# lenke182/flood-uav-video-segmentation

Hardware: AMD Instinct MI355X
Metric: segmentation FPS @713x713 (PSPNet-ResNet50 keyframe + linear interp, frame_delta=5) (higher is better)
Workload: dtype f32

## Files before the change

### flood_uav_video_segmentation_amd/_lib.py

```python
import ctypes
import os

import torch

_HERE = os.path.dirname(os.path.abspath(__file__))
LIB_PATH = os.path.join(_HERE, "libfloodseg.so")

c_float_p = ctypes.POINTER(ctypes.c_float)
c_void = ctypes.c_void_p
c_int = ctypes.c_int
c_i64 = ctypes.c_int64
c_f32 = ctypes.c_float


class FsConfig(ctypes.Structure):
    _fields_ = [("arch", c_int), ("layers", c_int), ("classes", c_int), ("patch", c_int), ("d_model", c_int),
                ("n_layers", c_int), ("dec_layers", c_int), ("image_size", c_int), ("flags", c_int), ("winograd_tile", c_int)]


ARCH_PSPNET = 0
ARCH_DEEPLABV3 = 1
ARCH_SEGMENTER = 2
OPT_NO_WINOGRAD = 1
OPT_NO_FUSED_HEAD = 2
OPT_NO_FUSED_SHORTCUT = 4
OPT_NO_FUSED_WINOGRAD = 8
OPT_NO_SPLIT_BF16 = 16
OPT_NO_RES_TOUCH = 128
OPT_NO_FUSED_POOL = 256
OPT_NO_FUSED_QKV = 1024
CONV_CHUNK_MAJOR = 0x400

_SIGNATURES = {
    "fs_version": (c_int, []),
    "fs_last_error": (ctypes.c_char_p, []),
    "fs_create": (c_int, [ctypes.POINTER(FsConfig), ctypes.POINTER(c_void)]),
    "fs_destroy": (c_int, [c_void]),
    "fs_load_weight": (c_int, [c_void, ctypes.c_char_p, c_void, ctypes.POINTER(c_i64), c_int, c_int, c_void]),
    "fs_finalize": (c_int, [c_void, c_void]),
    "fs_feature_shape": (c_int, [c_void, c_int, c_int, ctypes.POINTER(c_int), ctypes.POINTER(c_int), ctypes.POINTER(c_int)]),
    "fs_workspace_bytes": (ctypes.c_size_t, [c_void, c_int, c_int, c_int]),
    "fs_reserve": (c_int, [c_void, c_int, c_int, c_int, c_void]),
    "fs_reserved_bytes": (ctypes.c_size_t, [c_void]),
    "fs_encoder_forward": (c_int, [c_void, c_void, c_int, c_int, c_int, c_void, c_void]),
    "fs_decoder_forward": (c_int, [c_void, c_void, c_int, c_int, c_int, c_void, c_void]),
    "fs_segment_forward": (c_int, [c_void, c_void, c_int, c_int, c_int, c_void, c_void]),
    "fs_encoder_forward2": (c_int, [c_void, c_void, c_int, c_void, c_int, c_int, c_int, c_void, c_void]),
    "fs_segment_forward2": (c_int, [c_void, c_void, c_int, c_void, c_int, c_int, c_int, c_void, c_void]),
    "fs_segment_crops": (c_int, [c_void, c_void, c_void, c_int, c_int, c_int, ctypes.POINTER(c_int), ctypes.POINTER(c_int), c_int, c_int,
                                 c_void, c_void]),
    "fs_profile_enable": (c_int, [c_void, c_int]),
    "fs_profile_dump": (c_int, [c_void, ctypes.c_char_p, ctypes.c_size_t]),
    "fs_grid_sample_nchw": (c_int, [c_void, c_int, c_int, c_int, c_int, c_void, c_int, c_int, c_void, c_int, c_void]),
    "fs_grid_sample_nhwc": (c_int, [c_void, c_int, c_int, c_int, c_int, c_int, c_void, c_int, c_int, c_void, c_int, c_int, c_void]),
    "fs_resize_bilinear_nchw": (c_int, [c_void, c_int, c_int, c_int, c_void, c_int, c_int, c_int, c_void]),
    "fs_resize_bilinear_nhwc": (c_int, [c_void, c_int, c_int, c_int, c_int, c_int, c_void, c_int, c_int, c_int, c_int, c_void]),
    "fs_blend": (c_int, [c_void, c_f32, c_void, c_f32, c_void, c_i64, c_void]),
    "fs_seg_tail": (c_int, [c_void, c_void, ctypes.POINTER(c_void), ctypes.POINTER(c_void), c_int, c_int, c_int, c_int, c_int,
                            c_int, c_int, c_int, c_int, c_void, c_void, c_void, c_void]),
    "fs_feat_tail": (c_int, [c_void, c_void, c_int, c_int, c_int, ctypes.POINTER(c_void), ctypes.POINTER(c_void), c_int, c_int, c_void, c_int, c_int,
                             c_int, c_int, c_void, c_void, c_void]),
    "fs_seg_tail_accumulate": (c_int, [c_void, c_void, ctypes.POINTER(c_void), ctypes.POINTER(c_void), c_int, c_int, c_int, c_int, c_int,
                                       c_int, c_int, c_int, c_int, c_void, c_void, c_int, c_int, c_int, c_int, c_void, c_void]),
    "fs_canvas_resize_argmax": (c_int, [c_void, c_int, c_int, c_int, c_int, c_void, c_int, c_int, c_void]),
    "fs_crop_grids": (c_int, [ctypes.POINTER(c_void), c_int, c_int, c_int, c_int, c_int, c_int, ctypes.POINTER(c_int), ctypes.POINTER(c_int),
                              c_int, c_int, c_void, c_void]),
    "fs_crops_fuse": (c_int, [c_void, c_void, c_void, c_int, ctypes.POINTER(c_int), ctypes.POINTER(c_int)] + [c_int] * 9 + [c_void, c_void, c_int, c_int,
                              c_void, c_void]),
    "fs_argmax_u8": (c_int, [c_void, c_int, c_int, c_i64, c_void, c_void]),
    "fs_resize_crop": (c_int, [c_void, c_int, c_int, c_int, c_int, c_int, c_int, c_int, c_void, c_void, c_int, c_int, c_void]),
    "fs_resize_argmax_u8": (c_int, [c_void, c_int, c_int, c_int, c_int, c_void, c_int, c_int, c_void]),
    "fs_iou_hist": (c_int, [c_void, c_void, c_i64, c_int, c_int, c_void, c_void]),
    "fs_colorize": (c_int, [c_void, c_void, c_int, c_void, c_i64, c_void]),
    "fs_mv_to_grids": (c_int, [c_void, c_int, c_int, c_int, c_int, c_int, c_int, c_int, c_void, c_void, c_void, c_void]),
    "fs_softmax_accumulate": (c_int, [c_void, c_int, c_int, c_int, c_int, c_void, c_void, c_int, c_int, c_int, c_int, c_void]),
    "fs_canvas_finish": (c_int, [c_void, c_void, c_int, c_int, c_i64, c_void, c_void]),
    "fs_ms_prepare": (c_int, [c_void] + [c_int] * 6 + [c_float_p, c_float_p, c_void, c_int, c_void]),
    "fs_ms_fuse": (c_int, [c_void, c_void, c_int, ctypes.POINTER(c_int), ctypes.POINTER(c_int)] + [c_int] * 9 + [c_void, c_void] + [c_int] * 4
                   + [c_void, c_void]),
    "fs_test_hooks": (c_void, []),
}

_HOOKS = [
# ... 49 lines not shown
    ("seg_tail_weighted", c_int, [c_void, c_void, ctypes.POINTER(c_void), ctypes.POINTER(c_void)] + [c_int] * 9 + [c_void] * 4 + [c_int] * 4
     + [c_void, c_void, c_void]),
    ("crops_fuse_weighted", c_int, [c_void, c_void, c_void, c_int, ctypes.POINTER(c_int), ctypes.POINTER(c_int)] + [c_int] * 9
     + [c_void, c_void, c_int, c_int, c_void, c_void, c_void]),
    ("feat_tail_weighted", c_int, [c_void, c_void, c_int, c_int, c_int, ctypes.POINTER(c_void), ctypes.POINTER(c_void), c_int, c_int, c_void, c_int,
                                   c_int, c_int, c_int, c_void, c_void, c_void, c_void]),
    ("mask_confidence", c_int, [c_void] + [c_int] * 4 + [c_void, c_void, c_int, c_int, c_void]),
    ("canvas_confidence", c_int, [c_void] + [c_int] * 4 + [c_void, c_void, c_int, c_int, c_void]),
    ("frame_report", c_int, [c_void, c_void] + [c_int] * 5 + [c_void, c_void]),
    ("mask_regions", c_int, [c_void] + [c_int] * 5 + [c_void, c_void]),
    ("region_table", c_int, [c_void, c_void, c_void] + [c_int] * 6 + [c_void] * 5),
    ("region_filter", c_int, [c_void, c_void, c_void] + [c_int] * 6 + [c_void, c_void, c_void]),
    ("region_links", c_int, [c_void] * 6 + [c_int] * 6 + [c_void] * 5),
    ("region_tracks", c_int, [c_void] * 4 + [c_int] * 2 + [c_void] * 3),
    ("region_links_mc", c_int, [c_void] * 8 + [c_int] * 8 + [c_void] * 5),
]
EXT2_MAGIC = 0x4653455854414232

_EXT3_HOOKS = [
    ("region_outlines", c_int, [c_void] + [c_int] * 7 + [c_void] * 6),
]
EXT3_MAGIC = 0x4653455854414233

_EXT4_HOOKS = [
    ("outline_simplify", c_int, [c_void] * 3 + [c_int] * 5 + [c_void] * 5),
]
EXT4_MAGIC = 0x4653455854414234

_EXT5_HOOKS = [
    ("frame_compose_regions", c_int, [c_void, c_int, c_int, c_void, c_int, c_void, c_void, c_void] + [c_int] * 5 + [c_void, c_void, c_void] + [c_int] * 3
     + [c_void] * 4 + [c_int, c_void, c_int, c_void, c_int, c_int, c_i64, ctypes.c_uint32, ctypes.c_uint32, c_void, c_void]),
]
EXT5_MAGIC = 0x4653455854414235

_EXT6_HOOKS = [
    ("mask_stabilize", c_int, [c_void] * 4 + [c_int] * 9 + [c_void] * 5),
]
EXT6_MAGIC = 0x4653455854414236

_EXT7_HOOKS = [
    ("mask_distance", c_int, [c_void] + [c_int] * 3 + [ctypes.c_uint32, c_int] + [c_void] * 4),
    ("region_proximity", c_int, [c_void] * 5 + [c_int] * 5 + [ctypes.c_uint32, c_void, c_int] + [c_void] * 3),
]
EXT7_MAGIC = 0x4653455854414237

_EXT8_HOOKS = [
    ("global_motion", c_int, [c_void] * 3 + [ctypes.c_uint32] + [c_int] * 6 + [ctypes.c_int64, c_int, c_void, c_void]),
    ("pose_chain", c_int, [c_void] * 3 + [c_int] * 8 + [c_void]),
    ("mosaic_accumulate", c_int, [c_void] * 2 + [c_int] * 8 + [c_void] * 2),
    ("mosaic_resolve", c_int, [c_void] + [c_int] * 3 + [c_void] * 5),
]
EXT8_MAGIC = 0x4653455854414238


class FsTestApi(ctypes.Structure):
    _fields_ = [("size", ctypes.c_size_t)] + [(name, ctypes.CFUNCTYPE(res, *args)) for name, res, args in _HOOKS]


class FsExtApi(ctypes.Structure):
    _fields_ = [("magic", ctypes.c_uint64), ("size", ctypes.c_size_t)] + [(name, ctypes.CFUNCTYPE(res, *args)) for name, res, args in _EXT_HOOKS]


class FsHookTables(ctypes.Structure):
    _fields_ = [("test", FsTestApi), ("ext", FsExtApi)]


class FsExt2Api(ctypes.Structure):
    _fields_ = [("magic", ctypes.c_uint64), ("size", ctypes.c_size_t)] + [(name, ctypes.CFUNCTYPE(res, *args)) for name, res, args in _EXT2_HOOKS]


class FsHookTables2(ctypes.Structure):
    _fields_ = [("base", FsHookTables), ("ext2", FsExt2Api)]


class FsExt3Api(ctypes.Structure):
    _fields_ = [("magic", ctypes.c_uint64), ("size", ctypes.c_size_t)] + [(name, ctypes.CFUNCTYPE(res, *args)) for name, res, args in _EXT3_HOOKS]


class FsHookTables3(ctypes.Structure):
    _fields_ = [("base2", FsHookTables2), ("ext3", FsExt3Api)]


class FsExt4Api(ctypes.Structure):
    _fields_ = [("magic", ctypes.c_uint64), ("size", ctypes.c_size_t)] + [(name, ctypes.CFUNCTYPE(res, *args)) for name, res, args in _EXT4_HOOKS]


class FsHookTables4(ctypes.Structure):
    _fields_ = [("base3", FsHookTables3), ("ext4", FsExt4Api)]


class FsExt5Api(ctypes.Structure):
    _fields_ = [("magic", ctypes.c_uint64), ("size", ctypes.c_size_t)] + [(name, ctypes.CFUNCTYPE(res, *args)) for name, res, args in _EXT5_HOOKS]


class FsHookTables5(ctypes.Structure):
    _fields_ = [("base4", FsHookTables4), ("ext5", FsExt5Api)]


class FsExt6Api(ctypes.Structure):
    _fields_ = [("magic", ctypes.c_uint64), ("size", ctypes.c_size_t)] + [(name, ctypes.CFUNCTYPE(res, *args)) for name, res, args in _EXT6_HOOKS]


class FsHookTables6(ctypes.Structure):
    _fields_ = [("base5", FsHookTables5), ("ext6", FsExt6Api)]


class FsExt7Api(ctypes.Structure):
    _fields_ = [("magic", ctypes.c_uint64), ("size", ctypes.c_size_t)] + [(name, ctypes.CFUNCTYPE(res, *args)) for name, res, args in _EXT7_HOOKS]


class FsHookTables7(ctypes.Structure):
    _fields_ = [("base6", FsHookTables6), ("ext7", FsExt7Api)]


class FsExt8Api(ctypes.Structure):
    _fields_ = [("magic", ctypes.c_uint64), ("size", ctypes.c_size_t)] + [(name, ctypes.CFUNCTYPE(res, *args)) for name, res, args in _EXT8_HOOKS]


class FsHookTables8(ctypes.Structure):
    _fields_ = [("base7", FsHookTables7), ("ext8", FsExt8Api)]


class _Library:

    def __init__(self, cdll):
        self._cdll = cdll
        self._hooks = None
        self._ext = None
        self._ext2 = None
        self._ext3 = None
        self._ext4 = None
        self._ext5 = None
        self._ext6 = None
        self._ext7 = None
        self._ext8 = None

    def __getattr__(self, name):
        if name.startswith("fs_") and any(name == "fs_" + h[0] for h in _EXT8_HOOKS):
            if self._ext8 is None:
                all7 = ctypes.cast(self._cdll.fs_test_hooks(), ctypes.POINTER(FsHookTables7)).contents
                all5 = all7.base6.base5
                all2 = all5.base4.base3.base2
                if (all2.base.test.size != ctypes.sizeof(FsTestApi) or all2.base.ext.magic != EXT_MAGIC or all2.base.ext.size != ctypes.sizeof(FsExtApi)
                        or all2.ext2.magic != EXT2_MAGIC or all2.ext2.size != ctypes.sizeof(FsExt2Api)
                        or all5.base4.base3.ext3.magic != EXT3_MAGIC or all5.base4.base3.ext3.size != ctypes.sizeof(FsExt3Api)
                        or all5.base4.ext4.magic != EXT4_MAGIC or all5.base4.ext4.size != ctypes.sizeof(FsExt4Api)
                        or all5.ext5.magic != EXT5_MAGIC or all5.ext5.size != ctypes.sizeof(FsExt5Api)
                        or all7.base6.ext6.magic != EXT6_MAGIC or all7.base6.ext6.size != ctypes.sizeof(FsExt6Api)
                        or all7.ext7.magic != EXT7_MAGIC or all7.ext7.size != ctypes.sizeof(FsExt7Api)):
                    raise RuntimeError(f"floodseg: the library's first eight hook tables are not the ones this binding knows ({name} is missing)")
                ext8 = ctypes.cast(self._cdll.fs_test_hooks(), ctypes.POINTER(FsHookTables8)).contents.ext8
                if ext8.magic != EXT8_MAGIC:
                    raise RuntimeError(f"floodseg: the library has no eighth extension table ({name} is missing)")
                self._ext8 = ext8
            member = getattr(FsExt8Api, name[3:])
            if self._ext8.size < member.offset + member.size:
                raise RuntimeError(f"floodseg: the library's eighth extension table is older than this binding ({name} is missing)")
            fn = getattr(self._ext8, name[3:])
            setattr(self, name, fn)
            return fn
        if name.startswith("fs_") and any(name == "fs_" + h[0] for h in _EXT7_HOOKS):
            if self._ext7 is None:
                all6 = ctypes.cast(self._cdll.fs_test_hooks(), ctypes.POINTER(FsHookTables6)).contents
                all5 = all6.base5
                all2 = all5.base4.base3.base2
                if (all2.base.test.size != ctypes.sizeof(FsTestApi) or all2.base.ext.magic != EXT_MAGIC or all2.base.ext.size != ctypes.sizeof(FsExtApi)
                        or all2.ext2.magic != EXT2_MAGIC or all2.ext2.size != ctypes.sizeof(FsExt2Api)
                        or all5.base4.base3.ext3.magic != EXT3_MAGIC or all5.base4.base3.ext3.size != ctypes.sizeof(FsExt3Api)
                        or all5.base4.ext4.magic != EXT4_MAGIC or all5.base4.ext4.size != ctypes.sizeof(FsExt4Api)
                        or all5.ext5.magic != EXT5_MAGIC or all5.ext5.size != ctypes.sizeof(FsExt5Api)
                        or all6.ext6.magic != EXT6_MAGIC or all6.ext6.size != ctypes.sizeof(FsExt6Api)):
                    raise RuntimeError(f"floodseg: the library's first seven hook tables are not the ones this binding knows ({name} is missing)")
                ext7 = ctypes.cast(self._cdll.fs_test_hooks(), ctypes.POINTER(FsHookTables7)).contents.ext7
                if ext7.magic != EXT7_MAGIC:
                    raise RuntimeError(f"floodseg: the library has no seventh extension table ({name} is missing)")
                self._ext7 = ext7
            member = getattr(FsExt7Api, name[3:])
            if self._ext7.size < member.offset + member.size:
                raise RuntimeError(f"floodseg: the library's seventh extension table is older than this binding ({name} is missing)")
            fn = getattr(self._ext7, name[3:])
            setattr(self, name, fn)
            return fn
        if name.startswith("fs_") and any(name == "fs_" + h[0] for h in _EXT6_HOOKS):
            if self._ext6 is None:
                all5 = ctypes.cast(self._cdll.fs_test_hooks(), ctypes.POINTER(FsHookTables5)).contents
                all2 = all5.base4.base3.base2
                if (all2.base.test.size != ctypes.sizeof(FsTestApi) or all2.base.ext.magic != EXT_MAGIC or all2.base.ext.size != ctypes.sizeof(FsExtApi)
                        or all2.ext2.magic != EXT2_MAGIC or all2.ext2.size != ctypes.sizeof(FsExt2Api)
                        or all5.base4.base3.ext3.magic != EXT3_MAGIC or all5.base4.base3.ext3.size != ctypes.sizeof(FsExt3Api)
                        or all5.base4.ext4.magic != EXT4_MAGIC or all5.base4.ext4.size != ctypes.sizeof(FsExt4Api)
# ... 111 lines not shown
            f"{LIB_PATH} not found: build it with `python -c 'import __graft_entry__ as g; g.build()'` "
            "(hipcc --offload-arch=gfx950); there is no CPU fallback for this path")
    lib = ctypes.CDLL(LIB_PATH)
    for name, (res, args) in _SIGNATURES.items():
        if ALLOW_MISSING and not hasattr(lib, name):
            continue
        fn = getattr(lib, name)
        fn.restype = res
        fn.argtypes = args
    _lib = _Library(lib)
    return _lib


def exported_symbols():
    return sorted(_SIGNATURES)


def hook_names():
    return [h[0] for h in _HOOKS]


def ext_hook_names():
    return [h[0] for h in _EXT_HOOKS]


def ext2_hook_names():
    return [h[0] for h in _EXT2_HOOKS]


def ext3_hook_names():
    return [h[0] for h in _EXT3_HOOKS]


def ext4_hook_names():
    return [h[0] for h in _EXT4_HOOKS]


def ext5_hook_names():
    return [h[0] for h in _EXT5_HOOKS]


def ext6_hook_names():
    return [h[0] for h in _EXT6_HOOKS]


def ext7_hook_names():
    return [h[0] for h in _EXT7_HOOKS]


def ext8_hook_names():
    return [h[0] for h in _EXT8_HOOKS]


def check(rc):
    if rc != 0:
        msg = load().fs_last_error()
        raise RuntimeError("floodseg: " + (msg.decode() if msg else f"error {rc}"))


def stream_ptr(device=None):
    return ctypes.c_void_p(torch.cuda.current_stream(device).cuda_stream)


def one_device(*tensors, handle_device=None, what="floodseg"):
    dev = None
    for t in tensors:
        if t is None:
            continue
        if not t.is_cuda:
            raise RuntimeError(f"{what}: tensors must live on the GPU (no CPU fallback exists)")
        if dev is None:
            dev = t.device
        elif t.device != dev:
            raise RuntimeError(f"{what}: tensors on different devices ({dev} and {t.device})")
    if dev is None:
        raise RuntimeError(f"{what}: no device tensor given")
    if handle_device is not None and dev != handle_device:
        raise RuntimeError(f"{what}: tensor on {dev} but the network's weights live on {handle_device}")
    return dev


def ptr(t):
    if t is None:
        return ctypes.c_void_p(0)
    return ctypes.c_void_p(t.data_ptr())
```

### flood_uav_video_segmentation_amd/csrc/conv_igemm.hip

```cpp
#include "kernels.h"
#include "igemm_epilogue.h"

#include <algorithm>
#include <cstdlib>

namespace fs {

#define FS_DMA_PUBLISH() { __builtin_amdgcn_s_waitcnt(0x0070); __syncthreads(); }
constexpr int conv_split_rows(int BN, int waves) { return (BN / 16 + waves - 1) / waves * waves * 16; }
template <int BM, int BN, bool SPLIT, int WAVES = 4>
constexpr int conv_tile_lds_floats() { return 2 * (BM * 32 + (SPLIT ? 3 * conv_split_rows(BN, WAVES) * 16 : BN * 32)); }

template <int TM>
__device__ __forceinline__ void split_unit(int lvl, int pr, const f32x4 (&raw)[TM][2], float (&rq)[4 * TM][2], u32x4 (&ah)[TM][3], bool pin) {
    const int pi = pr / 4, pe = pr % 4;
    float x0 = lvl == 0 ? raw[pi][pe >> 1][2 * (pe & 1)] : rq[pr][0];
    float x1 = lvl == 0 ? raw[pi][pe >> 1][2 * (pe & 1) + 1] : rq[pr][1];
    unsigned pk = split_round(x0, x1);
    if (pin) asm volatile("" : "+v"(pk));
    ah[pi][lvl][pe] = pk;
    if (lvl < 2) {
        split_residue(pk, x0, x1);
        rq[pr][0] = x0;
        rq[pr][1] = x1;
    }
}

template <int BM, int BN, int WGM, int WGN, bool DUAL, bool SPLIT>
__device__ __forceinline__ void conv_tile(ConvParams p, const int m0, const int n0, float* __restrict__ lds) {
#if defined(__HIP_DEVICE_COMPILE__)
    constexpr int BK = 32;
    constexpr int NT = 64 * WGM * WGN;
    constexpr int RSTEP = NT / 8;
    constexpr int WM = BM / WGM, WN = BN / WGN;
    constexpr int TM = WM / 32, TN = WN / 32;
    constexpr int BNL = SPLIT ? conv_split_rows(BN, NT / 64) : BN;
    constexpr int BPL = BNL * 16;
    constexpr int RA = BM / RSTEP, RB = SPLIT ? 3 * (BNL / 16) / (NT / 64) : BN / RSTEP;
    constexpr int RB1 = SPLIT ? (BNL / 16) / (NT / 64) : RB;
    static_assert(BN % 32 == 0 && WN % 32 == 0 && (SPLIT || BN % RSTEP == 0), "tile columns: whole 32-column MFMA blocks per wave");
    constexpr int STAGE = BM * BK + (SPLIT ? 3 * BPL : BN * BK);

    const int t = threadIdx.x, lane = t & 63, wv = t >> 6;
    const int wm = wv / WGN, wn = wv % WGN, l31 = lane & 31, hh = lane >> 5;
    const int wv_u = __builtin_amdgcn_readfirstlane(wv);
    const int M = p.B * p.Ho * p.Wo;
    const int K = p.KH * p.KW * p.Cin + (DUAL ? p.Cin2 : 0);
    const int cpt = p.Cin >> 5;
    const int nchunks1 = p.KH * p.KW * cpt;
    const int nchunks = nchunks1 + (DUAL ? p.Cin2 >> 5 : 0);

    const int sc = t & 7, r0 = t >> 3;
    const int swz = sc ^ ((r0 >> 1) & 7);
    constexpr unsigned SENT = 0x80000000u;
    const long long pad_off = ((long long)p.pad * p.W + p.pad) * p.ld_in;
    const unsigned a_bytes = (unsigned)(((long long)p.B * p.H * p.W * p.ld_in + pad_off) * 4);
    const __amdgpu_buffer_rsrc_t a_rsrc = __builtin_amdgcn_make_buffer_rsrc((void*)(p.in - pad_off), 0, a_bytes, 0x00020000);
    const int ldw = p.ld_wgt ? p.ld_wgt : K;
    const __amdgpu_buffer_rsrc_t b_rsrc =
        SPLIT ? __builtin_amdgcn_make_buffer_rsrc((void*)p.wgt3, 0, 2u * p.plane_bytes + (unsigned)((((long long)p.Cout - 1) * ldw + K) * 2), 0x00020000)
              : __builtin_amdgcn_make_buffer_rsrc((void*)p.wgt, 0, (unsigned)((((long long)p.Cout - 1) * ldw + K) * 4), 0x00020000);
    unsigned a_voff[RA], a_mask[RA];
    if (p.KH * p.KW == 1 && p.stride == 1 && p.pad == 0) {
#pragma unroll
        for (int j = 0; j < RA; ++j) {
            const int m = m0 + r0 + RSTEP * j;
            a_voff[j] = (unsigned)((m * p.ld_in + swz * 4) * 4);
            a_mask[j] = m < M ? 1u : 0u;
        }
    } else {
#pragma unroll
        for (int j = 0; j < RA; ++j) {
            const int m = m0 + r0 + RSTEP * j;
            const bool v = m < M;
            const int mm = v ? m : 0;
            const int hw = p.Ho * p.Wo;
            const int b = mm / hw;
            const int rem = mm - b * hw;
            const int oy = rem / p.Wo;
            const int ox = rem - oy * p.Wo;
            a_voff[j] = (unsigned)(((b * p.H * p.W + oy * p.stride * p.W + ox * p.stride) * p.ld_in + swz * 4) * 4);
// ... 198 lines not shown
            __builtin_amdgcn_sched_barrier(0);
            cur ^= 1;
        }
        asm volatile("" ::"v"(touch0), "v"(touch1));
        if (!DUAL && p.res) igemm_load_residual(rv, p, M, em_base, en_base);
#undef FS_READ3
#undef FS_STEP3
    } else {
    if (!DUAL && p.res && nchunks <= 2) igemm_load_residual(rv, p, M, em_base, en_base);
    FS_FRAGS(0, 0, a0, b0)
    for (int kc = 0; kc < nchunks; ++kc) {
        FS_FRAGS(cur, 1, a1, b1)
        FS_MMA(a0, b0)
        __builtin_amdgcn_sched_group_barrier(0x008, 1, 0);
        __builtin_amdgcn_sched_group_barrier(0x100, TM + TN, 0);
        __builtin_amdgcn_sched_group_barrier(0x008, 4 * TM * TN - 1, 0);
        __builtin_amdgcn_sched_barrier(0);
        FS_FRAGS(cur, 2, a0, b0)
        __builtin_amdgcn_sched_barrier(0);
        FS_MMA(a1, b1)
        __builtin_amdgcn_sched_barrier(0);
        FS_FRAGS(cur, 3, a1, b1)
        __builtin_amdgcn_sched_barrier(0);
        FS_MMA(a0, b0)
        __builtin_amdgcn_sched_barrier(0);
        FS_DMA_PUBLISH()
        if (kc + 2 < nchunks) {
            FS_DMA_ALL(cur)
            FS_DMA_ADVANCE()
        }
        if (!DUAL && p.res && kc + 3 == nchunks) igemm_load_residual(rv, p, M, em_base, en_base);
        if (kc + 1 < nchunks) FS_FRAGS(cur ^ 1, 0, a0, b0)
        __builtin_amdgcn_sched_barrier(0);
        FS_MMA(a1, b1)
        __builtin_amdgcn_sched_barrier(0);
        cur ^= 1;
    }
    }
#undef FS_DMA_ROW
#undef FS_DMA_ADVANCE
#undef FS_DMA_ALL
#undef FS_FRAGS
#undef FS_MMA

    if constexpr (SPLIT && !DUAL && BN == 96 && TM == 1) {
        const int Dm = p.kv_heads * 64;
        if (p.kv_k && n0 >= Dm) {
            const int kind = n0 >= 2 * Dm ? 2 : 1;
            igemm_epilogue_kv<TN>(acc, sc_n, sh_n, p, kind, em_base, en_base - kind * Dm, en_base < p.Cout, lane);
            return;
        }
    }
    if (!DUAL && p.res) {
        if (p.relu == 1) igemm_epilogue<1, true>(acc, rv, sc_n, sh_n, p, M, em_base, en_base);
        else if (p.relu == 2) igemm_epilogue<2, true>(acc, rv, sc_n, sh_n, p, M, em_base, en_base);
        else igemm_epilogue<0, true>(acc, rv, sc_n, sh_n, p, M, em_base, en_base);
    } else {
        if (p.relu == 1) igemm_epilogue<1, false>(acc, rv, sc_n, sh_n, p, M, em_base, en_base);
        else if (p.relu == 2) igemm_epilogue<2, false>(acc, rv, sc_n, sh_n, p, M, em_base, en_base);
        else igemm_epilogue<0, false>(acc, rv, sc_n, sh_n, p, M, em_base, en_base);
    }
#endif
}

template <int BM, int BN, int WGM = 2, int WGN = 2, bool DUAL = false, bool SPLIT = false>
__global__ __launch_bounds__(64 * WGM * WGN) void conv_igemm_dma_f32(ConvParams p, int tiles_m, int tiles_n) {
#if defined(__HIP_DEVICE_COMPILE__)
    constexpr int PM = 8;
    __shared__ __attribute__((aligned(1024))) float lds[conv_tile_lds_floats<BM, BN, SPLIT, WGM * WGN>()];
    const int nblk = gridDim.x, bid = blockIdx.x;
    const int q = nblk >> 3, rr = nblk & 7, xcd = bid & 7;
    const int lid = (xcd < rr ? xcd * (q + 1) : rr * (q + 1) + (xcd - rr) * q) + (bid >> 3);
    const int per_group = tiles_m * tiles_n;
    const int grp = lid / per_group;
    const int lig = lid - grp * per_group;
    const int panel = lig / (PM * tiles_n);
    const int within = lig - panel * (PM * tiles_n);
    const int prow = min(PM, tiles_m - panel * PM);
    const int m0 = (panel * PM + within % prow) * BM, n0 = (within / prow) * BN;
    p.in += (long long)grp * p.g_in;
    p.wgt += (long long)grp * p.g_wgt;
    if (SPLIT) p.wgt3 = (const char*)p.wgt3 + (long long)grp * p.g_wgt * 2;
    p.out += (long long)grp * p.g_out;
    p.kv_b = grp;
    conv_tile<BM, BN, WGM, WGN, DUAL, SPLIT>(p, m0, n0, lds);
#endif
}

namespace {
struct TileCfg { int bm, bn; const char* name; };
const TileCfg kTiles[7] = {{0, 0, "auto"}, {128, 128, "igemm128x128"}, {128, 64, "igemm128x64"},
                           {64, 64, "igemm64x64"}, {64, 128, "igemm64x128"}, {0, 0, nullptr}, {128, 96, "split128x96"}};
bool tile_id_ok(int tile) { return tile >= 0 && tile <= 6 && tile != 5; }

int pick_tile(const ConvParams& p) {
    const int M = p.B * p.Ho * p.Wo;
    const double eff[7] = {0, 1.00, 0.92, 0.80, 0.92, 0, 0.97};
    int best = 1;
    double best_t = 1e300;
    const int last = p.in2 ? 2 : p.wgt3 ? 3 : 4;
    for (int c = 1; c <= 6; ++c) {
        if (c > last && !(c == 6 && p.wgt3 && !p.in2 && p.Cout % 96 == 0)) continue;
        const int bm = kTiles[c].bm, bn = kTiles[c].bn;
        if (p.Cout < bn && bn > 64) continue;
        const long tiles = (long)cdiv(M, bm) * cdiv(p.Cout, bn) * (p.groups > 1 ? p.groups : 1);
        const long per_cu = (tiles + 255) / 256;
        const double t = (double)per_cu * bm * bn / (eff[c] * (per_cu >= 2 ? 1.0 : 0.8));
        if (t < best_t) { best_t = t; best = c; }
    }
    return best;
}
}

const char* conv_igemm_tile_name(const ConvParams& p, int tile) {
    if (!tile_id_ok(tile)) return "(bad tile)";
    if (tile == 0) tile = pick_tile(p);
    if (p.in2 && p.wgt3) return tile == 2 ? "split128x64cat" : "split128x128cat";
    if (p.in2) return tile == 2 ? "igemm128x64cat" : "igemm128x128cat";
    if (p.wgt3) return tile == 1 ? "split128x128" : tile == 2 ? "split128x64" : tile == 4 ? "split64x128" : tile == 6 ? "split128x96" : "split64x64";
    return kTiles[tile].name;
}

namespace {
bool ldw_ok(const ConvParams& p) { return (p.ld_wgt ? p.ld_wgt : p.KH * p.KW * p.Cin + (p.in2 ? p.Cin2 : 0)) % 8 == 0; }

__global__ void split_bf16x3_kernel(const float* __restrict__ w, long long n, unsigned short* __restrict__ planes) {
    const long long i = (long long)blockIdx.x * blockDim.x + threadIdx.x;
    if (i >= n) return;
    split3(w[i], planes[i], planes[n + i], planes[2 * n + i]);
}
}

int launch_split_bf16x3(const float* w, long long n, void* planes, hipStream_t s) {
    FS_REQUIRE(w && planes && n > 0 && n % 8 == 0, "split_bf16x3: bad arguments (n=%lld)", n);
    hipLaunchKernelGGL(split_bf16x3_kernel, dim3((unsigned)((n + 255) / 256)), dim3(256), 0, s, w, n, (unsigned short*)planes);
    FS_HIP(hipGetLastError());
    return 0;
}

namespace {
int check_conv_params(const ConvParams& p) {
    FS_REQUIRE(p.Cin % 32 == 0, "conv_igemm: Cin=%d must be a multiple of 32", p.Cin);
    if (p.in2) {
        FS_REQUIRE(p.KH == 1 && p.KW == 1 && p.stride == 1 && p.pad == 0 && p.res == nullptr && p.groups <= 1,
                   "conv_igemm: a concatenated-K launch takes two 1x1 convs, the first with stride 1, and no residual");
        FS_REQUIRE(p.Cin2 >= 32 && p.Cin2 % 32 == 0 && p.ld_in2 % 4 == 0 && p.ld_in2 >= p.Cin2 && p.stride2 >= 1 && ((uintptr_t)p.in2 & 15) == 0,
                   "conv_igemm: bad second operand (Cin2=%d ld=%d stride=%d)", p.Cin2, p.ld_in2, p.stride2);
        FS_REQUIRE((p.H2 - 1) / p.stride2 + 1 == p.Ho && (p.W2 - 1) / p.stride2 + 1 == p.Wo, "conv_igemm: second operand %dx%d / stride %d does not give %dx%d",
                   p.H2, p.W2, p.stride2, p.Ho, p.Wo);
        FS_REQUIRE((int64_t)p.B * p.H2 * p.W2 * p.ld_in2 * 4 < (int64_t)1 << 31, "conv_igemm: second operand must be smaller than 2 GiB");
    }
    FS_REQUIRE(p.ld_in % 4 == 0 && p.ld_in >= p.Cin, "conv_igemm: bad ld_in=%d (Cin=%d)", p.ld_in, p.Cin);
    FS_REQUIRE(p.ld_out >= p.Cout, "conv_igemm: bad ld_out=%d (Cout=%d)", p.ld_out, p.Cout);
    FS_REQUIRE(((uintptr_t)p.in & 15) == 0 && ((uintptr_t)p.wgt & 15) == 0, "conv_igemm: unaligned operand");
    FS_REQUIRE(p.Ho == (p.H + 2 * p.pad - p.dil * (p.KH - 1) - 1) / p.stride + 1 &&
               p.Wo == (p.W + 2 * p.pad - p.dil * (p.KW - 1) - 1) / p.stride + 1,
               "conv_igemm: output geometry %dx%d inconsistent with input %dx%d", p.Ho, p.Wo, p.H, p.W);
    FS_REQUIRE(((int64_t)p.B * p.H * p.W * p.ld_in + ((int64_t)p.pad * p.W + p.pad) * p.ld_in) * 4 < (int64_t)1 << 31,
               "conv_igemm: input tensor must be smaller than 2 GiB");
    FS_REQUIRE((int64_t)p.Cout * std::max(p.ld_wgt, p.KH * p.KW * p.Cin + (p.in2 ? p.Cin2 : 0)) * 4 < (int64_t)1 << 31, "conv_igemm: filter bank must be smaller than 2 GiB");
    FS_REQUIRE(p.ld_wgt == 0 || (p.ld_wgt >= p.KH * p.KW * p.Cin + (p.in2 ? p.Cin2 : 0) && p.ld_wgt % 4 == 0), "conv_igemm: bad ld_wgt=%d", p.ld_wgt);
    FS_REQUIRE(p.KH * p.KW <= 32, "conv_igemm: at most 32 filter taps");
    FS_REQUIRE((int64_t)p.B * p.Ho * p.Wo * p.ld_out * 4 < (int64_t)1 << 31 && ((uintptr_t)p.out & 3) == 0,
               "conv_igemm: output tensor must be smaller than 2 GiB");
    FS_REQUIRE(p.res == nullptr || (int64_t)p.B * p.Ho * p.Wo * p.ld_res * 4 < (int64_t)1 << 31, "conv_igemm: residual tensor must be smaller than 2 GiB");
    if (!(p.res == nullptr || p.ld_res >= p.Cout)) return fail("conv_igemm: bad ld_res");
    return 0;
}
}

int launch_conv_igemm(const ConvParams& p, hipStream_t s, int tile) {
    FS_TRY(check_conv_params(p));
    FS_REQUIRE(tile_id_ok(tile), "conv_igemm: tile %d is not 0..4 or 6", tile);
    if (tile == 0) tile = pick_tile(p);
    FS_REQUIRE(tile < 6 || (p.wgt3 && !p.in2), "conv_igemm: tile 6 (128 x 96) exists on the split-operand route only");
    const int M = p.B * p.Ho * p.Wo;
    const int bm = kTiles[tile].bm, bn = kTiles[tile].bn;
    const int tm = cdiv(M, bm), tn = cdiv(p.Cout, bn);
    const int groups = p.groups > 1 ? p.groups : 1;
    FS_REQUIRE(groups == 1 || p.res == nullptr, "conv_igemm: grouped GEMM has no residual input");
    const dim3 grid(tm * tn * groups), block(256);
    if (p.kv_k) {
        const int Dm = p.kv_heads * 64;
        FS_REQUIRE(tile == 6 && p.wgt3 && !p.in2 && !p.res && p.KH == 1 && p.KW == 1 && p.stride == 1 && p.pad == 0 && p.relu == 0,
                   "conv_igemm: the K / V plane epilogue belongs to a plain Linear on the 128 x 96 split tile");
        FS_REQUIRE(p.kv_vt && p.kv_heads >= 1 && Dm % 96 == 0 && p.Cout == 3 * Dm && p.kv_N == M && p.kv_Npad % 32 == 0 && p.kv_Npad >= M &&
                       p.kv_Npad <= tm * bm && (int64_t)3 * p.kv_plane_bytes < (int64_t)1 << 31 &&
                       (int64_t)p.kv_plane_bytes == (int64_t)groups * p.kv_heads * p.kv_Npad * 128 && (((uintptr_t)p.kv_k | (uintptr_t)p.kv_vt) & 15) == 0,
                   "conv_igemm: bad K / V plane geometry (heads %d, tokens %d, padded %d)", p.kv_heads, p.kv_N, p.kv_Npad);
    }
    if (p.wgt3) {
        FS_REQUIRE(((uintptr_t)p.wgt3 & 15) == 0 && p.plane_bytes % 16 == 0 && (int64_t)3 * p.plane_bytes < (int64_t)1 << 31 && ldw_ok(p),
                   "conv_igemm: bad split filter bank (plane_bytes=%u)", p.plane_bytes);
        FS_REQUIRE((int64_t)groups * p.g_wgt * 2 <= (int64_t)p.plane_bytes, "conv_igemm: the groups' filters (%d x %lld) exceed a plane of the split bank", groups, p.g_wgt);
    }
    if (p.in2 && p.wgt3) {
        if (tile == 2) hipLaunchKernelGGL((conv_igemm_dma_f32<128, 64, 4, 1, true, true>), grid, block, 0, s, p, tm, tn);
        else if (tile == 1) hipLaunchKernelGGL((conv_igemm_dma_f32<128, 128, 4, 1, true, true>), grid, block, 0, s, p, tm, tn);
        else return fail("conv_igemm: concatenated-K launches use tile 1 or 2");
        FS_HIP(hipGetLastError());
        return 0;
    }
    if (p.in2) {
        if (tile == 2) hipLaunchKernelGGL((conv_igemm_dma_f32<128, 64, 2, 2, true>), grid, block, 0, s, p, tm, tn);
        else if (tile == 1) hipLaunchKernelGGL((conv_igemm_dma_f32<128, 128, 2, 2, true>), grid, block, 0, s, p, tm, tn);
        else return fail("conv_igemm: concatenated-K launches use tile 1 or 2");
        FS_HIP(hipGetLastError());
        return 0;
    }
    if (p.wgt3) {
        switch (tile) {
            case 1: hipLaunchKernelGGL((conv_igemm_dma_f32<128, 128, 4, 1, false, true>), grid, block, 0, s, p, tm, tn); break;
            case 2: hipLaunchKernelGGL((conv_igemm_dma_f32<128, 64, 4, 1, false, true>), grid, block, 0, s, p, tm, tn); break;
            case 3: hipLaunchKernelGGL((conv_igemm_dma_f32<64, 64, 2, 2, false, true>), grid, block, 0, s, p, tm, tn); break;
            case 4: hipLaunchKernelGGL((conv_igemm_dma_f32<64, 128, 2, 2, false, true>), grid, block, 0, s, p, tm, tn); break;
            case 6: hipLaunchKernelGGL((conv_igemm_dma_f32<128, 96, 4, 1, false, true>), grid, block, 0, s, p, tm, tn); break;
            default: return fail("conv_igemm: the split-operand route has tiles 1, 2, 3, 4 and 6");
        }
        FS_HIP(hipGetLastError());
        return 0;
    }
#define FS_CONV_LAUNCH(BM_, BN_) hipLaunchKernelGGL((conv_igemm_dma_f32<BM_, BN_>), grid, block, 0, s, p, tm, tn);
    switch (tile) {
        case 1: FS_CONV_LAUNCH(128, 128) break;
        case 2: FS_CONV_LAUNCH(128, 64) break;
        case 3: FS_CONV_LAUNCH(64, 64) break;
        default: FS_CONV_LAUNCH(64, 128) break;
    }
#undef FS_CONV_LAUNCH
    FS_HIP(hipGetLastError());
    return 0;
}


}
```

### flood_uav_video_segmentation_amd/csrc/igemm_epilogue.h

```cpp
#pragma once
#include "kernels.h"
#include "split.h"

namespace fs {

#if defined(__HIP_DEVICE_COMPILE__)
template <int TM, int TN>
__device__ __forceinline__ void igemm_load_residual(float (&rv)[TM][TN][16], const ConvParams& p, int M, int m_base, int n_base) {
    constexpr unsigned SENT = 0x80000000u;
    const __amdgpu_buffer_rsrc_t r_rsrc = __builtin_amdgcn_make_buffer_rsrc((void*)p.res, 0, (unsigned)((long long)M * p.ld_res * 4), 0x00020000);
    const unsigned row_r = (unsigned)p.ld_res * 4u;
#pragma unroll
    for (int j = 0; j < TN; ++j) {
        const int n = n_base + j * 32;
#pragma unroll
        for (int i = 0; i < TM; ++i) {
            const unsigned vr = n < p.Cout ? (unsigned)(m_base + i * 32) * row_r + (unsigned)n * 4u : SENT;
#pragma unroll
            for (int e = 0; e < 16; ++e)
                rv[i][j][e] = __builtin_bit_cast(float, __builtin_amdgcn_raw_buffer_load_b32(r_rsrc, vr + (unsigned)mfma32_row(e, 0) * row_r, 0, 0));
        }
    }
}

__device__ __forceinline__ float gelu_erf(float x) {
    const float a = fminf(fabsf(x), 4.f);
    float q = -1.434946029e-07f;
    q = fmaf(q, a, 3.633772167e-06f);
    q = fmaf(q, a, -4.095856275e-05f);
    q = fmaf(q, a, 2.688578097e-04f);
    q = fmaf(q, a, -1.106124604e-03f);
    q = fmaf(q, a, 2.616208512e-03f);
    q = fmaf(q, a, -3.566103114e-04f);
    q = fmaf(q, a, -2.759680524e-02f);
    q = fmaf(q, a, 1.482741833e-01f);
    q = fmaf(q, a, 9.184474349e-01f);
    q = fmaf(q, a, 1.627907038e+00f);
    return copysignf(1.f - __builtin_amdgcn_exp2f(-(q * a)), x);
}

template <int ACT, bool RES, int TM, int TN>
__device__ __forceinline__ void igemm_epilogue(const f32x16 (&acc)[TM][TN], const float (&rv)[TM][TN][16], const float (&sc)[TN],
                                               const float (&sh)[TN], const ConvParams& p, int M, int m_base, int n_base) {
    constexpr unsigned SENT = 0x80000000u;
    const __amdgpu_buffer_rsrc_t o_rsrc = __builtin_amdgcn_make_buffer_rsrc((void*)p.out, 0, (unsigned)((long long)M * p.ld_out * 4), 0x00020000);
    const unsigned row_o = (unsigned)p.ld_out * 4u;
#pragma unroll
    for (int j = 0; j < TN; ++j) {
        const int n = n_base + j * 32;
        const bool nok = n < p.Cout;
#pragma unroll
        for (int i = 0; i < TM; ++i) {
            const int mb = m_base + i * 32;
            const unsigned vo = nok ? (unsigned)mb * row_o + (unsigned)n * 4u : SENT;
#pragma unroll
            for (int e = 0; e < 16; ++e) {
                float v = acc[i][j][e] * sc[j] + sh[j];
                if (RES) v += rv[i][j][e];
                if (ACT == 1) v = fmaxf(v, 0.f);
                else if (ACT == 2) v = 0.5f * v * (1.f + gelu_erf(v * 0.70710678118654752f));
                __builtin_amdgcn_raw_buffer_store_b32(__builtin_bit_cast(unsigned, v), o_rsrc, vo + (unsigned)mfma32_row(e, 0) * row_o, 0, 0);
            }
        }
    }
}

template <int TN>
__device__ __forceinline__ void igemm_epilogue_kv(const f32x16 (&acc)[1][TN], const float (&sc)[TN], const float (&sh)[TN], const ConvParams& p, int kind,
                                                  int m_base, int n_rel, bool col_ok, int lane) {
    constexpr unsigned SENT = 0x80000000u;
    const int hh = lane >> 5, odd = lane & 1;
    const int N = p.kv_N, Npad = p.kv_Npad;
    const __amdgpu_buffer_rsrc_t rsrc = __builtin_amdgcn_make_buffer_rsrc((void*)(kind == 1 ? p.kv_k : p.kv_vt), 0, 3u * p.kv_plane_bytes, 0x00020000);
#pragma unroll
    for (int j = 0; j < TN; ++j) {
        const int n = n_rel + j * 32;
        const int bh = p.kv_b * p.kv_heads + (n >> 6), d = n & 63;
        if (kind == 1) {
#pragma unroll
            for (int ep = 0; ep < 8; ++ep) {
                const int e0 = 2 * ep, key0 = m_base + mfma32_row(e0, 0);
                const float v0 = key0 < N ? acc[0][j][e0] * sc[j] + sh[j] : 0.f;
                const float v1 = key0 + 1 < N ? acc[0][j][e0 + 1] * sc[j] + sh[j] : 0.f;
                unsigned H, Mm, L;
                split_pair(v0, v1, H, Mm, L);
                const unsigned send_hm = odd ? ((H & 0xffffu) | (Mm << 16)) : ((H >> 16) | (Mm & 0xffff0000u));
                const unsigned send_l = odd ? (L & 0xffffu) : (L >> 16);
                const unsigned recv_hm = (unsigned)__builtin_amdgcn_mov_dpp((int)send_hm, 0xB1, 0xf, 0xf, true);
                const unsigned recv_l = (unsigned)__builtin_amdgcn_mov_dpp((int)send_l, 0xB1, 0xf, 0xf, true);
                const unsigned oH = odd ? ((recv_hm & 0xffffu) | (H & 0xffff0000u)) : ((H & 0xffffu) | (recv_hm << 16));
                const unsigned oM = odd ? ((recv_hm >> 16) | (Mm & 0xffff0000u)) : ((Mm & 0xffffu) | (recv_hm & 0xffff0000u));
                const unsigned oL = odd ? ((recv_l & 0xffffu) | (L & 0xffff0000u)) : ((L & 0xffffu) | (recv_l << 16));
                const int key = key0 + odd;
                const unsigned vo = (col_ok && key < Npad) ? (unsigned)(((bh * Npad + key) * 64 + (d & ~1)) * 2) : SENT;
                __builtin_amdgcn_raw_buffer_store_b32(oH, rsrc, vo, 0, 0);
                __builtin_amdgcn_raw_buffer_store_b32(oM, rsrc, vo, (int)p.kv_plane_bytes, 0);
                __builtin_amdgcn_raw_buffer_store_b32(oL, rsrc, vo, (int)(2u * p.kv_plane_bytes), 0);
            }
        } else {
            const int kb = m_base - 4 * hh;
#pragma unroll
            for (int g = 0; g < 2; ++g) {
                u32x4 H, Mm, L;
#pragma unroll
                for (int t2 = 0; t2 < 4; ++t2) {
                    const int e0 = 8 * g + 2 * t2, key0 = m_base + mfma32_row(e0, 0);
                    const float v0 = key0 < N ? acc[0][j][e0] * sc[j] + sh[j] : 0.f;
                    const float v1 = key0 + 1 < N ? acc[0][j][e0 + 1] * sc[j] + sh[j] : 0.f;
                    unsigned h, m, l;
                    split_pair(v0, v1, h, m, l);
                    H[t2] = h; Mm[t2] = m; L[t2] = l;
                }
                const unsigned vo = (col_ok && kb < Npad) ? (unsigned)(((bh * 64 + d) * Npad + kb + 16 * g + 8 * hh) * 2) : SENT;
                __builtin_amdgcn_raw_buffer_store_b128(H, rsrc, vo, 0, 0);
                __builtin_amdgcn_raw_buffer_store_b128(Mm, rsrc, vo, (int)p.kv_plane_bytes, 0);
// ... 9 lines not shown
```

### flood_uav_video_segmentation_amd/csrc/kernels.h

```cpp
#pragma once
#include "common.h"

namespace fs {

struct ConvParams {
    const float* in;    int ld_in;
    const float* wgt;
    int ld_wgt;
    const float* scale;
    const float* shift;
    const float* res;   int ld_res;
    float* out;         int ld_out;
    int B, H, W, Cin;
    int Ho, Wo, Cout;
    int KH, KW, stride, pad, dil;
    const float* in2;   int ld_in2;
    int Cin2, stride2, H2, W2;
    int relu;
    int res_touch;
    int korder;
    int groups;
    long long g_in, g_wgt, g_out;
    const void* wgt3;
    unsigned plane_bytes;
    unsigned short* kv_k;
    unsigned short* kv_vt;
    int kv_N, kv_Npad, kv_heads;
    unsigned kv_plane_bytes;
    int kv_b;
};
int launch_conv_igemm(const ConvParams& p, hipStream_t s, int tile = 0);
const char* conv_igemm_tile_name(const ConvParams& p, int tile = 0);
int launch_split_bf16x3(const float* w, long long n, void* planes, hipStream_t s);

static inline int conv_out_size(int in, int k, int stride, int pad, int dil) { return (in + 2 * pad - dil * (k - 1) - 1) / stride + 1; }
static inline ConvParams conv2d_params(const float* in, int ld_in, const float* wgt, const float* scale, const float* shift, const float* res, int ld_res,
                                       float* out, int ld_out, int B, int H, int W, int Cin, int Cout, int KH, int KW, int stride, int pad, int dil,
                                       int relu, int korder) {
    ConvParams p{};
    p.in = in; p.ld_in = ld_in; p.wgt = wgt; p.scale = scale; p.shift = shift; p.res = res; p.ld_res = ld_res; p.out = out; p.ld_out = ld_out;
    p.B = B; p.H = H; p.W = W; p.Cin = Cin; p.Cout = Cout;
    p.Ho = conv_out_size(H, KH, stride, pad, dil);
    p.Wo = conv_out_size(W, KW, stride, pad, dil);
    p.KH = KH; p.KW = KW; p.stride = stride; p.pad = pad; p.dil = dil; p.relu = relu; p.korder = korder;
    return p;
}
static inline ConvParams gemm_params(const float* in, int ld_in, const float* w, float* out, int ld_out, int rows, int K, int N) {
    return conv2d_params(in, ld_in, w, nullptr, nullptr, nullptr, 0, out, ld_out, 1, rows, 1, K, N, 1, 1, 1, 0, 1, 0, 0);
}
static inline void attach_planes(ConvParams& p, const void* planes, size_t elems) {
    p.wgt3 = planes;
    p.plane_bytes = (unsigned)(elems * 2);
}

struct FrameSrc {
    const float* in;
    const float* in2;
    int B1;
    int ncrops, FH, FW;
    short cy[32], cx[32];
};
static inline FrameSrc frames_plain(const float* in, const float* in2, int B1) {
    FrameSrc f{};
    f.in = in;
    f.in2 = in2;
    f.B1 = B1;
    return f;
}

struct StemParams {
    FrameSrc src;
    const float* wgt;
    const float* scale; const float* shift;
    float* out; int ld_out;
    int B, H, W, Ho, Wo, Cout, KH, KW, stride, pad;
    int split;
};
int launch_stem_conv(const StemParams& p, hipStream_t s);
static inline StemParams stem_params(const FrameSrc& src, const float* wgt, const float* scale, const float* shift, float* out, int B, int H, int W,
                                     int Cout, int KH, int KW, int stride, int pad, int split) {
    StemParams p{};
    p.src = src; p.wgt = wgt; p.scale = scale; p.shift = shift; p.out = out; p.ld_out = Cout;
    p.B = B; p.H = H; p.W = W; p.Cout = Cout; p.KH = KH; p.KW = KW; p.stride = stride; p.pad = pad; p.split = split;
    p.Ho = conv_out_size(H, KH, stride, pad, 1);
    p.Wo = conv_out_size(W, KW, stride, pad, 1);
// ... 165 lines not shown
int launch_region_links(const int* index, const long long* table, const long long* counts, const int* prev_index, const long long* prev_table,
                        const long long* prev_counts, int n, int H, int W, int max_regions, int max_pairs, int min_overlap, int* back, int* fwd,
                        long long* link_counts, void* workspace, hipStream_t s);
int launch_region_links_mc(const int* index, const long long* table, const long long* counts, const int* prev_index, const long long* prev_table,
                           const long long* prev_counts, const int* mv, const int* pair_stats, int n, int H, int W, int frame_h, int frame_w,
                           int max_regions, int max_pairs, int min_overlap, int* back, int* fwd, long long* link_counts, void* workspace, hipStream_t s);
int launch_region_tracks(const int* back, const int* fwd, const long long* counts, const long long* prev_tracks, int n, int max_regions,
                         long long* state, long long* tracks, hipStream_t s);

int launch_mask_stabilize(const uint8_t* mask, const uint8_t* conf, const int* mv, const int* pair_stats, int n, int H, int W, int frame_h, int frame_w,
                          int K, int persist, int trust, int has_state, uint32_t* state, uint8_t* out, long long* counts, void* workspace, hipStream_t s);

int launch_mask_distance(const uint8_t* mask, int n, int H, int W, uint32_t source_set, int max_dist, uint32_t* d2, int32_t* nearest, void* workspace,
                         hipStream_t s);
int launch_region_proximity(const uint8_t* mask, const uint32_t* d2, const int32_t* nearest, const int32_t* index, const long long* counts, int n, int H,
                            int W, int K, int max_regions, uint32_t target_set, const int32_t* thresholds, int B, long long* exposure, long long* near,
                            hipStream_t s);

int launch_global_motion(const int32_t* tables, const int32_t* pair_stats, const uint8_t* mask, uint32_t exclude_set, int n, int FH, int FW, int H, int W,
                         int rounds, long long tol_q20, int min_inliers, long long* model, hipStream_t s);
int launch_pose_chain(const long long* model, long long* state, long long* poses, int n, int H, int W, int CH, int CW, int ox, int oy, int max_bridge,
                      hipStream_t s);
int launch_mosaic_accumulate(const uint8_t* mask, const long long* poses, int n, int H, int W, int K, int CH, int CW, int ox, int oy, uint16_t* votes,
                             hipStream_t s);
int launch_mosaic_resolve(const uint16_t* votes, int K, int CH, int CW, uint8_t* cls, uint8_t* conf, uint32_t* seen, long long* totals, hipStream_t s);

int launch_region_outlines(const int* index, int n, int H, int W, int max_regions, int connectivity, int max_contours, int max_vertices,
                           long long* contours, int* vertices, long long* shape, long long* counts, void* workspace, hipStream_t s);

int launch_outline_simplify(const long long* contours, const int* vertices, const long long* counts, int n, int max_contours, int max_vertices, int tol_q,
                            int max_rounds, long long* simple, int* simple_vertices, long long* simple_counts, void* workspace, hipStream_t s);

int launch_patchify(const float* in, const float* in2, int B1, float* out, int B, int H, int W, int P, int gh, int gw, hipStream_t s);
int launch_vit_assemble(const float* emb, const float* cls, const float* pos, float* X, int B, int N, int D, hipStream_t s);
int launch_dec_assemble(const float* Y, const float* cls_emb, float* Z, int B, int N, int K, int D, hipStream_t s);
int launch_layernorm(const float* in, const float* gamma, const float* beta, float* out, int rows, int D, int rows_per_batch,
                     int drop_first, hipStream_t s);
size_t attention_scratch_floats(int B, int N, int heads);
int launch_attention_f32(const float* qkv, float* out, int B, int N, int heads, float scale, float* scratch, hipStream_t s);
size_t attention_split_floats(int B, int N, int heads);
int launch_attention_split(const float* qkv, float* out, int B, int N, int heads, float scale, float* scratch, float* planes, hipStream_t s, bool planes_ready = false);
int launch_splitk_combine(const float* part, int nsplit, const float* bias, const float* res, float* out, int rows, int N, hipStream_t s);
int launch_splitk_combine_ln(const float* part, int nsplit, const float* bias, const float* res, float* out, const float* gamma, const float* beta,
                             float* ln_out, int rows, int N, hipStream_t s);
int launch_mask_head(const float* pp, const float* cc, const float* gamma, const float* beta, float* out, int B, int N, int K,
                     int D, hipStream_t s);


int launch_winograd_filter(const float* w, float* U , int O, int I, int mt, hipStream_t s, int chunk_major = 0);
int launch_winograd_input(const float* in, int ld_in, float* V , int B, int H, int W, int C, int dil, int mt,
                          hipStream_t s);
int launch_winograd_output(const float* M , const float* scale, const float* shift, float* out, int ld_out, int B,
                           int H, int W, int N, int relu, int dil, int mt, hipStream_t s);
struct WinoLayout { bool tile_major; long long s_pos, s_tile; };
WinoLayout winograd_layout(int mt, long long T, int C);
static inline ConvParams winograd_gemm_params(const float* V, const float* U, float* M, int mt, int T, int Cin, int Cout) {
    ConvParams p = gemm_params(V, Cin, U, M, Cout, T, Cin, Cout);
    const WinoLayout a = winograd_layout(mt, T, Cin), o = winograd_layout(mt, T, Cout);
    p.ld_in = (int)a.s_tile;
    p.g_in = a.s_pos;
    p.ld_out = (int)o.s_tile;
    p.g_out = o.s_pos;
    p.groups = (mt + 2) * (mt + 2);
    p.g_wgt = (long long)Cout * Cin;
    return p;
}
static inline size_t wino_v_floats(int mt, size_t T, int Cin, size_t align) { return ((size_t)(mt + 2) * (mt + 2) * T * Cin + align - 1) / align * align; }
static inline size_t wino_vm_floats(int mt, size_t T, int Cin, int Cout, size_t align) {
    return wino_v_floats(mt, T, Cin, align) + (size_t)(mt + 2) * (mt + 2) * T * Cout;
}
static inline int winograd_tiles(int B, int H, int W, int dil, int mt) {
    return B * dil * dil * ((cdiv(H, dil) + mt - 1) / mt) * ((cdiv(W, dil) + mt - 1) / mt);
}
static inline double winograd_gemm_rows(int B, int H, int W, int dil, int mt) {
    return (double)(mt + 2) * (mt + 2) * (double)(cdiv(winograd_tiles(B, H, W, dil, mt), 64) * 64);
}
static inline int winograd_pick_m(int , int H, int W, int dil) {
    const int m = winograd_gemm_rows(1, H, W, dil, 6) < winograd_gemm_rows(1, H, W, dil, 4) ? 6 : 4;
    return winograd_gemm_rows(1, H, W, dil, 3) < winograd_gemm_rows(1, H, W, dil, m) ? 3 : m;
}
static inline int wino_m(int force, int H, int W, int dil) { return force ? force : winograd_pick_m(1, H, W, dil); }

size_t wino_fused_bank_floats(int Cin, int Cout);
bool wino_fused_supported(int Cin, int Cout, int KH, int KW, int stride, int pad, int dil);
int launch_wino4_filter_packed(const float* w, float* U, int O, int I, hipStream_t s, int chunk_major = 0);
int launch_wino4_fused(const float* in, int ld_in, const float* U, const float* scale, const float* shift, float* out, int ld_out, int B, int H,
                       int W, int Cin, int Cout, int relu, hipStream_t s, int variant = 0);

int launch_wino4_fused_pool(const float* in, int ld_in, const float* U, const float* scale, const float* shift, float* pool, int ld_pool, int B,
                            int H, int W, int Cin, int Cout, hipStream_t s);

}
```

### flood_uav_video_segmentation_amd/csrc/net.h

```cpp
#pragma once
#include <map>
#include <memory>
#include <string>
#include <vector>

#include "../../include/floodseg.h"
#include "kernels.h"

namespace fs {

struct RawTensor {
    float* d = nullptr;
    std::vector<int64_t> shape;
    int64_t numel() const {
        int64_t n = 1;
        for (auto s : shape) n *= s;
        return n;
    }
};

struct WinoBank {
    float* U4 = nullptr;
    float* U6 = nullptr;
    float* U3 = nullptr;
    hipEvent_t ready[3] = {nullptr, nullptr, nullptr};
    hipStream_t built_on[3] = {nullptr, nullptr, nullptr};
};

struct ConvBN {
    std::string name;
    float* w = nullptr;
    float* scale = nullptr;
    float* shift = nullptr;
    int Cin = 0, Cout = 0, KH = 1, KW = 1, stride = 1, pad = 0, dil = 1, relu = 0;
    int korder = 0;
    std::shared_ptr<WinoBank> wino;
    float* wf = nullptr;
    int out_size(int in) const { return conv_out_size(in, KH, stride, pad, dil); }
};

struct Bottleneck {
    ConvBN c1, c2, c3, ds;
    bool has_ds = false;
    ConvBN c3ds;
    int ds_cin = 0, ds_stride = 1;
};

struct Linear {
    std::string name;
    float* w = nullptr;
    float* b = nullptr;
    int in = 0, out = 0;
};
struct LNorm {
    float* g = nullptr;
    float* b = nullptr;
    int D = 0;
};
struct VitBlock {
    LNorm n1, n2;
    Linear qkv, proj, fc1, fc2;
};

struct ProfRec {
    std::string name, kernel;
    double flops = 0, bytes = 0;
    hipEvent_t e0 = nullptr, e1 = nullptr;
};

}

struct fs_net {
    fs_config cfg{};
    bool finalized = false;
    std::map<std::string, fs::RawTensor> raw;
    std::vector<float*> owned;

    bool deep_stem = true;
    fs::ConvBN stem[3];
    std::vector<fs::Bottleneck> blocks;
    std::vector<int> layer_end;
    fs::ConvBN ppm[4];
    int bins[4] = {1, 2, 3, 6};
    fs::ConvBN cls_conv;
    fs::ConvBN cls_main;
    fs::ConvBN ppm_z[4];
    float* seg_feat = nullptr;
    size_t seg_feat_elems = 0;
    float* cls_w = nullptr;
    float* cls_b = nullptr;
    fs::ConvBN aspp[4];
    fs::ConvBN aspp_pool;
    fs::ConvBN project, head_conv;
    int cls_cin = 512;

    fs::Linear patch_embed;
    float* cls_token = nullptr;
    float* pos_embed = nullptr;
    int pos_g0 = 0;
    float* pos_cur = nullptr;
    int pos_gh = 0, pos_gw = 0;
    std::vector<fs::VitBlock> enc_blocks, dec_blocks;
    fs::LNorm enc_norm, dec_norm, mask_norm;
    fs::Linear proj_dec, proj_patch, proj_classes;
    float* cls_emb = nullptr;
    float* vit_ws = nullptr;
    size_t vit_ws_elems = 0;
    float* wino_ws = nullptr;
    size_t wino_ws_elems = 0;
    std::vector<hipEvent_t> bank_events;
    size_t bank_elems = 0;
    size_t pos_elems = 0;
    size_t ws_allocs = 0;
    bool use_winograd = true;
    int wino_force_m = 0;
    bool use_fused_head = true;
    bool use_fused_shortcut = true;
    bool use_fused_winograd = true;
    bool use_split = true;
    bool use_fused_qkv = true;
    bool use_fused_pool = true;
    bool res_touch = true;
    std::map<const float*, std::pair<void*, size_t>> split_banks;
    int device = 0;

    float* buf[4] = {nullptr, nullptr, nullptr, nullptr};
    size_t buf_elems = 0;
    float* small = nullptr;
    size_t small_elems = 0;

    bool profiling = false;
    std::vector<fs::ProfRec> prof;

    int feat_channels() const {
        if (cfg.arch == FS_ARCH_SEGMENTER) return cfg.d_model;
        return cfg.arch == FS_ARCH_PSPNET ? 4096 : 2048;
    }
};

namespace fs {
int net_create(const fs_config* cfg, fs_handle* out);
int net_destroy(fs_handle h);
int check_device(fs_net* h, const char* what);
int net_load_weight(fs_handle h, const char* name, const float* data, const int64_t* shape, int ndim, int on_device,
                    hipStream_t s);
int net_finalize(fs_handle h, hipStream_t s);
int net_feature_shape(fs_handle h, int H, int W, int* C, int* fh, int* fw);
size_t net_workspace_bytes(fs_handle h, int B, int H, int W);
int net_reserve(fs_handle h, int B, int H, int W, hipStream_t s);
size_t net_reserved_bytes(fs_handle h);
int net_encoder(fs_handle h, const FrameSrc& src, int B, int H, int W, float* out_nhwc, hipStream_t s);
int net_segment(fs_handle h, const FrameSrc& src, int B, int H, int W, float* out_nchw, hipStream_t s);
int net_decoder(fs_handle h, const float* feat, int B, int fh, int fw, float* out_nchw, hipStream_t s);
int net_profile_dump(fs_handle h, char* buf, size_t n);

int dev_alloc(fs_net* h, float** p, size_t elems);
int ws_grow(fs_net* h, float** p, size_t* have, size_t need, bool zero);
int split_attach(fs_net* h, const float* bank, size_t elems, hipStream_t s);
void split_use(const fs_net* h, ConvParams& p);

int linear_splits(int K, int N, int rows_per_image, int act, bool split_route);
ConvParams linear_params(const float* in, const float* w, const float* bias, const float* res, float* out, int rows, int K, int N, int act,
                         bool res_touch);
ConvParams linear_splitk_params(const float* in, const float* w, float* part, int rows, int K, int N, int split);
ConvParams linear_qkv_params(const float* in, const float* w, const float* bias, float* out, int B, int tokens, int D, float* planes);
ConvParams dual_conv_params(const float* a, int ld_a, const float* b, int ld_b, const float* wgt, const float* shift, float* out, int ld_out, int B,
                            int Ho, int Wo, int Cin, int Cin2, int H2, int W2, int stride2, int Cout, int relu);
ConvParams ppm_z_params(const float* reduced, const float* zw, float* zbuf, int B, int Cr, int Cout9);
int pyramid_pool(fs_net* h, const float* feat, int ld_feat, float* pooled, int B, int H, int W, int C, const int bins[4], hipStream_t s);
int conv_winograd(fs_net* h, const std::string& name, const float* in, int ld_in, const float* U, const void* U3, unsigned plane_bytes, float* V,
                  float* M, const float* scale, const float* shift, float* out, int ld_out, int B, int H, int W, int Cin, int Cout, int dil,
                  int relu, int mt, hipStream_t s);
int vit_reserve(fs_handle h, int B, int H, int W, hipStream_t s);
int fetch(fs_net* h, const std::string& name, const RawTensor** out);
int prof_begin(fs_net* h, const std::string& name, const char* kernel, double flops, double bytes, hipStream_t s);
int prof_end(fs_net* h, hipStream_t s);
int run_igemm(fs_net* h, const std::string& name, const ConvParams& p, double flops, double bytes, hipStream_t s, int tile = 0);
int vit_finalize(fs_handle h, hipStream_t s);
int vit_feature_shape(fs_handle h, int H, int W, int* C, int* fh, int* fw);
int vit_encoder(fs_handle h, const FrameSrc& src, int B, int H, int W, float* out_tokens, hipStream_t s);
int vit_decoder(fs_handle h, const float* tokens, int B, int gh, int gw, float* out_nchw, hipStream_t s);
}
```

### flood_uav_video_segmentation_amd/csrc/net.hip

```cpp
#include "net.h"

#include <cmath>
#include <cstdarg>
#include <cstring>

namespace fs {

std::string& last_error() {
    static thread_local std::string e;
    return e;
}
int fail(const char* fmt, ...) {
    char buf[1024];
    va_list ap;
    va_start(ap, fmt);
    vsnprintf(buf, sizeof(buf), fmt, ap);
    va_end(ap);
    last_error() = buf;
    return 1;
}

int dev_alloc(fs_net* h, float** p, size_t elems) {
    FS_HIP(hipMalloc(reinterpret_cast<void**>(p), std::max<size_t>(elems, 4) * sizeof(float)));
    h->owned.push_back(*p);
// ... 14 lines not shown
}

int split_attach(fs_net* h, const float* bank, size_t elems, hipStream_t s) {
    if (!h->use_split || elems % 8 != 0 || h->split_banks.count(bank)) return 0;
    float* planes = nullptr;
    FS_TRY(dev_alloc(h, &planes, (3 * elems + 1) / 2));
    FS_TRY(launch_split_bf16x3(bank, (long long)elems, planes, s));
    h->split_banks[bank] = {planes, elems};
    return 0;
}

void split_use(const fs_net* h, ConvParams& p) {
    p.wgt3 = nullptr;
    if (!h->use_split || p.Cin % 32 != 0 || h->split_banks.empty()) return;
    auto it = h->split_banks.upper_bound(p.wgt);
    if (it == h->split_banks.begin()) return;
    --it;
    const size_t off = (size_t)(p.wgt - it->first), elems = it->second.second;
    const int K = p.KH * p.KW * p.Cin + (p.in2 ? p.Cin2 : 0);
    if (off >= elems || off % 8 != 0 || (p.ld_wgt ? p.ld_wgt : K) % 8 != 0 || elems * 6 >= ((size_t)1 << 31)) return;
    p.wgt3 = (const char*)it->second.first + off * 2;
    p.plane_bytes = (unsigned)(elems * 2);
}

int fetch(fs_net* h, const std::string& name, const RawTensor** out) {
    auto it = h->raw.find(name);
    if (it == h->raw.end()) return fail("missing weight '%s'", name.c_str());
    *out = &it->second;
    return 0;
}

int to_host(const RawTensor& t, std::vector<float>& v) {
    v.resize((size_t)t.numel());
    FS_HIP(hipMemcpy(v.data(), t.d, v.size() * sizeof(float), hipMemcpyDeviceToHost));
    return 0;
}

namespace {

bool wino_eligible(const ConvBN& c, bool hwio) {
    return !hwio && c.KH == 3 && c.KW == 3 && c.stride == 1 && c.pad == c.dil && c.Cin >= 128 && c.Cin % 32 == 0 && c.Cout % 4 == 0;
}

int wino_bank(fs_net* h, const ConvBN& c, int mt, hipStream_t s, const float** U) {
    const int k = mt == 6 ? 1 : mt == 3 ? 2 : 0;
    float*& slot = mt == 6 ? c.wino->U6 : mt == 3 ? c.wino->U3 : c.wino->U4;
    if (!slot) {
        FS_REQUIRE(c.korder == 1, "winograd: conv '%s' has no chunk-major filter bank", c.name.c_str());
        float* bank = nullptr;
        const size_t elems = (size_t)(mt + 2) * (mt + 2) * c.Cout * c.Cin;
        FS_TRY(dev_alloc(h, &bank, elems));
        FS_TRY(launch_winograd_filter(c.w, bank, c.Cout, c.Cin, mt, s, 1));
        FS_TRY(split_attach(h, bank, elems, s));
        hipEvent_t ev = nullptr;
        FS_HIP(hipEventCreateWithFlags(&ev, hipEventDisableTiming));
        FS_HIP(hipEventRecord(ev, s));
        c.wino->ready[k] = ev;
        c.wino->built_on[k] = s;
        h->bank_events.push_back(ev);
        h->bank_elems += elems + (h->use_split ? (3 * elems + 1) / 2 : 0);
        ++h->ws_allocs;
        slot = bank;
    } else if (c.wino->built_on[k] != s && c.wino->ready[k]) {
        FS_HIP(hipStreamWaitEvent(s, c.wino->ready[k], 0));
    }
    *U = slot;
    return 0;
}

int fetch_host(fs_net* h, const std::string& name, std::vector<float>& v) {
    const RawTensor* t;
    FS_TRY(fetch(h, name, &t));
    return to_host(*t, v);
}

int make_conv(fs_net* h, ConvBN& c, const std::string& wname, const std::string& bn, const std::string& bias, int stride,
              int pad, int dil, int relu, bool hwio, hipStream_t s) {
    const RawTensor* w;
    FS_TRY(fetch(h, wname, &w));
    FS_REQUIRE(w->shape.size() == 4, "weight '%s' is not 4-D", wname.c_str());
    c.name = wname;
    c.Cout = (int)w->shape[0];
    c.Cin = (int)w->shape[1];
    c.KH = (int)w->shape[2];
    c.KW = (int)w->shape[3];
    c.stride = stride;
    c.pad = pad;
    c.dil = dil;
    c.relu = relu;
    FS_TRY(dev_alloc(h, &c.w, (size_t)w->numel()));
    if (hwio) {
        FS_TRY(launch_pack_oihw_to_hwio(w->d, c.w, c.Cout, c.Cin, c.KH, c.KW, s));
    } else if (c.KH * c.KW > 1 && c.Cin % 32 == 0) {
        c.korder = 1;
        FS_TRY(launch_pack_oihw_chunk_major(w->d, c.w, c.Cout, c.Cin, c.KH, c.KW, s));
    } else {
        FS_TRY(launch_pack_oihw_to_ohwi(w->d, c.w, c.Cout, c.Cin, c.KH, c.KW, s));
    }
    if (!hwio && c.Cin % 32 == 0) FS_TRY(split_attach(h, c.w, (size_t)w->numel(), s));
    if (wino_eligible(c, hwio)) c.wino = std::make_shared<WinoBank>();
    if (!hwio && c.korder == 1 && c.Cin <= 128 && wino_fused_supported(c.Cin, c.Cout, c.KH, c.KW, c.stride, c.pad, c.dil)) {
        FS_TRY(dev_alloc(h, &c.wf, wino_fused_bank_floats(c.Cin, c.Cout)));
        FS_TRY(launch_wino4_filter_packed(c.w, c.wf, c.Cout, c.Cin, s, 1));
    }
    if (!bn.empty()) {
        const size_t n = (size_t)c.Cout;
// ... 17 lines not shown
        const RawTensor* b;
        FS_TRY(fetch(h, bias, &b));
        FS_REQUIRE(b->numel() == c.Cout, "bias '%s' does not match %d output channels", bias.c_str(), c.Cout);
        FS_TRY(dev_alloc(h, &c.shift, (size_t)c.Cout));
        FS_HIP(hipMemcpy(c.shift, b->d, (size_t)c.Cout * sizeof(float), hipMemcpyDeviceToDevice));
    }
    return 0;
}

}

int prof_begin(fs_net* h, const std::string& name, const char* kernel, double flops, double bytes, hipStream_t s) {
    if (!h || !h->profiling) return 0;
    ProfRec r;
    r.name = name;
    r.kernel = kernel;
    r.flops = flops;
    r.bytes = bytes;
    FS_HIP(hipEventCreate(&r.e0));
    FS_HIP(hipEventCreate(&r.e1));
    FS_HIP(hipEventRecord(r.e0, s));
    h->prof.push_back(r);
    return 0;
}
int prof_end(fs_net* h, hipStream_t s) {
    if (!h || !h->profiling) return 0;
    FS_HIP(hipEventRecord(h->prof.back().e1, s));
    return 0;
}

int run_igemm(fs_net* h, const std::string& name, const ConvParams& p, double flops, double bytes, hipStream_t s, int tile) {
    FS_TRY(prof_begin(h, name, conv_igemm_tile_name(p, tile), flops, bytes, s));
    FS_TRY(launch_conv_igemm(p, s, tile));
    return prof_end(h, s);
}

int conv_winograd(fs_net* h, const std::string& name, const float* in, int ld_in, const float* U, const void* U3, unsigned plane_bytes, float* V,
                  float* M, const float* scale, const float* shift, float* out, int ld_out, int B, int H, int W, int Cin, int Cout, int dil,
                  int relu, int mt, hipStream_t s) {
    const int T = winograd_tiles(B, H, W, dil, mt);
    ConvParams p = winograd_gemm_params(V, U, M, mt, T, Cin, Cout);
    p.wgt3 = U3;
    p.plane_bytes = plane_bytes;
    const double G = p.groups, v_elems = G * T * Cin, m_elems = G * T * Cout, px = (double)B * H * W;
    FS_TRY(prof_begin(h, name + ".wino_in", "winograd_input", 0, 4.0 * (px * Cin + v_elems), s));
    FS_TRY(launch_winograd_input(in, ld_in, V, B, H, W, Cin, dil, mt, s));
    FS_TRY(prof_end(h, s));
    FS_TRY(run_igemm(h, name + ".wino_gemm", p, 2.0 * G * (double)T * Cin * Cout, 4.0 * (v_elems + G * Cout * Cin + m_elems), s));
    FS_TRY(prof_begin(h, name + ".wino_out", "winograd_output", 0, 4.0 * (m_elems + px * Cout), s));
    FS_TRY(launch_winograd_output(M, scale, shift, out, ld_out, B, H, W, Cout, relu, dil, mt, s));
    return prof_end(h, s);
}

namespace {

int run_conv_winograd(fs_net* h, const ConvBN& c, const float* in, int ld_in, int B, int H, int W, float* out, int ld_out,
                      hipStream_t s) {
    const int mt = wino_m(h->wino_force_m, H, W, c.dil);
    const size_t T = (size_t)winograd_tiles(B, H, W, c.dil, mt);
    const float* U = nullptr;
    FS_TRY(wino_bank(h, c, mt, s, &U));
    FS_TRY(ws_grow(h, &h->wino_ws, &h->wino_ws_elems, wino_vm_floats(mt, T, c.Cin, c.Cout, 8), false));
    float* V = h->wino_ws;
    float* M = h->wino_ws + wino_v_floats(mt, T, c.Cin, 8);
    ConvParams bank = winograd_gemm_params(V, U, M, mt, (int)T, c.Cin, c.Cout);
    split_use(h, bank);
    return conv_winograd(h, c.name, in, ld_in, U, bank.wgt3, bank.plane_bytes, V, M, c.scale, c.shift, out, ld_out, B, H, W, c.Cin, c.Cout,
                         c.dil, c.relu, mt, s);
}

bool takes_winograd(const fs_net* h, const ConvBN& c, int B, int H, int W, bool has_res) {
    if (!(c.wino && h->use_winograd && !has_res)) return false;
    if (c.Cin < 256 && c.wf && h->use_fused_winograd && (long)cdiv(H, 4) * cdiv(W, 4) >= 1500) return false;
    const int mt = wino_m(h->wino_force_m, H, W, c.dil);
    const double wino_rows = (double)(mt + 2) * (mt + 2) * winograd_tiles(B, H, W, c.dil, mt);
    const double direct_rows = 9.0 * (double)B * c.out_size(H) * c.out_size(W);
    return wino_rows < (c.dil <= 4 ? 0.8 : 0.7) * direct_rows;
}

int reserve_conv(fs_net* h, const ConvBN& c, int B, int H, int W, hipStream_t s, size_t* need) {
    if (!takes_winograd(h, c, B, H, W, false)) return 0;
    const int mt = wino_m(h->wino_force_m, H, W, c.dil);
    *need = std::max(*need, wino_vm_floats(mt, (size_t)winograd_tiles(B, H, W, c.dil, mt), c.Cin, c.Cout, 8));
    const float* U = nullptr;
    return wino_bank(h, c, mt, s, &U);
}

bool takes_fused_winograd(const fs_net* h, const ConvBN& c, int B, int H, int W, int ld_in, int ld_out, bool has_res) {
    const bool fits = (int64_t)B * H * W * ld_in * 4 < ((int64_t)1 << 30) && (int64_t)B * H * W * ld_out * 4 < ((int64_t)1 << 31);
    return c.wf && h->use_fused_winograd && !has_res && fits && (long)cdiv(H, 4) * cdiv(W, 4) >= 500;
}

ConvParams conv_params(const fs_net* h, const ConvBN& c, const float* in, int ld_in, int B, int H, int W, float* out, int ld_out, const float* res,
                       int ld_res) {
    ConvParams p = conv2d_params(in, ld_in, c.w, c.scale, c.shift, res, ld_res, out, ld_out, B, H, W, c.Cin, c.Cout, c.KH, c.KW, c.stride, c.pad,
                                 c.dil, c.relu, c.korder);
    p.res_touch = res != nullptr && h->res_touch;
    split_use(h, p);
    return p;
}

int run_conv(fs_net* h, const ConvBN& c, const float* in, int ld_in, int B, int H, int W, float* out, int ld_out,
             const float* res, int ld_res, hipStream_t s) {
    if (takes_winograd(h, c, B, H, W, res != nullptr)) return run_conv_winograd(h, c, in, ld_in, B, H, W, out, ld_out, s);
    if (takes_fused_winograd(h, c, B, H, W, ld_in, ld_out, res != nullptr)) {
        const double tiles = (double)B * cdiv(H, 4) * cdiv(W, 4);
        FS_TRY(prof_begin(h, c.name, "wino_fused", 2.0 * 36.0 * tiles * c.Cin * c.Cout,
                          4.0 * ((double)B * H * W * (c.Cin + c.Cout) + 36.0 * c.Cin * c.Cout), s));
        FS_TRY(launch_wino4_fused(in, ld_in, c.wf, c.scale, c.shift, out, ld_out, B, H, W, c.Cin, c.Cout, c.relu, s));
        return prof_end(h, s);
    }
    ConvParams p = conv_params(h, c, in, ld_in, B, H, W, out, ld_out, res, ld_res);
    const double M = (double)B * p.Ho * p.Wo;
    const double flops = 2.0 * M * c.Cout * c.KH * c.KW * c.Cin;
    const double bytes = 4.0 * ((double)B * H * W * c.Cin + (double)c.Cout * c.KH * c.KW * c.Cin + M * c.Cout * (res ? 2 : 1));
    return run_igemm(h, c.name, p, flops, bytes, s);
}

int ensure_workspace(fs_net* h, size_t buf_elems, size_t small_elems) {
    if (buf_elems > h->buf_elems) {
        for (int i = 0; i < 4; ++i) {
            size_t have = h->buf_elems;
            FS_TRY(ws_grow(h, &h->buf[i], &have, buf_elems, false));
        }
        h->buf_elems = buf_elems;
    }
    return ws_grow(h, &h->small, &h->small_elems, small_elems, true);
}

struct Geometry {
    int H1, W1, H2, W2, H3, W3;
};

Geometry geometry(const fs_net* h, int H, int W) {
    Geometry g;
    g.H1 = h->stem[0].out_size(H);
    g.W1 = h->stem[0].out_size(W);
    g.H2 = conv_out_size(g.H1, 3, 2, 1, 1);
    g.W2 = conv_out_size(g.W1, 3, 2, 1, 1);
    g.H3 = conv_out_size(g.H2, 3, 2, 1, 1);
    g.W3 = conv_out_size(g.W2, 3, 2, 1, 1);
    return g;
}

size_t encoder_buf_elems(const fs_net* h, int B, int H, int W) {
    const Geometry g = geometry(h, H, W);
    const size_t a = (size_t)B * g.H1 * g.W1 * 128;
    const size_t b = (size_t)B * g.H2 * g.W2 * 256;
    const size_t c = (size_t)B * g.H3 * g.W3 * 2048;
    return std::max(a, std::max(b, c));
}

size_t small_elems_for(int B) { return (size_t)B * (50 * 2048 + 4 * 36 * (512 + 9 * 512)) + 1024; }

}

int net_create(const fs_config* cfg, fs_handle* out) {
    FS_REQUIRE(cfg && out, "fs_create: null argument");
    FS_REQUIRE(cfg->arch == FS_ARCH_PSPNET || cfg->arch == FS_ARCH_DEEPLABV3 || cfg->arch == FS_ARCH_SEGMENTER,
               "fs_create: unknown arch %d", cfg->arch);
    FS_REQUIRE(cfg->arch == FS_ARCH_SEGMENTER || cfg->layers == 50 || cfg->layers == 101 || cfg->layers == 152,
               "fs_create: layers must be 50, 101 or 152");
    const int max_classes = cfg->arch == FS_ARCH_PSPNET ? 32 : 64;
    FS_REQUIRE(cfg->classes >= 1 && cfg->classes <= max_classes, "fs_create: classes out of range (%d; this arch takes 1..%d)", cfg->classes, max_classes);
    FS_REQUIRE((cfg->flags & ~(FS_OPT_NO_WINOGRAD | FS_OPT_NO_FUSED_HEAD | FS_OPT_NO_FUSED_SHORTCUT | FS_OPT_NO_FUSED_WINOGRAD | FS_OPT_NO_SPLIT_BF16 |
                               FS_OPT_NO_RES_TOUCH | FS_OPT_NO_FUSED_POOL | FS_OPT_NO_FUSED_QKV)) == 0,
               "fs_create: unknown option bits 0x%x", cfg->flags);
    FS_REQUIRE(cfg->winograd_tile == 0 || cfg->winograd_tile == 3 || cfg->winograd_tile == 4 || cfg->winograd_tile == 6,
               "fs_create: winograd_tile must be 0, 3, 4 or 6");
    fs_net* h = new fs_net();
    h->cfg = *cfg;
    h->use_winograd = !(cfg->flags & FS_OPT_NO_WINOGRAD);
    h->wino_force_m = cfg->winograd_tile;
    h->use_fused_head = !(cfg->flags & FS_OPT_NO_FUSED_HEAD);
    h->use_fused_shortcut = !(cfg->flags & FS_OPT_NO_FUSED_SHORTCUT);
    h->use_fused_winograd = !(cfg->flags & (FS_OPT_NO_FUSED_WINOGRAD | FS_OPT_NO_WINOGRAD));
    h->use_split = !(cfg->flags & FS_OPT_NO_SPLIT_BF16);
    h->res_touch = !(cfg->flags & FS_OPT_NO_RES_TOUCH);
    h->use_fused_pool = !(cfg->flags & FS_OPT_NO_FUSED_POOL);
    h->use_fused_qkv = h->use_split && !(cfg->flags & FS_OPT_NO_FUSED_QKV);
    if (hipGetDevice(&h->device) != hipSuccess) {
        delete h;
        return fail("fs_create: no HIP device");
    }
    h->deep_stem = cfg->arch == FS_ARCH_PSPNET;
    *out = h;
    return 0;
}

int check_device(fs_net* h, const char* what) {
    int cur = -1;
    FS_HIP(hipGetDevice(&cur));
    FS_REQUIRE(cur == h->device, "%s: the handle was created on HIP device %d but device %d is current", what, h->device, cur);
    return 0;
}

int net_destroy(fs_handle h) {
    if (!h) return 0;
    (void)hipDeviceSynchronize();
    for (auto& kv : h->raw)
        if (kv.second.d) (void)hipFree(kv.second.d);
    for (float* p : h->owned) (void)hipFree(p);
    for (int i = 0; i < 4; ++i)
        if (h->buf[i]) (void)hipFree(h->buf[i]);
    if (h->small) (void)hipFree(h->small);
    if (h->vit_ws) (void)hipFree(h->vit_ws);
    if (h->seg_feat) (void)hipFree(h->seg_feat);
    if (h->wino_ws) (void)hipFree(h->wino_ws);
    if (h->pos_cur) (void)hipFree(h->pos_cur);
    for (hipEvent_t e : h->bank_events) (void)hipEventDestroy(e);
    for (auto& r : h->prof) {
        (void)hipEventDestroy(r.e0);
        (void)hipEventDestroy(r.e1);
    }
    delete h;
    return 0;
}

int net_load_weight(fs_handle h, const char* name, const float* data, const int64_t* shape, int ndim, int on_device,
                    hipStream_t s) {
    FS_REQUIRE(h && name && data && (shape || ndim == 0), "fs_load_weight: null argument");
    FS_REQUIRE(!h->finalized, "fs_load_weight: network already finalized");
    FS_TRY(check_device(h, "fs_load_weight"));
    RawTensor t;
    t.shape.assign(shape, shape + ndim);
    const int64_t n = t.numel();
    FS_REQUIRE(n > 0, "fs_load_weight: '%s' is empty", name);
    auto it = h->raw.find(name);
    if (it != h->raw.end()) {
        (void)hipFree(it->second.d);
        h->raw.erase(it);
    }
    FS_HIP(hipMalloc(reinterpret_cast<void**>(&t.d), (size_t)n * sizeof(float)));
    FS_HIP(hipMemcpyAsync(t.d, data, (size_t)n * sizeof(float), on_device ? hipMemcpyDeviceToDevice : hipMemcpyHostToDevice, s));
    h->raw[name] = t;
    return 0;
}

namespace {
int load_classifier(fs_net* h, const std::string& prefix, int K) {
    const RawTensor *w, *b;
    FS_TRY(fetch(h, prefix + ".weight", &w));
    FS_TRY(fetch(h, prefix + ".bias", &b));
    FS_REQUIRE(w->shape.size() == 4 && w->shape[0] == K && w->shape[1] == h->cls_cin, "%s.weight has wrong shape", prefix.c_str());
    FS_TRY(dev_alloc(h, &h->cls_w, (size_t)w->numel()));
    FS_TRY(dev_alloc(h, &h->cls_b, (size_t)K));
    FS_HIP(hipMemcpy(h->cls_w, w->d, (size_t)w->numel() * sizeof(float), hipMemcpyDeviceToDevice));
    FS_HIP(hipMemcpy(h->cls_b, b->d, (size_t)K * sizeof(float), hipMemcpyDeviceToDevice));
    return 0;
}

int release_raw(fs_net* h) {
    FS_HIP(hipDeviceSynchronize());
    for (auto& kv : h->raw) {
        (void)hipFree(kv.second.d);
        kv.second.d = nullptr;
    }
    h->raw.clear();
    h->finalized = true;
    return 0;
}
// ... 119 lines not shown

int net_feature_shape(fs_handle h, int H, int W, int* C, int* fh, int* fw) {
    FS_REQUIRE(h && h->finalized, "fs_feature_shape: network not finalized");
    if (h->cfg.arch == FS_ARCH_SEGMENTER) return vit_feature_shape(h, H, W, C, fh, fw);
    const Geometry g = geometry(h, H, W);
    if (C) *C = h->feat_channels();
    if (fh) *fh = g.H3;
    if (fw) *fw = g.W3;
    return 0;
}

size_t net_workspace_bytes(fs_handle h, int B, int H, int W) {
    if (!h || !h->finalized) return 0;
    if (h->cfg.arch == FS_ARCH_SEGMENTER) {
        const int P = h->cfg.patch, D = h->cfg.d_model;
        const size_t T = (size_t)B * (((H + P - 1) / P) * ((W + P - 1) / P) + 1 + h->cfg.classes);
        return (T * D * 15 + T * 3 * P * P + 64) * sizeof(float);
    }
    return (4 * encoder_buf_elems(h, B, H, W) + small_elems_for(B)) * sizeof(float);
}

int net_reserve(fs_handle h, int B, int H, int W, hipStream_t s) {
    FS_REQUIRE(h && h->finalized, "fs_reserve: network not finalized");
    FS_TRY(check_device(h, "fs_reserve"));
    FS_REQUIRE(B >= 1 && H >= 1 && W >= 1, "fs_reserve: bad arguments (B=%d H=%d W=%d)", B, H, W);
    if (h->cfg.arch == FS_ARCH_SEGMENTER) return vit_reserve(h, B, H, W, s);
    FS_REQUIRE(H >= 33 && W >= 33, "fs_reserve: frames of at least 33 x 33 (got %d x %d)", H, W);
    const Geometry g = geometry(h, H, W);
    const int fh = g.H3, fw = g.W3;
    const size_t px = (size_t)B * fh * fw;
    const bool psp = h->cfg.arch == FS_ARCH_PSPNET;
    size_t buf = encoder_buf_elems(h, B, H, W);
    buf = std::max(buf, psp ? std::max(px * 512, ppm_term_scratch_floats(B, fh, h->cls_main.Cout)) : px * 1280);
    FS_TRY(ensure_workspace(h, buf, small_elems_for(B)));
    if (!psp || !h->use_fused_head) FS_TRY(ws_grow(h, &h->seg_feat, &h->seg_feat_elems, px * (size_t)h->feat_channels(), false));
    size_t wino = 0;
    if (h->deep_stem) {
        FS_TRY(reserve_conv(h, h->stem[1], B, g.H1, g.W1, s, &wino));
        FS_TRY(reserve_conv(h, h->stem[2], B, g.H1, g.W1, s, &wino));
    }
    int curH = g.H2, curW = g.W2;
    for (const Bottleneck& blk : h->blocks) {
        FS_TRY(reserve_conv(h, blk.c2, B, curH, curW, s, &wino));
        curH = blk.c2.out_size(curH);
        curW = blk.c2.out_size(curW);
    }
    if (psp) {
        FS_TRY(reserve_conv(h, h->use_fused_head ? h->cls_main : h->cls_conv, B, fh, fw, s, &wino));
        FS_TRY(reserve_conv(h, h->cls_conv, B, fh, fw, s, &wino));
    } else {
        for (int i = 1; i < 4; ++i) FS_TRY(reserve_conv(h, h->aspp[i], B, fh, fw, s, &wino));
        FS_TRY(reserve_conv(h, h->head_conv, B, fh, fw, s, &wino));
    }
    return ws_grow(h, &h->wino_ws, &h->wino_ws_elems, wino, false);
}

size_t net_reserved_bytes(fs_handle h) {
    if (!h) return 0;
    return (4 * h->buf_elems + h->small_elems + h->seg_feat_elems + h->wino_ws_elems + h->vit_ws_elems + h->pos_elems + h->bank_elems) * sizeof(float);
}

ConvParams dual_conv_params(const float* a, int ld_a, const float* b, int ld_b, const float* wgt, const float* shift, float* out, int ld_out, int B,
                            int Ho, int Wo, int Cin, int Cin2, int H2, int W2, int stride2, int Cout, int relu) {
    ConvParams p = conv2d_params(a, ld_a, wgt, nullptr, shift, nullptr, 0, out, ld_out, B, Ho, Wo, Cin, Cout, 1, 1, 1, 0, 1, relu, 0);
    p.in2 = b; p.ld_in2 = ld_b; p.Cin2 = Cin2; p.stride2 = stride2; p.H2 = H2; p.W2 = W2;
    return p;
}

ConvParams ppm_z_params(const float* reduced, const float* zw, float* zbuf, int B, int Cr, int Cout9) {
    const int rows = B * 36;
    ConvParams p = gemm_params(reduced, Cr, zw, zbuf, Cout9, rows, Cr, Cout9);
    p.groups = 4;
    p.g_in = (long long)rows * Cr;
    p.g_wgt = (long long)Cout9 * Cr;
    p.g_out = (long long)rows * Cout9;
    return p;
}

int pyramid_pool(fs_net* h, const float* feat, int ld_feat, float* pooled, int B, int H, int W, int C, const int bins[4], hipStream_t s) {
    size_t pool_off[4];
    {
        size_t po = 0;
        for (int i = 0; i < 4; ++i) {
            pool_off[i] = po;
            po += (size_t)B * bins[i] * bins[i] * C;
        }
    }
    const double bytes = 4.0 * B * H * W * C;
    if (H % 6 == 0 && W % 6 == 0 && bins[0] == 1 && bins[1] == 2 && bins[2] == 3 && bins[3] == 6) {
        FS_TRY(prof_begin(h, "ppm.pool6+combine", "adaptive_avgpool", 0, bytes, s));
        FS_TRY(launch_adaptive_avgpool(feat, ld_feat, pooled + pool_off[3], B, H, W, C, 6, s));
        FS_TRY(launch_ppm_pool_combine(pooled + pool_off[3], pooled + pool_off[0], pooled + pool_off[1], pooled + pool_off[2], B, C, s));
        FS_TRY(prof_end(h, s));
        return 0;
    }
    for (int i = 0; i < 4; ++i) {
        FS_TRY(prof_begin(h, "ppm.pool" + std::to_string(bins[i]), "adaptive_avgpool", 0, bytes, s));
        FS_TRY(launch_adaptive_avgpool(feat, ld_feat, pooled + pool_off[i], B, H, W, C, bins[i], s));
        FS_TRY(prof_end(h, s));
    }
    return 0;
}

namespace {
int pyramid_reduce(fs_net* h, const float* feat, int ld_feat, int B, int H, int W, hipStream_t s) {
    float* pooled = h->small;
    float* reduced = h->small + (size_t)B * 50 * 2048;
    FS_TRY(pyramid_pool(h, feat, ld_feat, pooled, B, H, W, 2048, h->bins, s));
    RowdotBatch pb{};
    double flops = 0;
    size_t pool_off = 0;
    for (int i = 0; i < 4; ++i) {
// ... 1 lines not shown
        const ConvBN& c = h->ppm[i];
        pb.p[i] = RowdotProblem{pooled + pool_off, c.w, c.scale, c.shift, reduced + (size_t)i * B * 36 * 512, B * cells};
        pool_off += (size_t)B * cells * 2048;
        flops += 2.0 * B * cells * 2048.0 * 512.0;
    }
    FS_TRY(prof_begin(h, "ppm.features.*.1.weight", "rowdot_1x1", flops, 4.0 * 4 * 2048.0 * 512.0, s));
    FS_TRY(launch_rowdot_1x1_batch(pb, 4, 2048, 512, 2048, 512, 1, s));
    FS_TRY(prof_end(h, s));
    return 0;
}

int encoder_core(fs_handle h, const FrameSrc& src, int B, int H, int W, float* out, float** feat2048, hipStream_t s) {
    const bool fused = out == nullptr;
    const Geometry g = geometry(h, H, W);
    FS_TRY(ensure_workspace(h, encoder_buf_elems(h, B, H, W), small_elems_for(B)));
    const bool psp = h->cfg.arch == FS_ARCH_PSPNET;
    float *X = h->buf[0], *F1 = h->buf[1], *F2 = h->buf[2], *F3 = h->buf[3];

    {
        const ConvBN& c = h->stem[0];
        const StemParams p = stem_params(src, c.w, c.scale, c.shift, X, B, H, W, c.Cout, c.KH, c.KW, c.stride, c.pad, h->use_split);
        const double M = (double)B * g.H1 * g.W1;
        FS_TRY(prof_begin(h, c.name, h->use_split ? "stem_conv_split" : "stem_conv", 2.0 * M * c.Cout * c.KH * c.KW * 3, 4.0 * (B * 3.0 * H * W + M * c.Cout), s));
        FS_TRY(launch_stem_conv(p, s));
        FS_TRY(prof_end(h, s));
    }
    int C = h->stem[0].Cout;
    bool pooled = false;
    if (h->deep_stem) {
        FS_TRY(run_conv(h, h->stem[1], X, C, B, g.H1, g.W1, F1, h->stem[1].Cout, nullptr, 0, s));
        const ConvBN& c = h->stem[2];
        pooled = h->use_fused_pool && c.relu == 1 && c.scale && takes_fused_winograd(h, c, B, g.H1, g.W1, h->stem[1].Cout, c.Cout, false) &&
                 g.H2 == (g.H1 - 1) / 2 + 1 && g.W2 == (g.W1 - 1) / 2 + 1;
        if (pooled) {
            const double tiles = (double)B * cdiv(g.H1, 4) * cdiv(g.W1, 4);
            FS_TRY(prof_begin(h, c.name + "+maxpool", "wino_fused_pool", 2.0 * 36.0 * tiles * c.Cin * c.Cout,
                              4.0 * ((double)B * g.H1 * g.W1 * c.Cin + 2.0 * (double)B * g.H2 * g.W2 * c.Cout + 36.0 * c.Cin * c.Cout), s));
            FS_TRY(launch_wino4_fused_pool(F1, h->stem[1].Cout, c.wf, c.scale, c.shift, X, c.Cout, B, g.H1, g.W1, c.Cin, c.Cout, s));
            FS_TRY(prof_end(h, s));
        } else {
            FS_TRY(run_conv(h, c, F1, h->stem[1].Cout, B, g.H1, g.W1, X, c.Cout, nullptr, 0, s));
        }
        C = c.Cout;
    }
    if (!pooled) {
        const double M = (double)B * g.H2 * g.W2;
        FS_TRY(prof_begin(h, "maxpool", "maxpool3x3s2", 0, 4.0 * ((double)B * g.H1 * g.W1 * C + M * C), s));
        FS_TRY(launch_maxpool3x3s2(X, C, F1, C, B, g.H1, g.W1, C, g.H2, g.W2, s));
        FS_TRY(prof_end(h, s));
        std::swap(X, F1);
    }
    int curH = g.H2, curW = g.W2;
    const int nblocks = (int)h->blocks.size();
    for (int bi = 0; bi < nblocks; ++bi) {
        const Bottleneck& blk = h->blocks[bi];
        const bool last = bi == nblocks - 1;
        const int oH = blk.c2.out_size(curH), oW = blk.c2.out_size(curW);
        FS_TRY(run_conv(h, blk.c1, X, C, B, curH, curW, F1, blk.c1.Cout, nullptr, 0, s));
        FS_TRY(run_conv(h, blk.c2, F1, blk.c1.Cout, B, curH, curW, F2, blk.c2.Cout, nullptr, 0, s));
        const int Cn = blk.c3.Cout;
        float* dst = last ? (fused ? F1 : out) : nullptr;
        const int ld_dst = last && !fused ? h->feat_channels() : Cn;
        ConvBN c3 = blk.c3;
        c3.relu = 1;
        if (blk.has_ds && blk.c3ds.w && h->use_fused_shortcut) {
            if (!dst) dst = F3;
            ConvParams p = dual_conv_params(F2, blk.c2.Cout, X, C, blk.c3ds.w, blk.c3ds.shift, dst, ld_dst, B, oH, oW, blk.c3ds.Cin, blk.ds_cin, curH,
                                            curW, blk.ds_stride, Cn, 1);
            split_use(h, p);
            const double M = (double)B * oH * oW;
            const double fl = 2.0 * M * Cn * (p.Cin + p.Cin2), by = 4.0 * (M * p.Cin + (double)B * curH * curW * p.Cin2 + (double)Cn * (p.Cin + p.Cin2) + M * Cn);
            FS_TRY(run_igemm(h, blk.c3ds.name, p, fl, by, s));
            if (!last) std::swap(X, F3);
        } else if (blk.has_ds) {
            FS_TRY(run_conv(h, blk.ds, X, C, B, curH, curW, F3, Cn, nullptr, 0, s));
            if (!dst) dst = F3;
            FS_TRY(run_conv(h, c3, F2, blk.c2.Cout, B, oH, oW, dst, ld_dst, F3, Cn, s));
            if (!last) std::swap(X, F3);
        } else {
            if (!dst) dst = X;
            FS_TRY(run_conv(h, c3, F2, blk.c2.Cout, B, oH, oW, dst, ld_dst, X, C, s));
        }
        C = Cn;
        curH = oH;
        curW = oW;
    }
    FS_REQUIRE(curH == g.H3 && curW == g.W3 && C == 2048, "encoder geometry mismatch");
    if (fused) {
        *feat2048 = F1;
        out = F1;
    }
    if (!psp) return 0;
    if (fused) return 0;
    FS_TRY(pyramid_reduce(h, out, 4096, B, curH, curW, s));
    float* reduced = h->small + (size_t)B * 50 * 2048;
    for (int i = 0; i < 4; ++i) {
        const int bin = h->bins[i];
        FS_TRY(prof_begin(h, "ppm.up" + std::to_string(bin), "upsample_into", 0, 4.0 * B * curH * curW * 512.0, s));
        FS_TRY(launch_upsample_into(reduced + (size_t)i * B * 36 * 512, bin, bin, out + 2048 + 512 * i, 4096, B, curH, curW, 512, 1, s));
        FS_TRY(prof_end(h, s));
    }
    return 0;
}
}

namespace {
int check_frames(const FrameSrc& f, int B, const char* what) {
    if (f.ncrops) return 0;
    FS_REQUIRE(B >= 1 && f.B1 >= 0 && f.B1 <= B && (f.B1 == 0 || f.in) && (f.B1 == B || f.in2), "%s: bad frame batch (B1=%d of B=%d)", what, f.B1, B);
    return 0;
}
}

int net_encoder(fs_handle h, const FrameSrc& src, int B, int H, int W, float* out, hipStream_t s) {
    FS_REQUIRE(h && h->finalized, "fs_encoder_forward: network not finalized");
    FS_TRY(check_device(h, "fs_encoder_forward"));
    FS_TRY(check_frames(src, B, "fs_encoder_forward"));
    if (h->cfg.arch == FS_ARCH_SEGMENTER) return vit_encoder(h, src, B, H, W, out, s);
    FS_REQUIRE(out && H >= 33 && W >= 33, "fs_encoder_forward: bad arguments (B=%d H=%d W=%d)", B, H, W);
    return encoder_core(h, src, B, H, W, out, nullptr, s);
}

int net_segment(fs_handle h, const FrameSrc& src, int B, int H, int W, float* out_nchw, hipStream_t s) {
    FS_REQUIRE(h && h->finalized, "fs_segment_forward: network not finalized");
    FS_TRY(check_device(h, "fs_segment_forward"));
    FS_REQUIRE(out_nchw && B >= 1 && H >= 1 && W >= 1, "fs_segment_forward: bad arguments (B=%d H=%d W=%d)", B, H, W);
    FS_TRY(check_frames(src, B, "fs_segment_forward"));
    int C = 0, fh = 0, fw = 0;
    if (h->cfg.arch != FS_ARCH_PSPNET || !h->use_fused_head) {
        FS_TRY(net_feature_shape(h, H, W, &C, &fh, &fw));
        const size_t need = h->cfg.arch == FS_ARCH_SEGMENTER ? (size_t)B * (fh * fw + 1) * C : (size_t)B * fh * fw * C;
        FS_TRY(ws_grow(h, &h->seg_feat, &h->seg_feat_elems, need, false));
        FS_TRY(net_encoder(h, src, B, H, W, h->seg_feat, s));
        return net_decoder(h, h->seg_feat, B, fh, fw, out_nchw, s);
    }
    FS_REQUIRE(H >= 33 && W >= 33, "fs_segment_forward: bad arguments (B=%d H=%d W=%d)", B, H, W);
    const Geometry g = geometry(h, H, W);
    fh = g.H3;
    fw = g.W3;
    FS_TRY(ensure_workspace(h, std::max(encoder_buf_elems(h, B, H, W), ppm_term_scratch_floats(B, fh, h->cls_main.Cout)), small_elems_for(B)));
    float* feat = nullptr;
    FS_TRY(encoder_core(h, src, B, H, W, nullptr, &feat, s));
    hipStream_t ps = s;
    FS_TRY(pyramid_reduce(h, feat, 2048, B, fh, fw, ps));
    float *T = nullptr, *R = nullptr;
    for (int i = 0; i < 4; ++i)
        if (h->buf[i] != feat) {
            R = T;
            T = h->buf[i];
        }
    FS_REQUIRE(ppm_term_scratch_floats(B, fh, h->cls_main.Cout) <= h->buf_elems, "fs_segment_forward: workspace too small for the pyramid term");
    const int K = h->cfg.classes, O = h->cls_main.Cout;
    const size_t px = (size_t)B * fh * fw;
    float* reduced = h->small + (size_t)B * 50 * 2048;
    float* zbuf = reduced + (size_t)4 * B * 36 * 512;
    const float* Z[4];
    {
        const ConvBN& z = h->ppm_z[0];
        ConvParams p = ppm_z_params(reduced, z.w, zbuf, B, 512, z.Cout);
        split_use(h, p);
        FS_TRY(run_igemm(h, "decoder.0.weight[:, ppm]", p, 2.0 * B * 50 * 512.0 * z.Cout, 4.0 * (4.0 * z.Cout * 512 + B * 50.0 * (512 + z.Cout)), ps));
        for (int i = 0; i < 4; ++i) Z[i] = zbuf + (size_t)i * p.g_out;
    }
    ConvBN raw = h->cls_main;
    raw.scale = raw.shift = nullptr;
    raw.relu = 0;
    FS_TRY(run_conv(h, raw, feat, 2048, B, fh, fw, T, O, nullptr, 0, s));
    FS_TRY(prof_begin(h, "decoder.0.pyramid_term+decoder.4", "ppm_term_classify", 2.0 * px * O * (24.0 + K), 4.0 * px * O, s));
    FS_TRY(launch_ppm_term_classify(T, O, Z, h->bins, R, h->cls_main.scale, h->cls_main.shift, B, fh, fw, O, 1, h->cls_w, h->cls_b, out_nchw, K, s));
    return prof_end(h, s);
}

int net_decoder(fs_handle h, const float* feat, int B, int fh, int fw, float* out_nchw, hipStream_t s) {
    FS_REQUIRE(h && h->finalized, "fs_decoder_forward: network not finalized");
    FS_TRY(check_device(h, "fs_decoder_forward"));
    if (h->cfg.arch == FS_ARCH_SEGMENTER) return vit_decoder(h, feat, B, fh, fw, out_nchw, s);
    FS_REQUIRE(feat && out_nchw && B >= 1 && fh >= 1 && fw >= 1, "fs_decoder_forward: bad arguments");
    const int K = h->cfg.classes;
    const size_t px = (size_t)B * fh * fw;
    if (h->cfg.arch == FS_ARCH_PSPNET) {
        FS_TRY(ensure_workspace(h, px * 512, small_elems_for(B)));
        float* T = h->buf[0];
        FS_TRY(run_conv(h, h->cls_conv, feat, 4096, B, fh, fw, T, 512, nullptr, 0, s));
        FS_TRY(prof_begin(h, "decoder.4", "classifier_nchw", 2.0 * px * 512.0 * K, 4.0 * px * 512.0, s));
        FS_TRY(launch_classifier_nchw(T, 512, h->cls_w, h->cls_b, out_nchw, B, fh * fw, 512, K, s));
        return prof_end(h, s);
    }
    FS_TRY(ensure_workspace(h, px * 1280, small_elems_for(B)));
    float *cat = h->buf[0], *P = h->buf[1], *Q = h->buf[2];
    for (int i = 0; i < 4; ++i) FS_TRY(run_conv(h, h->aspp[i], feat, 2048, B, fh, fw, cat + 256 * i, 1280, nullptr, 0, s));
    float* pooled = h->small;
    float* reduced = h->small + (size_t)B * 2048;
    FS_TRY(prof_begin(h, "aspp.pool", "adaptive_avgpool", 0, 4.0 * px * 2048.0, s));
    if (fh % 6 == 0 && fw % 6 == 0) {
        float* cells = h->small + (size_t)B * 4096;
        float* spare = cells + (size_t)B * 36 * 2048;
        FS_TRY(launch_adaptive_avgpool(feat, 2048, cells, B, fh, fw, 2048, 6, s));
        FS_TRY(launch_ppm_pool_combine(cells, pooled, spare, spare + (size_t)B * 4 * 2048, B, 2048, s));
    } else {
        FS_TRY(launch_adaptive_avgpool(feat, 2048, pooled, B, fh, fw, 2048, 1, s));
    }
    FS_TRY(prof_end(h, s));
    FS_TRY(prof_begin(h, h->aspp_pool.name, "rowdot_1x1", 2.0 * B * 2048.0 * 256.0, 4.0 * 2048.0 * 256.0, s));
    FS_TRY(launch_rowdot_1x1(pooled, 2048, h->aspp_pool.w, h->aspp_pool.scale, h->aspp_pool.shift, reduced, 256, B, 2048, 256, 1, s));
    FS_TRY(prof_end(h, s));
    FS_TRY(prof_begin(h, "aspp.up", "upsample_into", 0, 4.0 * px * 256.0, s));
    FS_TRY(launch_upsample_into(reduced, 1, 1, cat + 1024, 1280, B, fh, fw, 256, 0, s));
    FS_TRY(prof_end(h, s));
    FS_TRY(run_conv(h, h->project, cat, 1280, B, fh, fw, P, 256, nullptr, 0, s));
    FS_TRY(run_conv(h, h->head_conv, P, 256, B, fh, fw, Q, 256, nullptr, 0, s));
    FS_TRY(prof_begin(h, "classifier.4", "classifier_nchw", 2.0 * px * 256.0 * K, 4.0 * px * 256.0, s));
    FS_TRY(launch_classifier_nchw(Q, 256, h->cls_w, h->cls_b, out_nchw, B, fh * fw, 256, K, s));
    return prof_end(h, s);
}

int net_profile_dump(fs_handle h, char* buf, size_t n) {
    FS_REQUIRE(h && buf && n > 0, "fs_profile_dump: bad arguments");
    FS_HIP(hipDeviceSynchronize());
    size_t off = 0;
    buf[0] = 0;
// ... 15 lines not shown
```

### flood_uav_video_segmentation_amd/csrc/split.h

```cpp
#pragma once
#include "common.h"

namespace fs {

typedef __bf16 bf16x8 __attribute__((ext_vector_type(8)));
typedef __bf16 bf16x2 __attribute__((ext_vector_type(2)));
typedef unsigned u32x4 __attribute__((ext_vector_type(4)));
typedef int i32x4 __attribute__((ext_vector_type(4)));
typedef float f32x16 __attribute__((ext_vector_type(16)));

__device__ __forceinline__ unsigned split_round(float x0, float x1) {
    return __builtin_bit_cast(unsigned, __builtin_convertvector((f32x2){x0, x1}, bf16x2));
}
__device__ __forceinline__ void split_residue(unsigned pk, float& x0, float& x1) {
    x0 -= __builtin_bit_cast(float, pk << 16);
    x1 -= __builtin_bit_cast(float, pk & 0xffff0000u);
}
__device__ __forceinline__ unsigned split_level(float& x0, float& x1) {
    const unsigned pk = split_round(x0, x1);
    split_residue(pk, x0, x1);
    return pk;
}

__device__ __forceinline__ void split_pair(float x0, float x1, unsigned& h, unsigned& m, unsigned& l) {
    h = split_level(x0, x1);
    m = split_level(x0, x1);
    l = split_round(x0, x1);
}

__device__ __forceinline__ void split8(const float (&x)[8], u32x4 (&t)[3]) {
#pragma unroll
    for (int e = 0; e < 4; ++e) {
        unsigned h, m, l;
        split_pair(x[2 * e], x[2 * e + 1], h, m, l);
        t[0][e] = h; t[1][e] = m; t[2][e] = l;
    }
}

__device__ __forceinline__ void split3(float x, unsigned short& h, unsigned short& m, unsigned short& l) {
    unsigned ph, pm, pl;
    split_pair(x, 0.f, ph, pm, pl);
    h = (unsigned short)ph; m = (unsigned short)pm; l = (unsigned short)pl;
}

constexpr int SPLIT_PA[6] = {2, 0, 1, 1, 0, 0}, SPLIT_PB[6] = {0, 2, 1, 0, 1, 0};

__host__ __device__ constexpr int mfma32_row(int e, int h) { return (e & 3) + 8 * (e >> 2) + 4 * h; }

}
```

### flood_uav_video_segmentation_amd/csrc/winograd.hip

```cpp
#include "kernels.h"
#include "split.h"
#include "winograd.h"

namespace fs {

template <int MT>
__global__ __launch_bounds__(256) void winograd_filter_kernel(const float* __restrict__ w, float* __restrict__ U, int O, int I, int chunk_major) {
    constexpr int A = Wino<MT>::A;
    const int64_t total = (int64_t)O * I;
    const int ts = chunk_major ? 32 : 1;
    for (int64_t i = (int64_t)blockIdx.x * 256 + threadIdx.x; i < total; i += (int64_t)gridDim.x * 256) {
        const float* g = chunk_major ? w + (i >> 5) * 288 + (i & 31) : w + i * 9;
        double t[A][3];
#pragma unroll
        for (int s = 0; s < 3; ++s) {
            double col[A];
            Wino<MT>::g(g[(0 * 3 + s) * ts], g[(1 * 3 + s) * ts], g[(2 * 3 + s) * ts], col);
#pragma unroll
            for (int r = 0; r < A; ++r) t[r][s] = col[r];
        }
#pragma unroll
        for (int r = 0; r < A; ++r) {
            double u[A];
            Wino<MT>::g(t[r][0], t[r][1], t[r][2], u);
#pragma unroll
            for (int q = 0; q < A; ++q) U[(size_t)(r * A + q) * total + i] = (float)u[q];
        }
    }
}

int launch_winograd_filter(const float* w_oihw, float* U, int O, int I, int mt, hipStream_t s, int chunk_major) {
    FS_REQUIRE(mt == 3 || mt == 4 || mt == 6, "winograd: tile size must be 3, 4 or 6");
    FS_REQUIRE(!chunk_major || I % 32 == 0, "winograd_filter: a chunk-major bank needs Cin %% 32 == 0");
    const int64_t total = (int64_t)O * I;
    const dim3 grid((unsigned)std::min<int64_t>(cdiv64(total, 256), 65535));
    if (mt == 3) hipLaunchKernelGGL(winograd_filter_kernel<3>, grid, dim3(256), 0, s, w_oihw, U, O, I, chunk_major);
    else if (mt == 4) hipLaunchKernelGGL(winograd_filter_kernel<4>, grid, dim3(256), 0, s, w_oihw, U, O, I, chunk_major);
    else hipLaunchKernelGGL(winograd_filter_kernel<6>, grid, dim3(256), 0, s, w_oihw, U, O, I, chunk_major);
    FS_HIP(hipGetLastError());
    return 0;
}


template <int MT>
__global__ __launch_bounds__((MT + 2) * 32) void winograd_input_kernel(const float* __restrict__ in, int ld_in, float* __restrict__ V, int B, int H,
                                                                       int W, int C4, int th, int tw, int dil, long long s_pos, long long s_tile) {
    constexpr int A = Wino<MT>::A;
    __shared__ f32x4 tmp[A][A][32];
    const unsigned T = (unsigned)(B * dil * dil * th * tw);
    const int cq = threadIdx.x & 31, lane_x = threadIdx.x >> 5;
    const int c4 = blockIdx.x * 32 + cq;
    const bool cok = c4 < C4;
    for (unsigned t = blockIdx.y; t < T; t += gridDim.y) {
        const unsigned tw_u = (unsigned)tw, th_u = (unsigned)th, dd = (unsigned)(dil * dil);
        const unsigned q1 = t / tw_u, q2 = q1 / th_u, q3 = q2 / dd;
        const int tx = (int)(t - q1 * tw_u), ty = (int)(q1 - q2 * th_u), ph = (int)(q2 - q3 * dd), b = (int)q3;
        const int py = ph / dil, px = ph - py * dil;
        const int y0 = py + dil * (ty * MT - 1), x0 = px + dil * (tx * MT - 1);
        {
            const int ix = x0 + dil * lane_x;
            const float* base = in + (size_t)b * H * W * ld_in + (size_t)c4 * 4;
            f32x4 col[A];
#pragma unroll
            for (int y = 0; y < A; ++y) {
                const int iy = y0 + dil * y;
                const bool ok = cok && (unsigned)iy < (unsigned)H && (unsigned)ix < (unsigned)W;
                col[y] = ok ? *reinterpret_cast<const f32x4*>(base + ((size_t)iy * W + ix) * ld_in) : f32x4(0.f);
            }
            f32x4 tc[A];
            Wino<MT>::bt(col, tc);
#pragma unroll
            for (int r = 0; r < A; ++r) tmp[r][lane_x][cq] = tc[r];
        }
        __syncthreads();
        {
            f32x4 row[A], o[A];
#pragma unroll
            for (int x = 0; x < A; ++x) row[x] = tmp[lane_x][x][cq];
            Wino<MT>::bt(row, o);
            if (cok) {
#pragma unroll
                for (int q = 0; q < A; ++q) *reinterpret_cast<f32x4*>(V + (size_t)(lane_x * A + q) * s_pos + (size_t)t * s_tile + (size_t)c4 * 4) = o[q];
            }
        }
        __syncthreads();
    }
}

WinoLayout winograd_layout(int mt, long long T, int C) {
    const long long G = (long long)(mt + 2) * (mt + 2);
    WinoLayout l;
    l.tile_major = T * G * C * 4 < ((long long)1 << 31);
    l.s_pos = l.tile_major ? C : T * C;
    l.s_tile = l.tile_major ? G * C : C;
    return l;
}

int launch_winograd_input(const float* in, int ld_in, float* V, int B, int H, int W, int C, int dil, int mt, hipStream_t s) {
    FS_REQUIRE(C % 4 == 0 && ld_in % 4 == 0 && dil >= 1, "winograd_input: C must be a multiple of 4");
    FS_REQUIRE(mt == 3 || mt == 4 || mt == 6, "winograd: tile size must be 3, 4 or 6");
    FS_REQUIRE(((uintptr_t)in & 15) == 0 && ((uintptr_t)V & 15) == 0, "winograd_input: unaligned operand");
    const int th = (cdiv(H, dil) + mt - 1) / mt, tw = (cdiv(W, dil) + mt - 1) / mt;
    const long long T = (long long)B * dil * dil * th * tw;
    FS_REQUIRE(T < (1ll << 31), "winograd_input: too many tiles");
    const dim3 grid((unsigned)cdiv(C / 4, 32), (unsigned)std::min<long long>(T, 65535));
    const WinoLayout lay = winograd_layout(mt, T, C);
    if (mt == 3) hipLaunchKernelGGL((winograd_input_kernel<3>), grid, dim3(5 * 32), 0, s, in, ld_in, V, B, H, W, C / 4, th, tw, dil, lay.s_pos, lay.s_tile);
    else if (mt == 4) hipLaunchKernelGGL((winograd_input_kernel<4>), grid, dim3(6 * 32), 0, s, in, ld_in, V, B, H, W, C / 4, th, tw, dil, lay.s_pos, lay.s_tile);
    else hipLaunchKernelGGL((winograd_input_kernel<6>), grid, dim3(8 * 32), 0, s, in, ld_in, V, B, H, W, C / 4, th, tw, dil, lay.s_pos, lay.s_tile);
    FS_HIP(hipGetLastError());
    return 0;
}

template <int MT>
__global__ __launch_bounds__((MT + 2) * 32) void winograd_output_kernel(const float* __restrict__ M, const float* __restrict__ scale,
                                                                        const float* __restrict__ shift, float* __restrict__ out, int ld_out, int B,
                                                                        int H, int W, int N4, int th, int tw, int relu, int dil, long long s_pos,
                                                                        long long s_tile, unsigned out_bytes) {
#if defined(__HIP_DEVICE_COMPILE__)
    constexpr int A = Wino<MT>::A;
    __shared__ f32x4 tmp[MT][A][32];
    const unsigned T = (unsigned)(B * dil * dil * th * tw);
    const int oq = threadIdx.x & 31, lane_q = threadIdx.x >> 5;
    const int n4 = blockIdx.x * 32 + oq;
    const bool nok = n4 < N4;
    for (unsigned t = blockIdx.y; t < T; t += gridDim.y) {
        const unsigned tw_u = (unsigned)tw, th_u = (unsigned)th, dd = (unsigned)(dil * dil);
        const unsigned q1 = t / tw_u, q2 = q1 / th_u, q3 = q2 / dd;
        const int tx = (int)(t - q1 * tw_u), ty = (int)(q1 - q2 * th_u), ph = (int)(q2 - q3 * dd), b = (int)q3;
        const int py = ph / dil, px = ph - py * dil;
        {
            f32x4 col[A], y[MT];
#pragma unroll
            for (int r = 0; r < A; ++r)
                col[r] = nok ? *reinterpret_cast<const f32x4*>(M + (size_t)(r * A + lane_q) * s_pos + (size_t)t * s_tile + (size_t)n4 * 4) : f32x4(0.f);
            Wino<MT>::at(col, y);
#pragma unroll
            for (int a = 0; a < MT; ++a) tmp[a][lane_q][oq] = y[a];
        }
        __syncthreads();
        if (lane_q < MT && nok) {
            const int a = lane_q;
            f32x4 row[A], y[MT];
#pragma unroll
            for (int q = 0; q < A; ++q) row[q] = tmp[a][q][oq];
            Wino<MT>::at(row, y);
            const f32x4 sc = scale ? *reinterpret_cast<const f32x4*>(scale + (size_t)n4 * 4) : f32x4(1.f);
            const f32x4 sh = shift ? *reinterpret_cast<const f32x4*>(shift + (size_t)n4 * 4) : f32x4(0.f);
            const int oy = py + dil * (ty * MT + a);
            const __amdgpu_buffer_rsrc_t o_rsrc = __builtin_amdgcn_make_buffer_rsrc((void*)out, 0, out_bytes, 0x00020000);
            const unsigned rowoff = (unsigned)(((b * H + oy) * W) * ld_out + n4 * 4) * 4u;
#pragma unroll
            for (int c = 0; c < MT; ++c) {
                const int ox = px + dil * (tx * MT + c);
                f32x4 v = y[c] * sc + sh;
                if (relu) v = __builtin_elementwise_max(v, f32x4(0.f));
                const unsigned vo = (oy < H && ox < W) ? rowoff + (unsigned)(ox * ld_out) * 4u : 0x80000000u;
                __builtin_amdgcn_raw_buffer_store_b128(__builtin_bit_cast(u32x4, v), o_rsrc, vo, 0, 0);
            }
        }
        __syncthreads();
    }
#endif
}

int launch_winograd_output(const float* M, const float* scale, const float* shift, float* out, int ld_out, int B, int H, int W, int N,
                           int relu, int dil, int mt, hipStream_t s) {
    FS_REQUIRE(N % 4 == 0 && ld_out % 4 == 0 && dil >= 1, "winograd_output: N must be a multiple of 4");
    FS_REQUIRE(mt == 3 || mt == 4 || mt == 6, "winograd: tile size must be 3, 4 or 6");
    FS_REQUIRE(((uintptr_t)M & 15) == 0 && ((uintptr_t)out & 15) == 0 && ((uintptr_t)scale & 15) == 0 && ((uintptr_t)shift & 15) == 0,
               "winograd_output: unaligned operand");
    const int th = (cdiv(H, dil) + mt - 1) / mt, tw = (cdiv(W, dil) + mt - 1) / mt;
    const long long T = (long long)B * dil * dil * th * tw;
    FS_REQUIRE(T < (1ll << 31), "winograd_output: too many tiles");
    const long long out_bytes = ((long long)B * H * W - 1) * ld_out * 4 + (long long)N * 4;
    FS_REQUIRE(out_bytes < (1ll << 31), "winograd_output: output tensor must be smaller than 2 GiB");
    const dim3 grid((unsigned)cdiv(N / 4, 32), (unsigned)std::min<long long>(T, 65535));
    const WinoLayout lay = winograd_layout(mt, T, N);
    if (mt == 3)
        hipLaunchKernelGGL(winograd_output_kernel<3>, grid, dim3(5 * 32), 0, s, M, scale, shift, out, ld_out, B, H, W, N / 4, th, tw, relu, dil,
                           lay.s_pos, lay.s_tile, (unsigned)out_bytes);
    else if (mt == 4)
        hipLaunchKernelGGL(winograd_output_kernel<4>, grid, dim3(6 * 32), 0, s, M, scale, shift, out, ld_out, B, H, W, N / 4, th, tw, relu, dil,
                           lay.s_pos, lay.s_tile, (unsigned)out_bytes);
    else
        hipLaunchKernelGGL(winograd_output_kernel<6>, grid, dim3(8 * 32), 0, s, M, scale, shift, out, ld_out, B, H, W, N / 4, th, tw, relu, dil,
                           lay.s_pos, lay.s_tile, (unsigned)out_bytes);
    FS_HIP(hipGetLastError());
    return 0;
}

}
```

### flood_uav_video_segmentation_amd/model/hipnet.py

```python
import ctypes

import torch
from torch import nn

from .. import _lib, ops
from .._lib import check, one_device, ptr, stream_ptr


HIP_OPTIONS = ("hip_no_winograd", "hip_no_fused_head", "hip_no_fused_shortcut", "hip_no_fused_winograd", "hip_no_split_bf16", "hip_no_res_touch",
               "hip_no_fused_pool", "hip_no_fused_qkv", "hip_winograd_tile")


def check_hip_options(names):
    unknown = sorted(n for n in names if n.startswith("hip_") and n not in HIP_OPTIONS)
    if unknown:
        raise ValueError(f"floodseg: unknown hip option(s) {unknown}; known: {list(HIP_OPTIONS)}")


def hip_options(hparams):
    names = [n for n in dir(hparams) if not n.startswith("__")]
    if hasattr(hparams, "keys"):
        names += [str(k) for k in hparams.keys()]
    check_hip_options(names)
    return dict(no_winograd=bool(getattr(hparams, "hip_no_winograd", False)),
                no_fused_winograd=bool(getattr(hparams, "hip_no_fused_winograd", False)),
                no_split_bf16=bool(getattr(hparams, "hip_no_split_bf16", False)),
                no_res_touch=bool(getattr(hparams, "hip_no_res_touch", False)),
                no_fused_pool=bool(getattr(hparams, "hip_no_fused_pool", False)),
                no_fused_qkv=bool(getattr(hparams, "hip_no_fused_qkv", False)),
                no_fused_head=bool(getattr(hparams, "hip_no_fused_head", False)),
                no_fused_shortcut=bool(getattr(hparams, "hip_no_fused_shortcut", False)),
                winograd_tile=int(getattr(hparams, "hip_winograd_tile", 0)))


class HipNet:
    def __init__(self, arch, layers, classes, patch=0, d_model=0, n_layers=0, dec_layers=0, image_size=0, no_winograd=False,
                 no_fused_head=False, no_fused_shortcut=False, winograd_tile=0, no_fused_winograd=False, no_split_bf16=False,
                 no_res_touch=False, no_fused_pool=False, no_fused_qkv=False):
        self.arch, self.layers, self.classes = arch, int(layers), int(classes)
        self.vit = (int(patch), int(d_model), int(n_layers), int(dec_layers), int(image_size))
        self.flags = ((_lib.OPT_NO_WINOGRAD if no_winograd else 0) | (_lib.OPT_NO_FUSED_HEAD if no_fused_head else 0)
                      | (_lib.OPT_NO_FUSED_SHORTCUT if no_fused_shortcut else 0) | (_lib.OPT_NO_FUSED_WINOGRAD if no_fused_winograd else 0)
                      | (_lib.OPT_NO_SPLIT_BF16 if no_split_bf16 else 0) | (_lib.OPT_NO_RES_TOUCH if no_res_touch else 0)
                      | (_lib.OPT_NO_FUSED_POOL if no_fused_pool else 0) | (_lib.OPT_NO_FUSED_QKV if no_fused_qkv else 0))
        self.winograd_tile = int(winograd_tile)
        self._h = None
        self.ready = False
        self._lib = None
        self.device = None
        self.generation = 0

    def _create(self):
        lib = self._lib = _lib.load()
        cfg = _lib.FsConfig(self.arch, self.layers, self.classes, *self.vit, self.flags, self.winograd_tile)
        h = ctypes.c_void_p()
        check(lib.fs_create(ctypes.byref(cfg), ctypes.byref(h)))
        self._h = h

    def load(self, canonical_state, device=None):
        if not torch.cuda.is_available():
            raise RuntimeError("floodseg: a HIP device is required (there is no CPU fallback for this path)")
        self.close()
        if device is None:
            on_gpu = {t.device for t in canonical_state.values() if t.is_cuda}
            if len(on_gpu) > 1:
                raise RuntimeError(f"floodseg: state_dict tensors live on several devices ({sorted(map(str, on_gpu))})")
            device = on_gpu.pop() if on_gpu else torch.device("cuda", torch.cuda.current_device())
        device = torch.device(device)
        if device.type != "cuda":
            raise RuntimeError(f"floodseg: the network can only live on a HIP device, not {device}")
        if device.index is None:
            device = torch.device("cuda", torch.cuda.current_device())
        with torch.cuda.device(device):
            self._create()
            lib = self._lib
            keep = []
            for name, t in canonical_state.items():
                t = t.detach()
                if t.is_cuda and t.device != device:
                    raise RuntimeError(f"floodseg: weight '{name}' lives on {t.device}, the network on {device}")
                if t.dtype != torch.float32:
                    t = t.float()
                t = t.contiguous()
                keep.append(t)
                shape = (ctypes.c_int64 * max(t.dim(), 1))(*t.shape)
                check(lib.fs_load_weight(self._h, name.encode(), ptr(t), shape, t.dim(), int(t.is_cuda), stream_ptr()))
            torch.cuda.current_stream().synchronize()
            del keep
            check(lib.fs_finalize(self._h, stream_ptr()))
        self.device = device
        self.ready = True
        self.generation += 1

    def close(self):
        if self._h is not None and self._lib is not None:
            if self.device is not None:
                with torch.cuda.device(self.device):
# ... 93 lines not shown
            xs_ = [x.float().contiguous() for x in frames]
            fh_, fw_ = xs_[0].shape[2], xs_[0].shape[3]
            nc = len(crop_yx)
            ch, cw = int(crop_hw[0]), int(crop_hw[1])
            ys = (ctypes.c_int * nc)(*[int(y) for y, _ in crop_yx])
            xs = (ctypes.c_int * nc)(*[int(x) for _, x in crop_yx])
            _, fh, fw = self.feature_shape(ch, cw)
            shape = (nc * len(xs_), self.classes, fh, fw)
            if out is None:
                out = torch.empty(shape, dtype=torch.float32, device=xs_[0].device)
            elif tuple(out.shape) != shape or out.dtype != torch.float32 or not out.is_contiguous() or out.device != xs_[0].device:
                raise RuntimeError(f"floodseg segment_crops: out must be a contiguous fp32 {shape} tensor on {xs_[0].device}")
            check(self._lib.fs_segment_crops(self._h, ptr(xs_[0]), ptr(xs_[1]) if len(xs_) > 1 else None, fh_, fw_, nc, ys, xs, ch, cw,
                                             ptr(out), stream_ptr()))
        return out

    def profile(self, on):
        self._need_ready()
        check(self._lib.fs_profile_enable(self._h, int(on)))

    def profile_dump(self):
        buf = ctypes.create_string_buffer(1 << 20)
        with torch.cuda.device(self.device):
            check(self._lib.fs_profile_dump(self._h, buf, len(buf)))
        rows = []
        for line in buf.value.decode().splitlines():
            name, kernel, flops, nbytes, ms = line.rsplit(" ", 4)
            rows.append((name, kernel, float(flops), float(nbytes), float(ms)))
        return rows


class HipStage(nn.Module):

    def __init__(self, fn=None, what=""):
        super().__init__()
        self._fn = fn
        self._what = what

    def _load_from_state_dict(self, *args, **kwargs):
        return

    def forward(self, x):
        if self._fn is None:
            raise RuntimeError(f"floodseg: '{self._what}' has no standalone forward on the HIP path")
        return self._fn(x)


class HipSegNet(nn.Module):

    ARCH = None

    def __init__(self, hparams):
        super().__init__()
        self._hip_net = HipNet(self.ARCH, hparams.layers, hparams.classes, **hip_options(hparams))
        self.encoder = HipStage(self._hip_net.encode, "encoder")
        self.decoder = HipStage(self._hip_net.decode, "decoder")

    def reserve(self, batch, h, w):
        self._hip_net.reserve(batch, h, w)

    def encode_frames(self, *frames):
        return self._hip_net.encode(*frames)

    @staticmethod
    def canonical_name(key):
        raise NotImplementedError

    def _load_from_state_dict(self, state_dict, prefix, local_metadata, strict, missing_keys, unexpected_keys, error_msgs):
        canon = {}
        for key, t in state_dict.items():
            if not key.startswith(prefix):
                continue
            name = self.canonical_name(key[len(prefix):])
            if name is None:
                continue
            if name in canon:
                continue
            canon[name] = t
        if not canon:
            if strict:
                missing_keys.append(prefix + "<all weights>")
            return
        try:
            self._hip_net.load(canon)
        except RuntimeError as e:
            error_msgs.append(str(e))

    def load_state_dict(self, state_dict, strict=True, assign=False):
        missing, unexpected, errors = [], [], []
        self._load_from_state_dict(dict(state_dict), "", {}, strict, missing, unexpected, errors)
        if errors or (strict and missing):
            raise RuntimeError("Error(s) in loading state_dict for {}:\n\t{}".format(type(self).__name__, "\n\t".join(errors + missing)))
        return torch.nn.modules.module._IncompatibleKeys(missing, unexpected)
```

### include/floodseg.h

```cpp
#ifndef FLOODSEG_H_
#define FLOODSEG_H_

#include <stddef.h>
#include <stdint.h>

#ifdef __cplusplus
extern "C" {
#endif

typedef struct fs_net* fs_handle;
typedef void* fs_stream;

enum { FS_ARCH_PSPNET = 0, FS_ARCH_DEEPLABV3 = 1, FS_ARCH_SEGMENTER = 2 };

typedef struct fs_config {
    int arch;
    int layers;
    int classes;
    int patch;
    int d_model;
    int n_layers;
    int dec_layers;
    int image_size;
    int flags;
    int winograd_tile;
} fs_config;

enum {
    FS_OPT_NO_WINOGRAD = 1,
    FS_OPT_NO_FUSED_HEAD = 2,
    FS_OPT_NO_FUSED_SHORTCUT = 4,
    FS_OPT_NO_FUSED_WINOGRAD = 8,
    FS_OPT_NO_SPLIT_BF16 = 16,
    FS_OPT_NO_FUSED_POOL = 256,
    FS_OPT_NO_RES_TOUCH = 128,
    FS_OPT_NO_FUSED_QKV = 1024
};

int fs_version(void);
const char* fs_last_error(void);

int fs_create(const fs_config* cfg, fs_handle* out);
int fs_destroy(fs_handle h);
int fs_load_weight(fs_handle h, const char* name, const float* data, const int64_t* shape, int ndim, int on_device,
                   fs_stream stream);
int fs_finalize(fs_handle h, fs_stream stream);
int fs_feature_shape(fs_handle h, int H, int W, int* C, int* fh, int* fw);
size_t fs_workspace_bytes(fs_handle h, int B, int H, int W);
int fs_reserve(fs_handle h, int B, int H, int W, fs_stream stream);
size_t fs_reserved_bytes(fs_handle h);

int fs_encoder_forward(fs_handle h, const float* in_nchw, int B, int H, int W, float* out_nhwc, fs_stream stream);
int fs_decoder_forward(fs_handle h, const float* feat_nhwc, int B, int fh, int fw, float* out_nchw, fs_stream stream);
int fs_segment_forward(fs_handle h, const float* in_nchw, int B, int H, int W, float* out_nchw, fs_stream stream);
int fs_encoder_forward2(fs_handle h, const float* in_a, int Ba, const float* in_b, int Bb, int H, int W, float* out_nhwc,
                        fs_stream stream);
int fs_segment_forward2(fs_handle h, const float* in_a, int Ba, const float* in_b, int Bb, int H, int W, float* out_nchw,
                        fs_stream stream);

int fs_segment_crops(fs_handle h, const float* frame_a, const float* frame_b, int FH, int FW, int ncrops, const int* crop_y,
                     const int* crop_x, int ch, int cw, float* out_nchw, fs_stream stream);

int fs_profile_enable(fs_handle h, int on);
int fs_profile_dump(fs_handle h, char* buf, size_t buflen);

int fs_grid_sample_nchw(const float* in, int B, int C, int Hi, int Wi, const float* grid, int Hg, int Wg, float* out,
                        int align_corners, fs_stream stream);
int fs_grid_sample_nhwc(const float* in, int ld_in, int B, int C, int Hi, int Wi, const float* grid, int Hg, int Wg,
                        float* out, int ld_out, int align_corners, fs_stream stream);
int fs_resize_bilinear_nchw(const float* in, int BC, int Hi, int Wi, float* out, int Ho, int Wo, int align_corners,
                            fs_stream stream);
int fs_resize_bilinear_nhwc(const float* in, int ld_in, int B, int C, int Hi, int Wi, float* out, int ld_out, int Ho,
                            int Wo, int align_corners, fs_stream stream);
int fs_blend(const float* a, float wa, const float* b, float wb, float* out, int64_t numel, fs_stream stream);

int fs_seg_tail(const float* lo_prev, const float* lo_next, const float* const* grids_left,
                const float* const* grids_right, int K, int h, int w, int Hg, int Wg, int H, int W, int n, int no_warp,
                float* out_logits, uint8_t* out_mask, float* scratch, fs_stream stream);

int fs_feat_tail(const float* f_prev, const float* f_next, int C, int fh, int fw, const float* const* grids_left,
                 const float* const* grids_right, int Hg, int Wg, const float* grid0, int H0, int W0, int n, int no_warp, float* stack,
                 float* scratch, fs_stream stream);

int fs_seg_tail_accumulate(const float* lo_prev, const float* lo_next, const float* const* grids_left,
                           const float* const* grids_right, int K, int h, int w, int Hg, int Wg, int H, int W, int n, int no_warp,
                           double* canvas, double* count, int cH, int cW, int y0, int x0, float* scratch, fs_stream stream);

int fs_argmax_u8(const float* in, int B, int K, int64_t HW, uint8_t* out, fs_stream stream);
// ... 33 lines not shown
```

Measured before the change: 1249.

## Add two-plane fp16 split Winograd path with per-filter scaling and amax

Adds a Winograd convolution route that splits the transformed inputs and filters into high and low fp16 planes with per-filter power-of-two scales and activation amax tracking. The batched GEMM then runs on fp16 MFMA instructions using three cross terms in place of the previous split-bf16/f32 path, while the output transform rescales the result. The intent is higher matrix throughput from fp16 MFMA while keeping near-f32 accuracy. It adds amax reduction and scaling work, extra kernels and a new option flag to disable it, and carries a risk of accuracy or range problems.

```diff
diff --git a/flood_uav_video_segmentation_amd/_lib.py b/flood_uav_video_segmentation_amd/_lib.py
--- a/flood_uav_video_segmentation_amd/_lib.py
+++ b/flood_uav_video_segmentation_amd/_lib.py
@@ -29,6 +29,7 @@
 OPT_NO_RES_TOUCH = 128
 OPT_NO_FUSED_POOL = 256
 OPT_NO_FUSED_QKV = 1024
+OPT_NO_WINO_F16X2 = 2048
 CONV_CHUNK_MAJOR = 0x400
 
 _SIGNATURES = {
@@ -184,6 +185,15 @@
 ]
 EXT8_MAGIC = 0x4653455854414238
 
+_EXT9_HOOKS = [
+    ("winograd_f16x2_workspace_floats", ctypes.c_size_t, [c_int] * 7),
+    ("conv3x3_winograd_f16x2_nhwc", c_int, [c_void, c_int] + [c_void] * 5 + [c_int] * 11 + [c_void, c_void]),
+    ("winograd_input_f16x2", c_int, [c_void, c_int, c_void, c_void] + [c_int] * 6 + [c_void]),
+    ("conv1x1_split_amax", c_int, [c_void, c_int] + [c_void] * 4 + [c_int, c_void] + [c_int] * 8 + [c_void, c_void]),
+    ("mfma_f16_probe", c_int, [c_void] * 4),
+]
+EXT9_MAGIC = 0x4653455854414239
+
 
 class FsTestApi(ctypes.Structure):
     _fields_ = [("size", ctypes.c_size_t)] + [(name, ctypes.CFUNCTYPE(res, *args)) for name, res, args in _HOOKS]
@@ -251,6 +261,14 @@
 
 class FsHookTables8(ctypes.Structure):
     _fields_ = [("base7", FsHookTables7), ("ext8", FsExt8Api)]
+
+
+class FsExt9Api(ctypes.Structure):
+    _fields_ = [("magic", ctypes.c_uint64), ("size", ctypes.c_size_t)] + [(name, ctypes.CFUNCTYPE(res, *args)) for name, res, args in _EXT9_HOOKS]
+
+
+class FsHookTables9(ctypes.Structure):
+    _fields_ = [("base8", FsHookTables8), ("ext9", FsExt9Api)]
 
 
 class _Library:
@@ -266,8 +284,33 @@
         self._ext6 = None
         self._ext7 = None
         self._ext8 = None
+        self._ext9 = None
 
     def __getattr__(self, name):
+        if name.startswith("fs_") and any(name == "fs_" + h[0] for h in _EXT9_HOOKS):
+            if self._ext9 is None:
+                all8 = ctypes.cast(self._cdll.fs_test_hooks(), ctypes.POINTER(FsHookTables8)).contents
+                all5 = all8.base7.base6.base5
+                all2 = all5.base4.base3.base2
+                if (all2.base.test.size != ctypes.sizeof(FsTestApi) or all2.base.ext.magic != EXT_MAGIC or all2.base.ext.size != ctypes.sizeof(FsExtApi)
+                        or all2.ext2.magic != EXT2_MAGIC or all2.ext2.size != ctypes.sizeof(FsExt2Api)
+                        or all5.base4.base3.ext3.magic != EXT3_MAGIC or all5.base4.base3.ext3.size != ctypes.sizeof(FsExt3Api)
+                        or all5.base4.ext4.magic != EXT4_MAGIC or all5.base4.ext4.size != ctypes.sizeof(FsExt4Api)
+                        or all5.ext5.magic != EXT5_MAGIC or all5.ext5.size != ctypes.sizeof(FsExt5Api)
+                        or all8.base7.base6.ext6.magic != EXT6_MAGIC or all8.base7.base6.ext6.size != ctypes.sizeof(FsExt6Api)
+                        or all8.base7.ext7.magic != EXT7_MAGIC or all8.base7.ext7.size != ctypes.sizeof(FsExt7Api)
+                        or all8.ext8.magic != EXT8_MAGIC or all8.ext8.size != ctypes.sizeof(FsExt8Api)):
+                    raise RuntimeError(f"floodseg: the library's first nine hook tables are not the ones this binding knows ({name} is missing)")
+                ext9 = ctypes.cast(self._cdll.fs_test_hooks(), ctypes.POINTER(FsHookTables9)).contents.ext9
+                if ext9.magic != EXT9_MAGIC:
+                    raise RuntimeError(f"floodseg: the library has no ninth extension table ({name} is missing)")
+                self._ext9 = ext9
+            member = getattr(FsExt9Api, name[3:])
+            if self._ext9.size < member.offset + member.size:
+                raise RuntimeError(f"floodseg: the library's ninth extension table is older than this binding ({name} is missing)")
+            fn = getattr(self._ext9, name[3:])
+            setattr(self, name, fn)
+            return fn
         if name.startswith("fs_") and any(name == "fs_" + h[0] for h in _EXT8_HOOKS):
             if self._ext8 is None:
                 all7 = ctypes.cast(self._cdll.fs_test_hooks(), ctypes.POINTER(FsHookTables7)).contents
@@ -485,6 +528,10 @@
     return [h[0] for h in _EXT8_HOOKS]
 
 
+def ext9_hook_names():
+    return [h[0] for h in _EXT9_HOOKS]
+
+
 def check(rc):
     if rc != 0:
         msg = load().fs_last_error()
diff --git a/flood_uav_video_segmentation_amd/csrc/conv_igemm.hip b/flood_uav_video_segmentation_amd/csrc/conv_igemm.hip
--- a/flood_uav_video_segmentation_amd/csrc/conv_igemm.hip
+++ b/flood_uav_video_segmentation_amd/csrc/conv_igemm.hip
@@ -26,7 +26,7 @@
     }
 }
 
-template <int BM, int BN, int WGM, int WGN, bool DUAL, bool SPLIT>
+template <int BM, int BN, int WGM, int WGN, bool DUAL, bool SPLIT, bool AMAX = false>
 __device__ __forceinline__ void conv_tile(ConvParams p, const int m0, const int n0, float* __restrict__ lds) {
 #if defined(__HIP_DEVICE_COMPILE__)
     constexpr int BK = 32;
@@ -331,18 +331,18 @@
         }
     }
     if (!DUAL && p.res) {
-        if (p.relu == 1) igemm_epilogue<1, true>(acc, rv, sc_n, sh_n, p, M, em_base, en_base);
-        else if (p.relu == 2) igemm_epilogue<2, true>(acc, rv, sc_n, sh_n, p, M, em_base, en_base);
-        else igemm_epilogue<0, true>(acc, rv, sc_n, sh_n, p, M, em_base, en_base);
+        if (p.relu == 1) igemm_epilogue<1, true, AMAX>(acc, rv, sc_n, sh_n, p, M, em_base, en_base);
+        else if (p.relu == 2) igemm_epilogue<2, true, AMAX>(acc, rv, sc_n, sh_n, p, M, em_base, en_base);
+        else igemm_epilogue<0, true, AMAX>(acc, rv, sc_n, sh_n, p, M, em_base, en_base);
     } else {
-        if (p.relu == 1) igemm_epilogue<1, false>(acc, rv, sc_n, sh_n, p, M, em_base, en_base);
-        else if (p.relu == 2) igemm_epilogue<2, false>(acc, rv, sc_n, sh_n, p, M, em_base, en_base);
-        else igemm_epilogue<0, false>(acc, rv, sc_n, sh_n, p, M, em_base, en_base);
+        if (p.relu == 1) igemm_epilogue<1, false, AMAX>(acc, rv, sc_n, sh_n, p, M, em_base, en_base);
+        else if (p.relu == 2) igemm_epilogue<2, false, AMAX>(acc, rv, sc_n, sh_n, p, M, em_base, en_base);
+        else igemm_epilogue<0, false, AMAX>(acc, rv, sc_n, sh_n, p, M, em_base, en_base);
     }
 #endif
 }
 
-template <int BM, int BN, int WGM = 2, int WGN = 2, bool DUAL = false, bool SPLIT = false>
+template <int BM, int BN, int WGM = 2, int WGN = 2, bool DUAL = false, bool SPLIT = false, bool AMAX = false>
 __global__ __launch_bounds__(64 * WGM * WGN) void conv_igemm_dma_f32(ConvParams p, int tiles_m, int tiles_n) {
 #if defined(__HIP_DEVICE_COMPILE__)
     constexpr int PM = 8;
@@ -362,7 +362,120 @@
     if (SPLIT) p.wgt3 = (const char*)p.wgt3 + (long long)grp * p.g_wgt * 2;
     p.out += (long long)grp * p.g_out;
     p.kv_b = grp;
-    conv_tile<BM, BN, WGM, WGN, DUAL, SPLIT>(p, m0, n0, lds);
+    conv_tile<BM, BN, WGM, WGN, DUAL, SPLIT, AMAX>(p, m0, n0, lds);
+#endif
+}
+
+template <int BM, int BN, int WGM, int WGN>
+__global__ __launch_bounds__(256) void conv_igemm_dma_f32_planes(ConvParams p, int tiles_m, int tiles_n) {
+#if defined(__HIP_DEVICE_COMPILE__)
+    static_assert(WGM * WGN == 4, "four waves");
+    constexpr int PM = 8;
+    constexpr int GA = BM / 16, GB = BN / 16;
+    constexpr int NG = 2 * (GA + GB);
+    constexpr int NJ = NG / 4;
+    static_assert(GA % 4 == 0 && GB % 4 == 0, "every plane is a whole number of four-wave passes");
+    constexpr int STAGE = NG * 256;
+    constexpr int WM = BM / WGM, WN = BN / WGN, TM = WM / 32, TN = WN / 32;
+    static_assert(WM % 32 == 0 && WN % 32 == 0, "whole 32 x 32 MFMA blocks per wave");
+    __shared__ __attribute__((aligned(1024))) float lds[2 * STAGE];
+    const int nblk = gridDim.x, bid = blockIdx.x;
+    const int q = nblk >> 3, rr = nblk & 7, xcd = bid & 7;
+    const int lid = (xcd < rr ? xcd * (q + 1) : rr * (q + 1) + (xcd - rr) * q) + (bid >> 3);
+    const int per_group = tiles_m * tiles_n;
+    const int grp = lid / per_group;
+    const int lig = lid - grp * per_group;
+    const int panel = lig / (PM * tiles_n);
+    const int within = lig - panel * (PM * tiles_n);
+    const int prow = min(PM, tiles_m - panel * PM);
+    const int m0 = (panel * PM + within % prow) * BM, n0 = (within / prow) * BN;
+    p.out += (long long)grp * p.g_out;
+
+    const int t = threadIdx.x, lane = t & 63, wv = t >> 6;
+    const int wm = wv / WGN, wn = wv % WGN, l31 = lane & 31, hh = lane >> 5;
+    const int wv_u = __builtin_amdgcn_readfirstlane(wv);
+    const int M = p.B * p.Ho * p.Wo, K = p.Cin, nchunks = K >> 5;
+    const int ldw = p.ld_wgt ? p.ld_wgt : K;
+    constexpr unsigned SENT = 0x80000000u;
+    const __amdgpu_buffer_rsrc_t a_rsrc = __builtin_amdgcn_make_buffer_rsrc(
+        (void*)((const char*)p.a16 + (long long)grp * p.g_in * 2), 0, p.a_plane_bytes + (unsigned)((((long long)M - 1) * p.ld_in + K) * 2), 0x00020000);
+    const __amdgpu_buffer_rsrc_t b_rsrc = __builtin_amdgcn_make_buffer_rsrc(
+        (void*)((const char*)p.w16 + (long long)grp * p.g_wgt * 2), 0, p.w_plane_bytes + (unsigned)((((long long)p.Cout - 1) * ldw + K) * 2), 0x00020000);
+    unsigned voff[NJ];
+#pragma unroll
+    for (int j = 0; j < NJ; ++j) {
+        const bool isa = 4 * j < 2 * GA;
+        const int g = isa ? (4 * j) % GA + wv : (4 * j - 2 * GA) % GB + wv;
+        const int row = 16 * g + (lane >> 2);
+        const unsigned piece = (unsigned)(((lane & 3) ^ ((row >> 2) & 3)) * 16);
+        if (isa) voff[j] = m0 + row < M ? (unsigned)((m0 + row) * p.ld_in * 2) + piece : SENT;
+        else voff[j] = n0 + row < p.Cout ? (unsigned)((n0 + row) * ldw * 2) + piece : SENT;
+    }
+    f32x16 acc[TM][TN];
+#pragma unroll
+    for (int i = 0; i < TM; ++i)
+#pragma unroll
+        for (int j = 0; j < TN; ++j)
+#pragma unroll
+            for (int e = 0; e < 16; ++e) acc[i][j][e] = 0.f;
+
+    unsigned k_soff = 0;
+#define FS_PL_DMA(STG)                                                                                            \
+    {                                                                                                             \
+        _Pragma("unroll") for (int j = 0; j < NJ; ++j) {                                                          \
+            const bool isa = 4 * j < 2 * GA;                                                                      \
+            const int pl = isa ? (4 * j) / GA : (4 * j - 2 * GA) / GB;                                            \
+            __builtin_amdgcn_raw_ptr_buffer_load_lds(isa ? a_rsrc : b_rsrc,                                       \
+                (__attribute__((address_space(3))) void*)(lds + (STG) * STAGE + (4 * j + wv_u) * 256), 16, voff[j], \
+                k_soff + (unsigned)pl * (isa ? p.a_plane_bytes : p.w_plane_bytes), 0, 0);                         \
+        }                                                                                                         \
+        k_soff += 64;                                                                                             \
+    }
+#define FS_PL_READ(STG, S_, A_, B_)                                                                               \
+    {                                                                                                             \
+        const float* a_src = lds + (STG) * STAGE;                                                                 \
+        const float* b_src = a_src + 2 * GA * 256;                                                                \
+        const int slot = (2 * (S_) + hh) ^ ((l31 >> 2) & 3);                                                      \
+        _Pragma("unroll") for (int pl = 0; pl < 2; ++pl) {                                                        \
+            _Pragma("unroll") for (int i = 0; i < TM; ++i)                                                        \
+                A_[i][pl] = __builtin_bit_cast(f16x8, *reinterpret_cast<const u32x4*>(&a_src[pl * GA * 256 + (wm * WM + i * 32 + l31) * 16 + 4 * slot])); \
+            _Pragma("unroll") for (int j = 0; j < TN; ++j)                                                        \
+                B_[j][pl] = __builtin_bit_cast(f16x8, *reinterpret_cast<const u32x4*>(&b_src[pl * GB * 256 + (wn * WN + j * 32 + l31) * 16 + 4 * slot])); \
+        }                                                                                                         \
+    }
+#define FS_PL_MMA(A_, B_)                                                                                         \
+    _Pragma("unroll") for (int term = 0; term < 3; ++term)                                                        \
+        _Pragma("unroll") for (int i = 0; i < TM; ++i)                                                            \
+            _Pragma("unroll") for (int j = 0; j < TN; ++j)                                                        \
+                acc[i][j] = __builtin_amdgcn_mfma_f32_32x32x16_f16(A_[i][SPLIT16_PA[term]], B_[j][SPLIT16_PB[term]], acc[i][j], 0, 0, 0);
+
+    FS_PL_DMA(0)
+    FS_DMA_PUBLISH()
+    if (nchunks > 1) FS_PL_DMA(1)
+    f16x8 A0[TM][2], B0[TN][2], A1[TM][2], B1[TN][2];
+    FS_PL_READ(0, 0, A0, B0)
+    int cur = 0;
+    for (int kc = 0; kc < nchunks; ++kc) {
+        FS_PL_READ(cur, 1, A1, B1)
+        __builtin_amdgcn_sched_barrier(0);
+        FS_PL_MMA(A0, B0)
+        __builtin_amdgcn_sched_barrier(0);
+        FS_DMA_PUBLISH()
+        if (kc + 2 < nchunks) FS_PL_DMA(cur)
+        __builtin_amdgcn_sched_barrier(0);
+        FS_PL_READ(cur ^ 1, 0, A0, B0)
+        __builtin_amdgcn_sched_barrier(0);
+        FS_PL_MMA(A1, B1)
+        __builtin_amdgcn_sched_barrier(0);
+        cur ^= 1;
+    }
+#undef FS_PL_DMA
+#undef FS_PL_READ
+#undef FS_PL_MMA
+    float rv[TM][TN][16], sc_n[TN], sh_n[TN];
+#pragma unroll
+    for (int j = 0; j < TN; ++j) { sc_n[j] = 1.f; sh_n[j] = 0.f; }
+    igemm_epilogue<0, false>(acc, rv, sc_n, sh_n, p, M, m0 + wm * WM + 4 * hh, n0 + wn * WN + l31);
 #endif
 }
 
@@ -377,9 +490,9 @@
     const double eff[7] = {0, 1.00, 0.92, 0.80, 0.92, 0, 0.97};
     int best = 1;
     double best_t = 1e300;
-    const int last = p.in2 ? 2 : p.wgt3 ? 3 : 4;
+    const int last = p.in2 ? 2 : (p.wgt3 || p.a16) ? 3 : 4;
     for (int c = 1; c <= 6; ++c) {
-        if (c > last && !(c == 6 && p.wgt3 && !p.in2 && p.Cout % 96 == 0)) continue;
+        if (c > last && !(c == 6 && p.wgt3 && !p.in2 && !p.amax && !p.a16 && p.Cout % 96 == 0)) continue;
         const int bm = kTiles[c].bm, bn = kTiles[c].bn;
         if (p.Cout < bn && bn > 64) continue;
         const long tiles = (long)cdiv(M, bm) * cdiv(p.Cout, bn) * (p.groups > 1 ? p.groups : 1);
@@ -394,6 +507,7 @@
 const char* conv_igemm_tile_name(const ConvParams& p, int tile) {
     if (!tile_id_ok(tile)) return "(bad tile)";
     if (tile == 0) tile = pick_tile(p);
+    if (p.a16) return tile == 1 ? "splitf16_128x128" : tile == 2 ? "splitf16_128x64" : tile == 4 ? "splitf16_64x128" : "splitf16_64x64";
     if (p.in2 && p.wgt3) return tile == 2 ? "split128x64cat" : "split128x128cat";
     if (p.in2) return tile == 2 ? "igemm128x64cat" : "igemm128x128cat";
     if (p.wgt3) return tile == 1 ? "split128x128" : tile == 2 ? "split128x64" : tile == 4 ? "split64x128" : tile == 6 ? "split128x96" : "split64x64";
@@ -448,7 +562,67 @@
 }
 }
 
+namespace {
+__global__ __launch_bounds__(64) void mfma_f16_probe_kernel(const unsigned short* __restrict__ a, const unsigned short* __restrict__ b, float* __restrict__ out) {
+#if defined(__HIP_DEVICE_COMPILE__)
+    const int lane = threadIdx.x, l31 = lane & 31, hh = lane >> 5;
+    const f16x8 av = __builtin_bit_cast(f16x8, *reinterpret_cast<const u32x4*>(a + l31 * 16 + 8 * hh));
+    const f16x8 bv = __builtin_bit_cast(f16x8, *reinterpret_cast<const u32x4*>(b + l31 * 16 + 8 * hh));
+    f32x16 acc;
+#pragma unroll
+    for (int e = 0; e < 16; ++e) acc[e] = 0.f;
+    acc = __builtin_amdgcn_mfma_f32_32x32x16_f16(av, bv, acc, 0, 0, 0);
+#pragma unroll
+    for (int e = 0; e < 16; ++e) out[mfma32_row(e, hh) * 32 + l31] = acc[e];
+#endif
+}
+}
+
+int launch_mfma_f16_probe(const void* a, const void* b, float* out, hipStream_t s) {
+    FS_REQUIRE(a && b && out && (((uintptr_t)a | (uintptr_t)b) & 15) == 0, "mfma_f16_probe: bad arguments");
+    hipLaunchKernelGGL(mfma_f16_probe_kernel, dim3(1), dim3(64), 0, s, (const unsigned short*)a, (const unsigned short*)b, out);
+    FS_HIP(hipGetLastError());
+    return 0;
+}
+
+namespace {
+int launch_conv_igemm_planes(const ConvParams& p, hipStream_t s, int tile) {
+    const int M = p.B * p.Ho * p.Wo, K = p.Cin, groups = p.groups > 1 ? p.groups : 1;
+    const long long ldw = p.ld_wgt ? p.ld_wgt : K;
+    FS_REQUIRE(p.w16 && p.out && !p.in2 && !p.res && !p.scale && !p.shift && !p.relu && !p.amax && !p.kv_k && p.KH == 1 && p.KW == 1 && p.stride == 1 &&
+                   p.pad == 0 && p.Ho == p.H && p.Wo == p.W, "conv_igemm: the two-fp16-plane route takes a plain or grouped 1x1 GEMM without an epilogue");
+    FS_REQUIRE(M >= 1 && p.Cout >= 1 && K >= 32 && K % 32 == 0 && p.ld_in % 8 == 0 && p.ld_in >= K && ldw % 8 == 0 && ldw >= K && p.ld_out >= p.Cout,
+               "conv_igemm: bad plane GEMM geometry (M=%d K=%d N=%d ld_in=%d)", M, K, p.Cout, p.ld_in);
+    FS_REQUIRE((((uintptr_t)p.a16 | (uintptr_t)p.w16) & 15) == 0 && p.a_plane_bytes % 16 == 0 && p.w_plane_bytes % 16 == 0 && ((uintptr_t)p.out & 3) == 0 &&
+                   (p.g_in * 2) % 16 == 0 && (p.g_wgt * 2) % 16 == 0,
+               "conv_igemm: unaligned operand planes");
+    FS_REQUIRE((int64_t)2 * p.a_plane_bytes < (int64_t)1 << 31 && (int64_t)2 * p.w_plane_bytes < (int64_t)1 << 31 &&
+                   ((int64_t)(groups - 1) * p.g_in + ((int64_t)M - 1) * p.ld_in + K) * 2 <= (int64_t)p.a_plane_bytes &&
+                   ((int64_t)(groups - 1) * p.g_wgt + ((int64_t)p.Cout - 1) * ldw + K) * 2 <= (int64_t)p.w_plane_bytes,
+               "conv_igemm: the operands' rows exceed their planes (plane bytes %u / %u)", p.a_plane_bytes, p.w_plane_bytes);
+    FS_REQUIRE(((int64_t)(groups - 1) * p.g_out + (int64_t)M * p.ld_out) * 4 < (int64_t)1 << 31, "conv_igemm: output tensor must be smaller than 2 GiB");
+    if (tile == 0) tile = pick_tile(p);
+    const int bm = kTiles[tile].bm, bn = kTiles[tile].bn;
+    const int tm = cdiv(M, bm), tn = cdiv(p.Cout, bn);
+    const dim3 grid(tm * tn * groups), block(256);
+    switch (tile) {
+        case 1: hipLaunchKernelGGL((conv_igemm_dma_f32_planes<128, 128, 2, 2>), grid, block, 0, s, p, tm, tn); break;
+        case 2: hipLaunchKernelGGL((conv_igemm_dma_f32_planes<128, 64, 2, 2>), grid, block, 0, s, p, tm, tn); break;
+        case 3: hipLaunchKernelGGL((conv_igemm_dma_f32_planes<64, 64, 2, 2>), grid, block, 0, s, p, tm, tn); break;
+        case 4: hipLaunchKernelGGL((conv_igemm_dma_f32_planes<64, 128, 2, 2>), grid, block, 0, s, p, tm, tn); break;
+        default: return fail("conv_igemm: the two-fp16-plane route has tiles 1 to 4");
+    }
+    FS_HIP(hipGetLastError());
+    return 0;
+}
+}
+
 int launch_conv_igemm(const ConvParams& p, hipStream_t s, int tile) {
+    if (p.a16) {
+        FS_REQUIRE(tile_id_ok(tile), "conv_igemm: tile %d is not 0..4 or 6", tile);
+        return launch_conv_igemm_planes(p, s, tile);
+    }
+    FS_REQUIRE(!p.amax || (p.wgt3 && !p.in2), "conv_igemm: the amax slot exists on the split-operand route without a second operand");
     FS_TRY(check_conv_params(p));
     FS_REQUIRE(tile_id_ok(tile), "conv_igemm: tile %d is not 0..4 or 6", tile);
     if (tile == 0) tile = pick_tile(p);
@@ -487,6 +661,19 @@
         FS_HIP(hipGetLastError());
         return 0;
     }
+    if (p.wgt3 && p.amax) {
+        FS_REQUIRE(p.Ho * p.Wo >= 128 && groups == 1 && !p.kv_k && ((uintptr_t)p.amax & 3) == 0,
+                   "conv_igemm: the amax slot needs maps of at least 128 pixels and a plain launch (%d x %d, %d groups)", p.Ho, p.Wo, groups);
+        switch (tile) {
+            case 1: hipLaunchKernelGGL((conv_igemm_dma_f32<128, 128, 4, 1, false, true, true>), grid, block, 0, s, p, tm, tn); break;
+            case 2: hipLaunchKernelGGL((conv_igemm_dma_f32<128, 64, 4, 1, false, true, true>), grid, block, 0, s, p, tm, tn); break;
+            case 3: hipLaunchKernelGGL((conv_igemm_dma_f32<64, 64, 2, 2, false, true, true>), grid, block, 0, s, p, tm, tn); break;
+            case 4: hipLaunchKernelGGL((conv_igemm_dma_f32<64, 128, 2, 2, false, true, true>), grid, block, 0, s, p, tm, tn); break;
+            default: return fail("conv_igemm: the amax slot exists on tiles 1 to 4");
+        }
+        FS_HIP(hipGetLastError());
+        return 0;
+    }
     if (p.wgt3) {
         switch (tile) {
             case 1: hipLaunchKernelGGL((conv_igemm_dma_f32<128, 128, 4, 1, false, true>), grid, block, 0, s, p, tm, tn); break;
diff --git a/flood_uav_video_segmentation_amd/csrc/igemm_epilogue.h b/flood_uav_video_segmentation_amd/csrc/igemm_epilogue.h
--- a/flood_uav_video_segmentation_amd/csrc/igemm_epilogue.h
+++ b/flood_uav_video_segmentation_amd/csrc/igemm_epilogue.h
@@ -39,12 +39,17 @@
     return copysignf(1.f - __builtin_amdgcn_exp2f(-(q * a)), x);
 }
 
-template <int ACT, bool RES, int TM, int TN>
+template <int ACT, bool RES, bool AMAX = false, int TM, int TN>
 __device__ __forceinline__ void igemm_epilogue(const f32x16 (&acc)[TM][TN], const float (&rv)[TM][TN][16], const float (&sc)[TN],
                                                const float (&sh)[TN], const ConvParams& p, int M, int m_base, int n_base) {
     constexpr unsigned SENT = 0x80000000u;
     const __amdgpu_buffer_rsrc_t o_rsrc = __builtin_amdgcn_make_buffer_rsrc((void*)p.out, 0, (unsigned)((long long)M * p.ld_out * 4), 0x00020000);
     const unsigned row_o = (unsigned)p.ld_out * 4u;
+    const int hw = p.Ho * p.Wo;
+    const int row0 = m_base & ~127;
+    const int img0 = AMAX ? row0 / hw : 0;
+    const int edge = AMAX ? min((img0 + 1) * hw, M) : 0;
+    int mx0 = 0, mx1 = 0;
 #pragma unroll
     for (int j = 0; j < TN; ++j) {
         const int n = n_base + j * 32;
@@ -60,7 +65,24 @@
                 if (ACT == 1) v = fmaxf(v, 0.f);
                 else if (ACT == 2) v = 0.5f * v * (1.f + gelu_erf(v * 0.70710678118654752f));
                 __builtin_amdgcn_raw_buffer_store_b32(__builtin_bit_cast(unsigned, v), o_rsrc, vo + (unsigned)mfma32_row(e, 0) * row_o, 0, 0);
+                if (AMAX) {
+                    const int m = mb + mfma32_row(e, 0);
+                    const int bits = nok ? (int)(__builtin_bit_cast(unsigned, v) & 0x7fffffffu) : 0;
+                    mx0 = max(mx0, m < edge ? bits : 0);
+                    mx1 = max(mx1, (m >= edge && m < M) ? bits : 0);
+                }
             }
+        }
+    }
+    if (AMAX) {
+#pragma unroll
+        for (int d = 32; d >= 1; d >>= 1) {
+            mx0 = max(mx0, __shfl_xor(mx0, d, 64));
+            mx1 = max(mx1, __shfl_xor(mx1, d, 64));
+        }
+        if ((threadIdx.x & 63) == 0) {
+            if (mx0 > 0) atomicMax(p.amax + img0, mx0);
+            if (mx1 > 0) atomicMax(p.amax + img0 + 1, mx1);
         }
     }
 }
diff --git a/flood_uav_video_segmentation_amd/csrc/kernels.h b/flood_uav_video_segmentation_amd/csrc/kernels.h
--- a/flood_uav_video_segmentation_amd/csrc/kernels.h
+++ b/flood_uav_video_segmentation_amd/csrc/kernels.h
@@ -28,9 +28,14 @@
     int kv_N, kv_Npad, kv_heads;
     unsigned kv_plane_bytes;
     int kv_b;
+    int* amax;
+    const void* a16;
+    const void* w16;
+    unsigned a_plane_bytes, w_plane_bytes;
 };
 int launch_conv_igemm(const ConvParams& p, hipStream_t s, int tile = 0);
 const char* conv_igemm_tile_name(const ConvParams& p, int tile = 0);
+int launch_mfma_f16_probe(const void* a, const void* b, float* out, hipStream_t s);
 int launch_split_bf16x3(const float* w, long long n, void* planes, hipStream_t s);
 
 static inline int conv_out_size(int in, int k, int stride, int pad, int dil) { return (in + 2 * pad - dil * (k - 1) - 1) / stride + 1; }
@@ -302,6 +307,17 @@
                           hipStream_t s);
 int launch_winograd_output(const float* M , const float* scale, const float* shift, float* out, int ld_out, int B,
                            int H, int W, int N, int relu, int dil, int mt, hipStream_t s);
+int launch_winograd_input_f16x2(const float* in, int ld_in, const int* amax, void* V16, int B, int H, int W, int C, int dil, int mt, hipStream_t s);
+int launch_winograd_filter_f16x2(const float* U, void* U16, float* uscale, int O, int I, int mt, hipStream_t s);
+int launch_winograd_output_f16x2(const float* M, const int* amax, const float* uscale, const float* scale, const float* shift, float* out, int ld_out,
+                                 int B, int H, int W, int N, int relu, int dil, int mt, hipStream_t s);
+__host__ __device__ static inline int wino16_exponent(int amax_bits, int mt) {
+    const int e = (amax_bits >> 23) & 0xff;
+    if (amax_bits == 0) return 0;
+    const int k = (e - 126) + (mt == 6 ? 8 : mt == 4 ? 7 : 6) - 15;
+    return k < -126 ? -126 : k > 126 ? 126 : k;
+}
+__host__ __device__ static inline float pow2f(int k) { union { int i; float f; } u; u.i = (k + 127) << 23; return u.f; }
 struct WinoLayout { bool tile_major; long long s_pos, s_tile; };
 WinoLayout winograd_layout(int mt, long long T, int C);
 static inline ConvParams winograd_gemm_params(const float* V, const float* U, float* M, int mt, int T, int Cin, int Cout) {
diff --git a/flood_uav_video_segmentation_amd/csrc/net.h b/flood_uav_video_segmentation_amd/csrc/net.h
--- a/flood_uav_video_segmentation_amd/csrc/net.h
+++ b/flood_uav_video_segmentation_amd/csrc/net.h
@@ -25,6 +25,8 @@
     float* U3 = nullptr;
     hipEvent_t ready[3] = {nullptr, nullptr, nullptr};
     hipStream_t built_on[3] = {nullptr, nullptr, nullptr};
+    void* planes16[3] = {nullptr, nullptr, nullptr};
+    float* uscale[3] = {nullptr, nullptr, nullptr};
 };
 
 struct ConvBN {
@@ -120,6 +122,10 @@
     bool use_split = true;
     bool use_fused_qkv = true;
     bool use_fused_pool = true;
+    bool use_wino_f16 = true;
+    int* amax = nullptr;
+    size_t amax_elems = 0;
+    const int* head_amax = nullptr;
     bool res_touch = true;
     std::map<const float*, std::pair<void*, size_t>> split_banks;
     int device = 0;
@@ -171,6 +177,10 @@
 int conv_winograd(fs_net* h, const std::string& name, const float* in, int ld_in, const float* U, const void* U3, unsigned plane_bytes, float* V,
                   float* M, const float* scale, const float* shift, float* out, int ld_out, int B, int H, int W, int Cin, int Cout, int dil,
                   int relu, int mt, hipStream_t s);
+int conv_winograd_f16x2(fs_net* h, const std::string& name, const float* in, int ld_in, const int* amax, const void* U16, const float* uscale, void* V16,
+                        float* M, const float* scale, const float* shift, float* out, int ld_out, int B, int H, int W, int Cin, int Cout, int dil,
+                        int relu, int mt, hipStream_t s, int tile = 0);
+bool wino_f16x2_fits(int mt, long long T, int Cin, int Cout);
 int vit_reserve(fs_handle h, int B, int H, int W, hipStream_t s);
 int fetch(fs_net* h, const std::string& name, const RawTensor** out);
 int prof_begin(fs_net* h, const std::string& name, const char* kernel, double flops, double bytes, hipStream_t s);
diff --git a/flood_uav_video_segmentation_amd/csrc/net.hip b/flood_uav_video_segmentation_amd/csrc/net.hip
--- a/flood_uav_video_segmentation_amd/csrc/net.hip
+++ b/flood_uav_video_segmentation_amd/csrc/net.hip
@@ -90,6 +90,15 @@
         FS_TRY(dev_alloc(h, &bank, elems));
         FS_TRY(launch_winograd_filter(c.w, bank, c.Cout, c.Cin, mt, s, 1));
         FS_TRY(split_attach(h, bank, elems, s));
+        if (h->use_wino_f16) {
+            float *planes = nullptr, *us = nullptr;
+            FS_TRY(dev_alloc(h, &planes, elems));
+            FS_TRY(dev_alloc(h, &us, (size_t)c.Cout));
+            FS_TRY(launch_winograd_filter_f16x2(bank, planes, us, c.Cout, c.Cin, mt, s));
+            c.wino->planes16[k] = planes;
+            c.wino->uscale[k] = us;
+            h->bank_elems += elems + (size_t)c.Cout;
+        }
         hipEvent_t ev = nullptr;
         FS_HIP(hipEventCreateWithFlags(&ev, hipEventDisableTiming));
         FS_HIP(hipEventRecord(ev, s));
@@ -213,10 +222,35 @@
     return prof_end(h, s);
 }
 
+bool wino_f16x2_fits(int mt, long long T, int Cin, int Cout) {
+    const long long G = (long long)(mt + 2) * (mt + 2);
+    return Cin % 32 == 0 && G * T * Cin * 4 < (1ll << 31) && G * Cout * Cin * 4 < (1ll << 31);
+}
+
+int conv_winograd_f16x2(fs_net* h, const std::string& name, const float* in, int ld_in, const int* amax, const void* U16, const float* uscale, void* V16,
+                        float* M, const float* scale, const float* shift, float* out, int ld_out, int B, int H, int W, int Cin, int Cout, int dil,
+                        int relu, int mt, hipStream_t s, int tile) {
+    const int T = winograd_tiles(B, H, W, dil, mt);
+    FS_REQUIRE(wino_f16x2_fits(mt, T, Cin, Cout), "winograd f16x2: %d tiles x %d -> %d channels exceed the 2 GiB of a plane pair", T, Cin, Cout);
+    ConvParams p = winograd_gemm_params(nullptr, nullptr, M, mt, T, Cin, Cout);
+    const double G = p.groups, v_elems = G * T * Cin, m_elems = G * T * Cout, px = (double)B * H * W;
+    p.a16 = V16;
+    p.a_plane_bytes = (unsigned)(v_elems * 2);
+    p.w16 = U16;
+    p.w_plane_bytes = (unsigned)(G * Cout * Cin * 2);
+    FS_TRY(prof_begin(h, name + ".wino_in", "winograd_input", 0, 4.0 * (px * Cin + v_elems), s));
+    FS_TRY(launch_winograd_input_f16x2(in, ld_in, amax, V16, B, H, W, Cin, dil, mt, s));
+    FS_TRY(prof_end(h, s));
+    FS_TRY(run_igemm(h, name + ".wino_gemm", p, 2.0 * G * (double)T * Cin * Cout, 4.0 * (v_elems + G * Cout * Cin + m_elems), s, tile));
+    FS_TRY(prof_begin(h, name + ".wino_out", "winograd_output", 0, 4.0 * (m_elems + px * Cout), s));
+    FS_TRY(launch_winograd_output_f16x2(M, amax, uscale, scale, shift, out, ld_out, B, H, W, Cout, relu, dil, mt, s));
+    return prof_end(h, s);
+}
+
 namespace {
 
 int run_conv_winograd(fs_net* h, const ConvBN& c, const float* in, int ld_in, int B, int H, int W, float* out, int ld_out,
-                      hipStream_t s) {
+                      hipStream_t s, const int* amax) {
     const int mt = wino_m(h->wino_force_m, H, W, c.dil);
     const size_t T = (size_t)winograd_tiles(B, H, W, c.dil, mt);
     const float* U = nullptr;
@@ -224,6 +258,12 @@
     FS_TRY(ws_grow(h, &h->wino_ws, &h->wino_ws_elems, wino_vm_floats(mt, T, c.Cin, c.Cout, 8), false));
     float* V = h->wino_ws;
     float* M = h->wino_ws + wino_v_floats(mt, T, c.Cin, 8);
+    if (amax) {
+        const int k = mt == 6 ? 1 : mt == 3 ? 2 : 0;
+        FS_REQUIRE(c.wino->planes16[k], "winograd f16x2: conv '%s' has no fp16 planes", c.name.c_str());
+        return conv_winograd_f16x2(h, c.name, in, ld_in, amax, c.wino->planes16[k], c.wino->uscale[k], V, M, c.scale, c.shift, out, ld_out, B, H, W,
+                                   c.Cin, c.Cout, c.dil, c.relu, mt, s);
+    }
     ConvParams bank = winograd_gemm_params(V, U, M, mt, (int)T, c.Cin, c.Cout);
     split_use(h, bank);
     return conv_winograd(h, c.name, in, ld_in, U, bank.wgt3, bank.plane_bytes, V, M, c.scale, c.shift, out, ld_out, B, H, W, c.Cin, c.Cout,
@@ -239,6 +279,12 @@
     return wino_rows < (c.dil <= 4 ? 0.8 : 0.7) * direct_rows;
 }
 
+bool takes_wino_f16x2(const fs_net* h, const ConvBN& c, int B, int H, int W) {
+    if (!h->use_wino_f16 || !takes_winograd(h, c, B, H, W, false) || H * W < 128) return false;
+    const int mt = wino_m(h->wino_force_m, H, W, c.dil);
+    return wino_f16x2_fits(mt, winograd_tiles(B, H, W, c.dil, mt), c.Cin, c.Cout);
+}
+
 int reserve_conv(fs_net* h, const ConvBN& c, int B, int H, int W, hipStream_t s, size_t* need) {
     if (!takes_winograd(h, c, B, H, W, false)) return 0;
     const int mt = wino_m(h->wino_force_m, H, W, c.dil);
@@ -262,9 +308,14 @@
 }
 
 int run_conv(fs_net* h, const ConvBN& c, const float* in, int ld_in, int B, int H, int W, float* out, int ld_out,
-             const float* res, int ld_res, hipStream_t s) {
-    if (takes_winograd(h, c, B, H, W, res != nullptr)) return run_conv_winograd(h, c, in, ld_in, B, H, W, out, ld_out, s);
+             const float* res, int ld_res, hipStream_t s, const int* amax_in = nullptr, int* amax_out = nullptr) {
+    if (takes_winograd(h, c, B, H, W, res != nullptr)) {
+        FS_REQUIRE(!amax_out, "conv '%s': a Winograd launch publishes no amax", c.name.c_str());
+        return run_conv_winograd(h, c, in, ld_in, B, H, W, out, ld_out, s, amax_in);
+    }
+    FS_REQUIRE(!amax_in, "conv '%s': amax slots handed to a conv that is not on the three-launch Winograd route", c.name.c_str());
     if (takes_fused_winograd(h, c, B, H, W, ld_in, ld_out, res != nullptr)) {
+        FS_REQUIRE(!amax_out, "conv '%s': the one-kernel Winograd publishes no amax", c.name.c_str());
         const double tiles = (double)B * cdiv(H, 4) * cdiv(W, 4);
         FS_TRY(prof_begin(h, c.name, "wino_fused", 2.0 * 36.0 * tiles * c.Cin * c.Cout,
                           4.0 * ((double)B * H * W * (c.Cin + c.Cout) + 36.0 * c.Cin * c.Cout), s));
@@ -272,6 +323,8 @@
         return prof_end(h, s);
     }
     ConvParams p = conv_params(h, c, in, ld_in, B, H, W, out, ld_out, res, ld_res);
+    FS_REQUIRE(!amax_out || p.wgt3, "conv '%s': the amax epilogue needs the split-operand route", c.name.c_str());
+    p.amax = amax_out;
     const double M = (double)B * p.Ho * p.Wo;
     const double flops = 2.0 * M * c.Cout * c.KH * c.KW * c.Cin;
     const double bytes = 4.0 * ((double)B * H * W * c.Cin + (double)c.Cout * c.KH * c.KW * c.Cin + M * c.Cout * (res ? 2 : 1));
@@ -325,7 +378,7 @@
     const int max_classes = cfg->arch == FS_ARCH_PSPNET ? 32 : 64;
     FS_REQUIRE(cfg->classes >= 1 && cfg->classes <= max_classes, "fs_create: classes out of range (%d; this arch takes 1..%d)", cfg->classes, max_classes);
     FS_REQUIRE((cfg->flags & ~(FS_OPT_NO_WINOGRAD | FS_OPT_NO_FUSED_HEAD | FS_OPT_NO_FUSED_SHORTCUT | FS_OPT_NO_FUSED_WINOGRAD | FS_OPT_NO_SPLIT_BF16 |
-                               FS_OPT_NO_RES_TOUCH | FS_OPT_NO_FUSED_POOL | FS_OPT_NO_FUSED_QKV)) == 0,
+                               FS_OPT_NO_RES_TOUCH | FS_OPT_NO_FUSED_POOL | FS_OPT_NO_FUSED_QKV | FS_OPT_NO_WINO_F16X2)) == 0,
                "fs_create: unknown option bits 0x%x", cfg->flags);
     FS_REQUIRE(cfg->winograd_tile == 0 || cfg->winograd_tile == 3 || cfg->winograd_tile == 4 || cfg->winograd_tile == 6,
                "fs_create: winograd_tile must be 0, 3, 4 or 6");
@@ -340,6 +393,7 @@
     h->res_touch = !(cfg->flags & FS_OPT_NO_RES_TOUCH);
     h->use_fused_pool = !(cfg->flags & FS_OPT_NO_FUSED_POOL);
     h->use_fused_qkv = h->use_split && !(cfg->flags & FS_OPT_NO_FUSED_QKV);
+    h->use_wino_f16 = h->use_split && h->use_winograd && !(cfg->flags & FS_OPT_NO_WINO_F16X2);
     if (hipGetDevice(&h->device) != hipSuccess) {
         delete h;
         return fail("fs_create: no HIP device");
@@ -368,6 +422,7 @@
     if (h->vit_ws) (void)hipFree(h->vit_ws);
     if (h->seg_feat) (void)hipFree(h->seg_feat);
     if (h->wino_ws) (void)hipFree(h->wino_ws);
+    if (h->amax) (void)hipFree(h->amax);
     if (h->pos_cur) (void)hipFree(h->pos_cur);
     for (hipEvent_t e : h->bank_events) (void)hipEventDestroy(e);
     for (auto& r : h->prof) {
@@ -593,12 +648,13 @@
         for (int i = 1; i < 4; ++i) FS_TRY(reserve_conv(h, h->aspp[i], B, fh, fw, s, &wino));
         FS_TRY(reserve_conv(h, h->head_conv, B, fh, fw, s, &wino));
     }
+    if (h->use_wino_f16) FS_TRY(ws_grow(h, reinterpret_cast<float**>(&h->amax), &h->amax_elems, (h->blocks.size() + 1) * (size_t)B, false));
     return ws_grow(h, &h->wino_ws, &h->wino_ws_elems, wino, false);
 }
 
 size_t net_reserved_bytes(fs_handle h) {
     if (!h) return 0;
-    return (4 * h->buf_elems + h->small_elems + h->seg_feat_elems + h->wino_ws_elems + h->vit_ws_elems + h->pos_elems + h->bank_elems) * sizeof(float);
+    return (4 * h->buf_elems + h->small_elems + h->seg_feat_elems + h->wino_ws_elems + h->amax_elems + h->vit_ws_elems + h->pos_elems + h->bank_elems) * sizeof(float);
 }
 
 ConvParams dual_conv_params(const float* a, int ld_a, const float* b, int ld_b, const float* wgt, const float* shift, float* out, int ld_out, int B,
@@ -706,12 +762,22 @@
     }
     int curH = g.H2, curW = g.W2;
     const int nblocks = (int)h->blocks.size();
+    h->head_amax = nullptr;
+    if (h->use_wino_f16) {
+        FS_TRY(ws_grow(h, reinterpret_cast<float**>(&h->amax), &h->amax_elems, (size_t)(nblocks + 1) * B, false));
+        FS_HIP(hipMemsetAsync(h->amax, 0, (size_t)(nblocks + 1) * B * sizeof(int), s));
+    }
     for (int bi = 0; bi < nblocks; ++bi) {
         const Bottleneck& blk = h->blocks[bi];
         const bool last = bi == nblocks - 1;
         const int oH = blk.c2.out_size(curH), oW = blk.c2.out_size(curW);
-        FS_TRY(run_conv(h, blk.c1, X, C, B, curH, curW, F1, blk.c1.Cout, nullptr, 0, s));
-        FS_TRY(run_conv(h, blk.c2, F1, blk.c1.Cout, B, curH, curW, F2, blk.c2.Cout, nullptr, 0, s));
+        int* const a12 = takes_wino_f16x2(h, blk.c2, B, curH, curW) && !takes_winograd(h, blk.c1, B, curH, curW, false) &&
+                                 !takes_fused_winograd(h, blk.c1, B, curH, curW, C, blk.c1.Cout, false) && blk.c1.Cin % 32 == 0
+                             ? h->amax + (size_t)bi * B : nullptr;
+        int* const a_head = last && fused && psp && !blk.has_ds && takes_wino_f16x2(h, h->cls_main, B, oH, oW) && blk.c3.Cin % 32 == 0 && blk.c3.KH == 1
+                                ? h->amax + (size_t)nblocks * B : nullptr;
+        FS_TRY(run_conv(h, blk.c1, X, C, B, curH, curW, F1, blk.c1.Cout, nullptr, 0, s, nullptr, a12));
+        FS_TRY(run_conv(h, blk.c2, F1, blk.c1.Cout, B, curH, curW, F2, blk.c2.Cout, nullptr, 0, s, a12));
         const int Cn = blk.c3.Cout;
         float* dst = last ? (fused ? F1 : out) : nullptr;
         const int ld_dst = last && !fused ? h->feat_channels() : Cn;
@@ -733,7 +799,8 @@
             if (!last) std::swap(X, F3);
         } else {
             if (!dst) dst = X;
-            FS_TRY(run_conv(h, c3, F2, blk.c2.Cout, B, oH, oW, dst, ld_dst, X, C, s));
+            FS_TRY(run_conv(h, c3, F2, blk.c2.Cout, B, oH, oW, dst, ld_dst, X, C, s, nullptr, a_head));
+            h->head_amax = a_head;
         }
         C = Cn;
         curH = oH;
@@ -819,7 +886,7 @@
     ConvBN raw = h->cls_main;
     raw.scale = raw.shift = nullptr;
     raw.relu = 0;
-    FS_TRY(run_conv(h, raw, feat, 2048, B, fh, fw, T, O, nullptr, 0, s));
+    FS_TRY(run_conv(h, raw, feat, 2048, B, fh, fw, T, O, nullptr, 0, s, h->head_amax));
     FS_TRY(prof_begin(h, "decoder.0.pyramid_term+decoder.4", "ppm_term_classify", 2.0 * px * O * (24.0 + K), 4.0 * px * O, s));
     FS_TRY(launch_ppm_term_classify(T, O, Z, h->bins, R, h->cls_main.scale, h->cls_main.shift, B, fh, fw, O, 1, h->cls_w, h->cls_b, out_nchw, K, s));
     return prof_end(h, s);
diff --git a/flood_uav_video_segmentation_amd/csrc/split.h b/flood_uav_video_segmentation_amd/csrc/split.h
--- a/flood_uav_video_segmentation_amd/csrc/split.h
+++ b/flood_uav_video_segmentation_amd/csrc/split.h
@@ -6,6 +6,7 @@
 typedef __bf16 bf16x8 __attribute__((ext_vector_type(8)));
 typedef __bf16 bf16x2 __attribute__((ext_vector_type(2)));
 typedef unsigned u32x4 __attribute__((ext_vector_type(4)));
+typedef unsigned u32x2 __attribute__((ext_vector_type(2)));
 typedef int i32x4 __attribute__((ext_vector_type(4)));
 typedef float f32x16 __attribute__((ext_vector_type(16)));
 
@@ -45,6 +46,24 @@
 
 constexpr int SPLIT_PA[6] = {2, 0, 1, 1, 0, 0}, SPLIT_PB[6] = {0, 2, 1, 0, 1, 0};
 
+typedef _Float16 f16x8 __attribute__((ext_vector_type(8)));
+typedef _Float16 f16x2 __attribute__((ext_vector_type(2)));
+
+__device__ __forceinline__ unsigned split16_round(float x0, float x1) {
+    return __builtin_bit_cast(unsigned, __builtin_convertvector((f32x2){x0, x1}, f16x2));
+}
+__device__ __forceinline__ void split16_residue(unsigned pk, float& x0, float& x1) {
+    const f32x2 r = __builtin_convertvector(__builtin_bit_cast(f16x2, pk), f32x2);
+    x0 -= r[0];
+    x1 -= r[1];
+}
+__device__ __forceinline__ void split16_pair(float x0, float x1, unsigned& h, unsigned& m) {
+    h = split16_round(x0, x1);
+    split16_residue(h, x0, x1);
+    m = split16_round(x0, x1);
+}
+constexpr int SPLIT16_PA[3] = {1, 0, 0}, SPLIT16_PB[3] = {0, 1, 0};
+
 __host__ __device__ constexpr int mfma32_row(int e, int h) { return (e & 3) + 8 * (e >> 2) + 4 * h; }
 
 }
diff --git a/flood_uav_video_segmentation_amd/csrc/winograd.hip b/flood_uav_video_segmentation_amd/csrc/winograd.hip
--- a/flood_uav_video_segmentation_amd/csrc/winograd.hip
+++ b/flood_uav_video_segmentation_amd/csrc/winograd.hip
@@ -42,9 +42,10 @@
 }
 
 
-template <int MT>
+template <int MT, bool F16 = false>
 __global__ __launch_bounds__((MT + 2) * 32) void winograd_input_kernel(const float* __restrict__ in, int ld_in, float* __restrict__ V, int B, int H,
-                                                                       int W, int C4, int th, int tw, int dil, long long s_pos, long long s_tile) {
+                                                                       int W, int C4, int th, int tw, int dil, long long s_pos, long long s_tile,
+                                                                       const int* __restrict__ amax = nullptr, long long plane_elems = 0) {
     constexpr int A = Wino<MT>::A;
     __shared__ f32x4 tmp[A][A][32];
     const unsigned T = (unsigned)(B * dil * dil * th * tw);
@@ -78,7 +79,20 @@
 #pragma unroll
             for (int x = 0; x < A; ++x) row[x] = tmp[lane_x][x][cq];
             Wino<MT>::bt(row, o);
-            if (cok) {
+            if (cok && F16) {
+                const float sinv = pow2f(-wino16_exponent(amax[b], MT));
+                unsigned short* Vh = reinterpret_cast<unsigned short*>(V);
+#pragma unroll
+                for (int q = 0; q < A; ++q) {
+                    unsigned h0, m0, h1, m1;
+                    split16_pair(o[q][0] * sinv, o[q][1] * sinv, h0, m0);
+                    split16_pair(o[q][2] * sinv, o[q][3] * sinv, h1, m1);
+                    const u32x2 h = {h0, h1}, m = {m0, m1};
+                    const size_t at = (size_t)(lane_x * A + q) * s_pos + (size_t)t * s_tile + (size_t)c4 * 4;
+                    *reinterpret_cast<u32x2*>(Vh + at) = h;
+                    *reinterpret_cast<u32x2*>(Vh + plane_elems + at) = m;
+                }
+            } else if (cok) {
 #pragma unroll
                 for (int q = 0; q < A; ++q) *reinterpret_cast<f32x4*>(V + (size_t)(lane_x * A + q) * s_pos + (size_t)t * s_tile + (size_t)c4 * 4) = o[q];
             }
@@ -96,7 +110,18 @@
     return l;
 }
 
+namespace {
+int winograd_input_any(const float* in, int ld_in, float* V, const int* amax, int B, int H, int W, int C, int dil, int mt, hipStream_t s);
+}
 int launch_winograd_input(const float* in, int ld_in, float* V, int B, int H, int W, int C, int dil, int mt, hipStream_t s) {
+    return winograd_input_any(in, ld_in, V, nullptr, B, H, W, C, dil, mt, s);
+}
+int launch_winograd_input_f16x2(const float* in, int ld_in, const int* amax, void* V16, int B, int H, int W, int C, int dil, int mt, hipStream_t s) {
+    FS_REQUIRE(amax && ((uintptr_t)amax & 3) == 0, "winograd_input_f16x2: no amax slots");
+    return winograd_input_any(in, ld_in, static_cast<float*>(V16), amax, B, H, W, C, dil, mt, s);
+}
+namespace {
+int winograd_input_any(const float* in, int ld_in, float* V, const int* amax, int B, int H, int W, int C, int dil, int mt, hipStream_t s) {
     FS_REQUIRE(C % 4 == 0 && ld_in % 4 == 0 && dil >= 1, "winograd_input: C must be a multiple of 4");
     FS_REQUIRE(mt == 3 || mt == 4 || mt == 6, "winograd: tile size must be 3, 4 or 6");
     FS_REQUIRE(((uintptr_t)in & 15) == 0 && ((uintptr_t)V & 15) == 0, "winograd_input: unaligned operand");
@@ -105,18 +130,25 @@
     FS_REQUIRE(T < (1ll << 31), "winograd_input: too many tiles");
     const dim3 grid((unsigned)cdiv(C / 4, 32), (unsigned)std::min<long long>(T, 65535));
     const WinoLayout lay = winograd_layout(mt, T, C);
-    if (mt == 3) hipLaunchKernelGGL((winograd_input_kernel<3>), grid, dim3(5 * 32), 0, s, in, ld_in, V, B, H, W, C / 4, th, tw, dil, lay.s_pos, lay.s_tile);
-    else if (mt == 4) hipLaunchKernelGGL((winograd_input_kernel<4>), grid, dim3(6 * 32), 0, s, in, ld_in, V, B, H, W, C / 4, th, tw, dil, lay.s_pos, lay.s_tile);
-    else hipLaunchKernelGGL((winograd_input_kernel<6>), grid, dim3(8 * 32), 0, s, in, ld_in, V, B, H, W, C / 4, th, tw, dil, lay.s_pos, lay.s_tile);
-    FS_HIP(hipGetLastError());
-    return 0;
-}
-
-template <int MT>
+    const long long pe = (long long)(mt + 2) * (mt + 2) * T * C;
+    const int* const none = nullptr;
+    if (amax && mt == 3) hipLaunchKernelGGL((winograd_input_kernel<3, true>), grid, dim3(5 * 32), 0, s, in, ld_in, V, B, H, W, C / 4, th, tw, dil, lay.s_pos, lay.s_tile, amax, pe);
+    else if (amax && mt == 4) hipLaunchKernelGGL((winograd_input_kernel<4, true>), grid, dim3(6 * 32), 0, s, in, ld_in, V, B, H, W, C / 4, th, tw, dil, lay.s_pos, lay.s_tile, amax, pe);
+    else if (amax) hipLaunchKernelGGL((winograd_input_kernel<6, true>), grid, dim3(8 * 32), 0, s, in, ld_in, V, B, H, W, C / 4, th, tw, dil, lay.s_pos, lay.s_tile, amax, pe);
+    else if (mt == 3) hipLaunchKernelGGL((winograd_input_kernel<3>), grid, dim3(5 * 32), 0, s, in, ld_in, V, B, H, W, C / 4, th, tw, dil, lay.s_pos, lay.s_tile, none, 0ll);
+    else if (mt == 4) hipLaunchKernelGGL((winograd_input_kernel<4>), grid, dim3(6 * 32), 0, s, in, ld_in, V, B, H, W, C / 4, th, tw, dil, lay.s_pos, lay.s_tile, none, 0ll);
+    else hipLaunchKernelGGL((winograd_input_kernel<6>), grid, dim3(8 * 32), 0, s, in, ld_in, V, B, H, W, C / 4, th, tw, dil, lay.s_pos, lay.s_tile, none, 0ll);
+    FS_HIP(hipGetLastError());
+    return 0;
+}
+}
+
+template <int MT, bool F16 = false>
 __global__ __launch_bounds__((MT + 2) * 32) void winograd_output_kernel(const float* __restrict__ M, const float* __restrict__ scale,
                                                                         const float* __restrict__ shift, float* __restrict__ out, int ld_out, int B,
                                                                         int H, int W, int N4, int th, int tw, int relu, int dil, long long s_pos,
-                                                                        long long s_tile, unsigned out_bytes) {
+                                                                        long long s_tile, unsigned out_bytes, const int* __restrict__ amax = nullptr,
+                                                                        const float* __restrict__ uscale = nullptr) {
 #if defined(__HIP_DEVICE_COMPILE__)
     constexpr int A = Wino<MT>::A;
     __shared__ f32x4 tmp[MT][A][32];
@@ -147,6 +179,12 @@
             Wino<MT>::at(row, y);
             const f32x4 sc = scale ? *reinterpret_cast<const f32x4*>(scale + (size_t)n4 * 4) : f32x4(1.f);
             const f32x4 sh = shift ? *reinterpret_cast<const f32x4*>(shift + (size_t)n4 * 4) : f32x4(0.f);
+            if (F16) {
+                const float sb = pow2f(wino16_exponent(amax[b], MT));
+                const f32x4 us = *reinterpret_cast<const f32x4*>(uscale + (size_t)n4 * 4);
+#pragma unroll
+                for (int c = 0; c < MT; ++c) y[c] = y[c] * sb * us;
+            }
             const int oy = py + dil * (ty * MT + a);
             const __amdgpu_buffer_rsrc_t o_rsrc = __builtin_amdgcn_make_buffer_rsrc((void*)out, 0, out_bytes, 0x00020000);
             const unsigned rowoff = (unsigned)(((b * H + oy) * W) * ld_out + n4 * 4) * 4u;
@@ -164,8 +202,22 @@
 #endif
 }
 
+namespace {
+int winograd_output_any(const float* M, const int* amax, const float* uscale, const float* scale, const float* shift, float* out, int ld_out, int B,
+                        int H, int W, int N, int relu, int dil, int mt, hipStream_t s);
+}
 int launch_winograd_output(const float* M, const float* scale, const float* shift, float* out, int ld_out, int B, int H, int W, int N,
                            int relu, int dil, int mt, hipStream_t s) {
+    return winograd_output_any(M, nullptr, nullptr, scale, shift, out, ld_out, B, H, W, N, relu, dil, mt, s);
+}
+int launch_winograd_output_f16x2(const float* M, const int* amax, const float* uscale, const float* scale, const float* shift, float* out, int ld_out,
+                                 int B, int H, int W, int N, int relu, int dil, int mt, hipStream_t s) {
+    FS_REQUIRE(amax && uscale && ((uintptr_t)amax & 3) == 0 && ((uintptr_t)uscale & 15) == 0, "winograd_output_f16x2: no amax slots / filter scales");
+    return winograd_output_any(M, amax, uscale, scale, shift, out, ld_out, B, H, W, N, relu, dil, mt, s);
+}
+namespace {
+int winograd_output_any(const float* M, const int* amax, const float* uscale, const float* scale, const float* shift, float* out, int ld_out, int B,
+                        int H, int W, int N, int relu, int dil, int mt, hipStream_t s) {
     FS_REQUIRE(N % 4 == 0 && ld_out % 4 == 0 && dil >= 1, "winograd_output: N must be a multiple of 4");
     FS_REQUIRE(mt == 3 || mt == 4 || mt == 6, "winograd: tile size must be 3, 4 or 6");
     FS_REQUIRE(((uintptr_t)M & 15) == 0 && ((uintptr_t)out & 15) == 0 && ((uintptr_t)scale & 15) == 0 && ((uintptr_t)shift & 15) == 0,
@@ -177,17 +229,61 @@
     FS_REQUIRE(out_bytes < (1ll << 31), "winograd_output: output tensor must be smaller than 2 GiB");
     const dim3 grid((unsigned)cdiv(N / 4, 32), (unsigned)std::min<long long>(T, 65535));
     const WinoLayout lay = winograd_layout(mt, T, N);
-    if (mt == 3)
-        hipLaunchKernelGGL(winograd_output_kernel<3>, grid, dim3(5 * 32), 0, s, M, scale, shift, out, ld_out, B, H, W, N / 4, th, tw, relu, dil,
-                           lay.s_pos, lay.s_tile, (unsigned)out_bytes);
-    else if (mt == 4)
-        hipLaunchKernelGGL(winograd_output_kernel<4>, grid, dim3(6 * 32), 0, s, M, scale, shift, out, ld_out, B, H, W, N / 4, th, tw, relu, dil,
-                           lay.s_pos, lay.s_tile, (unsigned)out_bytes);
-    else
-        hipLaunchKernelGGL(winograd_output_kernel<6>, grid, dim3(8 * 32), 0, s, M, scale, shift, out, ld_out, B, H, W, N / 4, th, tw, relu, dil,
-                           lay.s_pos, lay.s_tile, (unsigned)out_bytes);
-    FS_HIP(hipGetLastError());
-    return 0;
-}
-
-}
+#define FS_WINO_OUT(MT_, F16_)                                                                                                                  \
+    hipLaunchKernelGGL((winograd_output_kernel<MT_, F16_>), grid, dim3((MT_ + 2) * 32), 0, s, M, scale, shift, out, ld_out, B, H, W, N / 4, th, tw, relu, \
+                       dil, lay.s_pos, lay.s_tile, (unsigned)out_bytes, amax, uscale)
+    if (amax && mt == 3) FS_WINO_OUT(3, true);
+    else if (amax && mt == 4) FS_WINO_OUT(4, true);
+    else if (amax) FS_WINO_OUT(6, true);
+    else if (mt == 3) FS_WINO_OUT(3, false);
+    else if (mt == 4) FS_WINO_OUT(4, false);
+    else FS_WINO_OUT(6, false);
+#undef FS_WINO_OUT
+    FS_HIP(hipGetLastError());
+    return 0;
+}
+}
+
+__global__ __launch_bounds__(256) void winograd_filter_f16x2_kernel(const float* __restrict__ U, unsigned* __restrict__ U16, float* __restrict__ uscale,
+                                                                    int O, int I, int G) {
+    __shared__ int red[256];
+    const int o = blockIdx.x, t = threadIdx.x;
+    const int pairs = I / 2;
+    const size_t plane_pairs = (size_t)G * O * pairs;
+    int mine = 0;
+    for (int i = t; i < G * I; i += 256) {
+        const int g = i / I, c = i - g * I;
+        const int bits = (int)(__float_as_uint(U[((size_t)g * O + o) * I + c]) & 0x7fffffffu);
+        mine = bits > mine ? bits : mine;
+    }
+    red[t] = mine;
+    __syncthreads();
+    for (int n = 128; n >= 1; n >>= 1) {
+        if (t < n) red[t] = red[t] > red[t + n] ? red[t] : red[t + n];
+        __syncthreads();
+    }
+    const int mx = red[0];
+    int f = mx == 0 ? 0 : ((mx >> 23) & 0xff) - 126 - 15;
+    f = f < -126 ? -126 : f > 126 ? 126 : f;
+    const float finv = pow2f(-f);
+    if (t == 0) uscale[o] = pow2f(f);
+    for (int i = t; i < G * pairs; i += 256) {
+        const int g = i / pairs, c2 = i - g * pairs;
+        const size_t at = ((size_t)g * O + o) * pairs + c2;
+        const f32x2 u = *reinterpret_cast<const f32x2*>(U + 2 * at);
+        unsigned h, m;
+        split16_pair(u[0] * finv, u[1] * finv, h, m);
+        U16[at] = h;
+        U16[plane_pairs + at] = m;
+    }
+}
+
+int launch_winograd_filter_f16x2(const float* U, void* U16, float* uscale, int O, int I, int mt, hipStream_t s) {
+    FS_REQUIRE(U && U16 && uscale && O >= 1 && I >= 2 && I % 2 == 0 && (mt == 3 || mt == 4 || mt == 6), "winograd_filter_f16x2: bad arguments");
+    FS_REQUIRE((((uintptr_t)U | (uintptr_t)U16) & 7) == 0, "winograd_filter_f16x2: unaligned operand");
+    hipLaunchKernelGGL(winograd_filter_f16x2_kernel, dim3((unsigned)O), dim3(256), 0, s, U, (unsigned*)U16, uscale, O, I, (mt + 2) * (mt + 2));
+    FS_HIP(hipGetLastError());
+    return 0;
+}
+
+}
diff --git a/flood_uav_video_segmentation_amd/model/hipnet.py b/flood_uav_video_segmentation_amd/model/hipnet.py
--- a/flood_uav_video_segmentation_amd/model/hipnet.py
+++ b/flood_uav_video_segmentation_amd/model/hipnet.py
@@ -8,7 +8,7 @@
 
 
 HIP_OPTIONS = ("hip_no_winograd", "hip_no_fused_head", "hip_no_fused_shortcut", "hip_no_fused_winograd", "hip_no_split_bf16", "hip_no_res_touch",
-               "hip_no_fused_pool", "hip_no_fused_qkv", "hip_winograd_tile")
+               "hip_no_fused_pool", "hip_no_fused_qkv", "hip_winograd_tile", "hip_no_wino_f16x2")
 
 
 def check_hip_options(names):
@@ -36,13 +36,14 @@
 class HipNet:
     def __init__(self, arch, layers, classes, patch=0, d_model=0, n_layers=0, dec_layers=0, image_size=0, no_winograd=False,
                  no_fused_head=False, no_fused_shortcut=False, winograd_tile=0, no_fused_winograd=False, no_split_bf16=False,
-                 no_res_touch=False, no_fused_pool=False, no_fused_qkv=False):
+                 no_res_touch=False, no_fused_pool=False, no_fused_qkv=False, no_wino_f16x2=False):
         self.arch, self.layers, self.classes = arch, int(layers), int(classes)
         self.vit = (int(patch), int(d_model), int(n_layers), int(dec_layers), int(image_size))
         self.flags = ((_lib.OPT_NO_WINOGRAD if no_winograd else 0) | (_lib.OPT_NO_FUSED_HEAD if no_fused_head else 0)
                       | (_lib.OPT_NO_FUSED_SHORTCUT if no_fused_shortcut else 0) | (_lib.OPT_NO_FUSED_WINOGRAD if no_fused_winograd else 0)
                       | (_lib.OPT_NO_SPLIT_BF16 if no_split_bf16 else 0) | (_lib.OPT_NO_RES_TOUCH if no_res_touch else 0)
-                      | (_lib.OPT_NO_FUSED_POOL if no_fused_pool else 0) | (_lib.OPT_NO_FUSED_QKV if no_fused_qkv else 0))
+                      | (_lib.OPT_NO_FUSED_POOL if no_fused_pool else 0) | (_lib.OPT_NO_FUSED_QKV if no_fused_qkv else 0)
+                      | (_lib.OPT_NO_WINO_F16X2 if no_wino_f16x2 else 0))
         self.winograd_tile = int(winograd_tile)
         self._h = None
         self.ready = False
@@ -242,7 +243,8 @@
 
     def __init__(self, hparams):
         super().__init__()
-        self._hip_net = HipNet(self.ARCH, hparams.layers, hparams.classes, **hip_options(hparams))
+        self._hip_net = HipNet(self.ARCH, hparams.layers, hparams.classes, no_wino_f16x2=bool(getattr(hparams, "hip_no_wino_f16x2", False)),
+                               **hip_options(hparams))
         self.encoder = HipStage(self._hip_net.encode, "encoder")
         self.decoder = HipStage(self._hip_net.decode, "decoder")
 
diff --git a/include/floodseg.h b/include/floodseg.h
--- a/include/floodseg.h
+++ b/include/floodseg.h
@@ -34,6 +34,7 @@
     FS_OPT_NO_SPLIT_BF16 = 16,
     FS_OPT_NO_FUSED_POOL = 256,
     FS_OPT_NO_RES_TOUCH = 128,
+    FS_OPT_NO_WINO_F16X2 = 2048,
     FS_OPT_NO_FUSED_QKV = 1024
 };
 
```

Result: no change. 1254 (median of 6 runs) (+0.4%).
